# mmigas/LiverRenderer

Hardware: AMD Instinct MI355X
Metric: Msamples/s (higher is better)
Workload: dtype f32; 1 GPU; C3 Liver-SingleMesh volpath 1920x1080 512 spp max_depth 12 (homogeneous medium, isotropic phase, envmap); width=1920, height=1080, spp=512, parallelism=1 GPU

## Files before the change

include/liverrt.h:

```cpp
#ifndef LIVERRT_H
#define LIVERRT_H

#include <stdint.h>
#include <stddef.h>

#ifdef __cplusplus
extern "C" {
#endif

#define LRT_API __attribute__((visibility("default")))

typedef enum {
    LRT_OK = 0,
    LRT_ERR_INVALID = 1,
    LRT_ERR_IO = 2,
    LRT_ERR_DEVICE = 3,
    LRT_ERR_UNSUPPORTED = 4
} lrt_status;

enum { LRT_INTEGRATOR_PATH = 0, LRT_INTEGRATOR_VOLPATH = 1, LRT_INTEGRATOR_PRBVOLPATH = 2,
       LRT_INTEGRATOR_VOLPATHMIS = 5,
       LRT_INTEGRATOR_BIOVOLPATH = 3,
       LRT_INTEGRATOR_BIOVOLPATH06 = 4    };
enum { LRT_MEDIUM_HOMOGENEOUS = 0, LRT_MEDIUM_LIVER = 1, LRT_MEDIUM_PARENCHYMA = 2, LRT_MEDIUM_GLISSON = 3,
// ... 129 lines not shown
} lrt_integrator_desc;

typedef struct {
    uint32_t n_vertices, n_faces, n_shapes, n_bsdfs, n_textures, n_media, n_emitters;
    const float    *positions;
    const float    *normals;
    const float    *texcoords;
    const uint32_t *faces;
    const uint32_t *face_shape;
    const lrt_shape_desc   *shapes;
    const lrt_bsdf_desc    *bsdfs;
    const lrt_texture_desc *textures;
    const lrt_medium_desc  *media;
    const lrt_emitter_desc *emitters;
    lrt_sensor_desc     sensor;
    lrt_film_desc       film;
    lrt_integrator_desc integrator;
    uint32_t sample_count;
    uint32_t sampler_seed;
    uint32_t sampler_type;
    uint32_t samples_per_pass;
    uint32_t use_spectral_mis;
    uint32_t pad;
    uint32_t n_phases, pad_phases;
    const lrt_phase_desc *phases;
} lrt_scene_desc;

typedef struct {
    int32_t  integrator;
    int32_t  max_depth;
    int32_t  rr_depth;
    int32_t  hide_emitters;
    uint32_t spp;
    uint32_t seed;
    uint32_t tile_rank, tile_count;
    int32_t  device;
    int32_t  output_on_device;
    int32_t  grad_medium;
    int32_t  pad;
} lrt_render_opts;

typedef struct {
    uint64_t n_samples;
    uint64_t n_iter;
    uint64_t n_shadow;
    uint64_t n_launches;
    uint64_t n_records;
    double   kernel_ms;
    double   total_ms;
    uint64_t lds_resident;
    uint64_t record_bytes;
    uint64_t n_closed_guard;
    uint64_t n_proven;
} lrt_render_stats;

typedef struct {
    float d_sigma_t[3];
    float d_albedo[3];
    float d_g;
} lrt_param_grads;

typedef struct lrt_scene lrt_scene;

LRT_API const char *lrt_last_error(void);
LRT_API int         lrt_version(void);

LRT_API lrt_status lrt_scene_load_xml(const char *path, const char *const *defines,
                                      int n_defines, lrt_scene **out);
LRT_API lrt_status lrt_scene_load_xml_string(const char *xml, const char *base_dir,
                                             const char *const *defines, int n_defines,
                                             lrt_scene **out);
LRT_API lrt_status lrt_scene_from_desc(const lrt_scene_desc *desc, lrt_scene **out);
LRT_API const lrt_scene_desc *lrt_scene_desc_get(const lrt_scene *scene);
LRT_API void       lrt_scene_free(lrt_scene *scene);

LRT_API lrt_status lrt_render(lrt_scene *scene, const lrt_render_opts *opts,
                              float *film_raw, float *image);
LRT_API lrt_status lrt_render_stats_get(const lrt_scene *scene, lrt_render_stats *out);
LRT_API lrt_status lrt_film_develop(lrt_scene *scene, const float *film_raw, float *image,
                                    int on_device);

LRT_API lrt_status lrt_render_samples(lrt_scene *scene, const lrt_render_opts *opts,
                                      uint64_t lane_begin, uint32_t n, float *out);

LRT_API lrt_status lrt_render_backward(lrt_scene *scene, const lrt_render_opts *opts,
                                       const float *grad_image, lrt_param_grads *out);

LRT_API lrt_status lrt_render_backward_grid(lrt_scene *scene, const lrt_render_opts *opts, const float *grad_image,
                                            lrt_param_grads *out, float *d_grid);

LRT_API lrt_status lrt_render_multi(lrt_scene *scene, const lrt_render_opts *opts, int n_devices, const int *device_ids,
                                    float *film_raw, float *image);
LRT_API lrt_status lrt_render_backward_multi(lrt_scene *scene, const lrt_render_opts *opts, int n_devices, const int *device_ids,
                                             const float *grad_image, lrt_param_grads *out);

LRT_API lrt_status lrt_math_eval(int fn, const float *x, const float *y, uint32_t n, float *out, float *out2, int device);

#define LRT_PROBE_FLOATS 20
LRT_API lrt_status lrt_emitter_probe(lrt_scene *scene, const float *ref_p, const float *sample, uint32_t n, float *out, int device);

LRT_API lrt_status lrt_envmap_probe(lrt_scene *scene, const float *dir, uint32_t n, float *out, int device);

#define LRT_BSDF_PROBE_FLOATS 30
LRT_API lrt_status lrt_bsdf_probe(lrt_scene *scene, const float *o, const float *d, const float *sample, const float *wo_query,
                                  uint32_t n, float *out, int device);

#define LRT_PHASE_PROBE_FLOATS 7
LRT_API lrt_status lrt_phase_probe(lrt_scene *scene, int medium, const float *wi, const float *sample, const float *wo_query,
                                   uint32_t n, float *out, int device);

#define LRT_MEDIUM_PROBE_FLOATS 22
LRT_API lrt_status lrt_medium_probe(lrt_scene *scene, int medium, const float *o, const float *d, const float *maxt, const float *sample,
                                    const uint32_t *channel, uint32_t n, float *out, int device);

#define LRT_SENSOR_PROBE_FLOATS 16
LRT_API lrt_status lrt_sensor_probe(lrt_scene *scene, const float *in, uint32_t n, float *out, int device);

typedef struct { const float *ox, *oy, *oz, *dx, *dy, *dz, *tmax; } lrt_rays_soa;
typedef struct { float *t, *u, *v; uint32_t *prim; } lrt_hits_soa;
LRT_API lrt_status lrt_trace(lrt_scene *scene, const lrt_rays_soa *rays,
                             const lrt_hits_soa *hits, uint32_t n, int any_hit);

LRT_API lrt_status lrt_param_set(lrt_scene *scene, const char *key, const float *v, int n);
LRT_API lrt_status lrt_param_get(const lrt_scene *scene, const char *key, float *v, int n);

LRT_API lrt_status lrt_image_read(const char *path, int *width, int *height, int *channels, float **data);
LRT_API void       lrt_image_free(float *data);
LRT_API lrt_status lrt_image_write_exr(const char *path, int width, int height, int channels, const float *data);
LRT_API lrt_status lrt_image_write_png(const char *path, int width, int height, int channels, const float *data);

#define LRT_AOV_MAX_INTEGRATORS 4
// ... 90 lines not shown
```

liverrenderer_amd/__init__.py:

```python
import ctypes as C
import math
import os

import numpy as np

from . import _lib
from ._lib import make_opts

__all__ = ["set_variant", "variant", "variants", "load_file", "load_string", "load_dict", "cornell_box", "render",
           "traverse", "Scene", "ScalarTransform4f", "render_stats", "write_volume_grid", "Bitmap", "Struct", "util", "read_image", "write_exr", "write_png",
           "Denoiser", "OptixDenoiser", "denoise", "moment_variance", "z_test"]

_VARIANT = "hip_ad_rgb"


def variants():
    return ["hip_ad_rgb"]


def set_variant(name):
    global _VARIANT
    if name not in variants():
        raise ImportError(f"Requested an unsupported variant \"{name}\". The following variants are available: "
                          + ", ".join(variants()) + ".")
# ... 339 lines not shown
        out = _lib.ParamGrads()
        _lib.check(self._lib.lrt_render_backward(self._h, C.byref(o), g.ctypes.data, C.byref(out)))
        return {"sigma_t": np.array(out.d_sigma_t[:], dtype=np.float32), "albedo": np.array(out.d_albedo[:], dtype=np.float32),
                "g": float(out.d_g)}

    def heterogeneous_media(self):
        d = self.desc
        return [i for i in range(d.n_media) if d.media[i].type == _lib.MEDIUM["heterogeneous"]]

    def grid_shape(self, medium):
        r = self.desc.media[medium].grid_res
        return (int(r[2]), int(r[1]), int(r[0]))

    def _render_backward_grid(self, grad_image, kw):
        m = kw.get("medium")
        if m is None or m < 0:
            het = self.heterogeneous_media()
            if len(het) != 1:
                raise RuntimeError(f"render_backward(grid=True): the scene holds {len(het)} heterogeneous media; name one with medium=")
            m = het[0]
        if not 0 <= m < self.desc.n_media or m not in self.heterogeneous_media():
            shape = None
        else:
            shape = self.grid_shape(m)
        out_t = kw.get("out")
        on_device = out_t is not None
        h, w, c = self.film_shape()
        if on_device:
            import torch
            if not _is_torch(out_t) or not out_t.is_cuda or out_t.dtype != torch.float32 or not out_t.is_contiguous() or (shape is not None and tuple(out_t.shape) != shape):
                raise RuntimeError(f"render_backward(grid=True): out must be a contiguous float32 CUDA tensor of shape {shape}")
            dev = out_t.device.index or 0
            if kw.get("device", dev) != dev:
                raise RuntimeError(f"render_backward(grid=True): out lives on {out_t.device}, the render was asked for device {kw['device']}")
            g = grad_image if _is_torch(grad_image) else torch.from_numpy(np.ascontiguousarray(grad_image, dtype=np.float32))
            g = g.to(device=out_t.device, dtype=torch.float32).contiguous()
            if g.numel() != h * w * c:
                raise RuntimeError(f"render_backward: grad_image has {g.numel()} values, the image {h * w * c}")
            torch.cuda.current_stream(out_t.device).synchronize()
            g_ptr, d_ptr, res = g.data_ptr(), out_t.data_ptr(), out_t
        else:
            g = np.ascontiguousarray(grad_image, dtype=np.float32)
            if g.size != h * w * c:
                raise RuntimeError(f"render_backward: grad_image has {g.size} values, the image {h * w * c}")
            res = np.empty(shape if shape is not None else (1,), dtype=np.float32)
            g_ptr, d_ptr, dev = g.ctypes.data, res.ctypes.data, kw.get("device", 0)
        o = make_opts(kw.get("integrator"), kw.get("max_depth"), kw.get("rr_depth"), kw.get("hide_emitters"), kw.get("spp", 0),
                      kw.get("seed", 0), kw.get("tile_rank", 0), kw.get("tile_count", 1), dev, on_device, grad_medium=m)
        out = _lib.ParamGrads()
        _lib.check(self._lib.lrt_render_backward_grid(self._h, C.byref(o), C.c_void_p(g_ptr), C.byref(out), C.c_void_p(d_ptr)))
        return {"sigma_t": np.array(out.d_sigma_t[:], dtype=np.float32), "albedo": np.array(out.d_albedo[:], dtype=np.float32),
                "g": float(out.d_g), "sigma_t_data": res}

    def stats(self):
        s = _lib.RenderStats()
        _lib.check(self._lib.lrt_render_stats_get(self._h, C.byref(s)))
        return {k: getattr(s, k) for k, _ in _lib.RenderStats._fields_}

    def trace(self, o, d, tmax=None, any_hit=False):
        o = np.ascontiguousarray(o, dtype=np.float32); d = np.ascontiguousarray(d, dtype=np.float32)
        n = o.shape[0]
        tmax = np.full(n, np.finfo(np.float32).max, dtype=np.float32) if tmax is None else np.ascontiguousarray(tmax, dtype=np.float32)
        cols = [np.ascontiguousarray(a) for a in (o[:, 0], o[:, 1], o[:, 2], d[:, 0], d[:, 1], d[:, 2], tmax)]
        t = np.empty(n, np.float32); u = np.empty(n, np.float32); v = np.empty(n, np.float32); prim = np.empty(n, np.uint32)
        FP = C.POINTER(C.c_float)
        rays = _lib.RaysSoA(*[c.ctypes.data_as(FP) for c in cols])
        hits = _lib.HitsSoA(t.ctypes.data_as(FP), u.ctypes.data_as(FP), v.ctypes.data_as(FP), prim.ctypes.data_as(C.POINTER(C.c_uint32)))
        _lib.check(self._lib.lrt_trace(self._h, C.byref(rays), C.byref(hits), n, int(any_hit)))
        return t, u, v, prim

    def _probe(self, name, inputs, out_width, alloc=np.empty, medium=None, device=0):
        cols = [np.ascontiguousarray(a, dtype=dt).reshape(-1, w) for _, a, w, dt in inputs]
        n = cols[0].shape[0]
        if any(c.shape[0] != n for c in cols):
            names = [i[0] for i in inputs]
            raise ValueError("%s: %s and %s must have the same number of rows" % (name, ", ".join(names[:-1]), names[-1]))
        out = alloc((n, out_width), dtype=np.float32)
        ptr = lambda a: a.ctypes.data_as(C.POINTER(np.ctypeslib.as_ctypes_type(a.dtype)))
        _lib.check(getattr(self._lib, "lrt_" + name)(self._h, *([] if medium is None else [int(medium)]), *map(ptr, cols), n, ptr(out), int(device)))
        return out

    def emitter_probe(self, ref_p, sample, device=0):
        out = self._probe("emitter_probe", [("ref_p", ref_p, 3, np.float32), ("sample", sample, 2, np.float32)], _lib.PROBE_FLOATS, device=device)
        return {"p": out[:, 0:3], "n": out[:, 3:6], "d": out[:, 6:9], "dist": out[:, 9], "pdf": out[:, 10], "weight": out[:, 11:14],
                "emitter": out[:, 14].astype(np.int32), "hit_shape": out[:, 15].astype(np.int32), "hit_pdf": out[:, 16], "hit_le": out[:, 17:20]}

    def envmap_probe(self, directions, device=0):
        out = self._probe("envmap_probe", [("directions", directions, 3, np.float32)], 4, device=device)
        return out[:, 0].copy(), out[:, 1:4].copy()

    def phase_probe(self, medium, wi, sample, wo_query, device=0):
        out = self._probe("phase_probe", [("wi", wi, 3, np.float32), ("sample", sample, 3, np.float32), ("wo_query", wo_query, 3, np.float32)],
                          _lib.PHASE_PROBE_FLOATS, np.zeros, medium, device)
        return {"wo": out[:, 0:3], "weight": out[:, 3], "pdf": out[:, 4], "eval": out[:, 5], "eval_pdf": out[:, 6]}

    def medium_probe(self, medium, o, d, maxt, sample, channel, device=0):
        out = self._probe("medium_probe", [("o", o, 3, np.float32), ("d", d, 3, np.float32), ("maxt", maxt, 1, np.float32), ("sample", sample, 1, np.float32),
                                           ("channel", channel, 1, np.uint32)], _lib.MEDIUM_PROBE_FLOATS, np.zeros, medium, device)
        return _lib.medium_probe_fields(out)

    def sensor_probe(self, inputs, device=0):
        return _lib.sensor_probe_fields(self._probe("sensor_probe", [("inputs", inputs, 5, np.float32)], _lib.SENSOR_PROBE_FLOATS, np.zeros, device=device))

    def bsdf_probe(self, o, d, sample, wo_query, device=0):
        out = self._probe("bsdf_probe", [("o", o, 3, np.float32), ("d", d, 3, np.float32), ("sample", sample, 3, np.float32), ("wo_query", wo_query, 3, np.float32)],
                          _lib.BSDF_PROBE_FLOATS, device=device)
# ... 475 lines not shown
```

liverrenderer_amd/_lib.py:

```python
import ctypes as C
import os

_HERE = os.path.dirname(os.path.abspath(__file__))
LIB_PATH = os.environ.get("LRT_LIBRARY") or os.path.join(_HERE, "libliverrt.so")

OK, INVALID, UNSUPPORTED = 0, 1, 4
INTEGRATOR = {"path": 0, "volpath": 1, "prbvolpath": 2, "biovolpath": 3, "biovolpath06": 4, "volpathmis": 5}
MEDIUM = {"homogeneous": 0, "liver": 1, "parenchyma": 2, "glissonCapsule": 3, "heterogeneous": 4}
EMITTER = {"area": 0, "envmap": 1, "constant": 2, "point": 3, "spot": 4, "directional": 5}
PROBE_FLOATS = 20
MEDIUM_PROBE_FLOATS = 22
PHASE_PROBE_FLOATS = 7
SENSOR_PROBE_FLOATS = 16
BSDF_PROBE_FLOATS = 30


class ShapeDesc(C.Structure):
    _fields_ = [("kind", C.c_int32), ("first_face", C.c_uint32), ("n_faces", C.c_uint32), ("bsdf", C.c_int32),
                ("emitter", C.c_int32), ("interior_medium", C.c_int32), ("exterior_medium", C.c_int32),
                ("has_normals", C.c_int32), ("has_texcoords", C.c_int32), ("flip_normals", C.c_int32),
                ("to_world", C.c_float * 16)]


class TextureDesc(C.Structure):
# ... 38 lines not shown
class SensorDesc(C.Structure):
    _fields_ = [("to_world", C.c_float * 16), ("fov_x", C.c_float), ("near_clip", C.c_float), ("far_clip", C.c_float),
                ("medium", C.c_int32), ("principal_point_offset_x", C.c_float), ("principal_point_offset_y", C.c_float), ("pad", C.c_int32)]


class FilmDesc(C.Structure):
    _fields_ = [("width", C.c_int32), ("height", C.c_int32), ("crop_offset_x", C.c_int32), ("crop_offset_y", C.c_int32),
                ("crop_width", C.c_int32), ("crop_height", C.c_int32), ("has_alpha", C.c_int32), ("rfilter", C.c_int32),
                ("rfilter_param", C.c_float)]


class IntegratorDesc(C.Structure):
    _fields_ = [("type", C.c_int32), ("max_depth", C.c_int32), ("rr_depth", C.c_int32), ("hide_emitters", C.c_int32)]


class SceneDesc(C.Structure):
    _fields_ = [("n_vertices", C.c_uint32), ("n_faces", C.c_uint32), ("n_shapes", C.c_uint32), ("n_bsdfs", C.c_uint32),
                ("n_textures", C.c_uint32), ("n_media", C.c_uint32), ("n_emitters", C.c_uint32),
                ("positions", C.POINTER(C.c_float)), ("normals", C.POINTER(C.c_float)), ("texcoords", C.POINTER(C.c_float)),
                ("faces", C.POINTER(C.c_uint32)), ("face_shape", C.POINTER(C.c_uint32)),
                ("shapes", C.POINTER(ShapeDesc)), ("bsdfs", C.POINTER(BsdfDesc)), ("textures", C.POINTER(TextureDesc)),
                ("media", C.POINTER(MediumDesc)), ("emitters", C.POINTER(EmitterDesc)),
                ("sensor", SensorDesc), ("film", FilmDesc), ("integrator", IntegratorDesc),
                ("sample_count", C.c_uint32), ("sampler_seed", C.c_uint32),
                ("sampler_type", C.c_uint32), ("samples_per_pass", C.c_uint32), ("use_spectral_mis", C.c_uint32), ("pad", C.c_uint32),
                ("n_phases", C.c_uint32), ("pad_phases", C.c_uint32), ("phases", C.POINTER(PhaseDesc))]


AOV_MAX_INTEGRATORS, AOV_MAX_AOVS, AOV_NAME_LEN = 4, 16, 64
AOV_TYPES = {"albedo": 0, "depth": 1, "position": 2, "uv": 3, "geo_normal": 4, "sh_normal": 5, "dp_du": 6, "dp_dv": 7,
             "prim_index": 8, "shape_index": 9}


class AovDesc(C.Structure):
    _fields_ = [("n_integrators", C.c_int32), ("integrators", IntegratorDesc * AOV_MAX_INTEGRATORS),
                ("integrator_names", (C.c_char * AOV_NAME_LEN) * AOV_MAX_INTEGRATORS),
                ("n_aovs", C.c_int32), ("aov_types", C.c_int32 * AOV_MAX_AOVS), ("aov_names", (C.c_char * AOV_NAME_LEN) * AOV_MAX_AOVS),
                ("n_aov_channels", C.c_int32), ("n_channels", C.c_int32)]


class MomentDesc(C.Structure):
    _fields_ = [("integrator", IntegratorDesc), ("name", C.c_char * AOV_NAME_LEN), ("n_channels", C.c_int32), ("n_raw_channels", C.c_int32)]


class RenderOpts(C.Structure):
    _fields_ = [("integrator", C.c_int32), ("max_depth", C.c_int32), ("rr_depth", C.c_int32), ("hide_emitters", C.c_int32),
                ("spp", C.c_uint32), ("seed", C.c_uint32), ("tile_rank", C.c_uint32), ("tile_count", C.c_uint32),
                ("device", C.c_int32), ("output_on_device", C.c_int32), ("grad_medium", C.c_int32), ("pad", C.c_int32)]


class RenderStats(C.Structure):
    _fields_ = [("n_samples", C.c_uint64), ("n_iter", C.c_uint64), ("n_shadow", C.c_uint64), ("n_launches", C.c_uint64),
                ("n_records", C.c_uint64), ("kernel_ms", C.c_double), ("total_ms", C.c_double), ("lds_resident", C.c_uint64),
                ("record_bytes", C.c_uint64), ("n_closed_guard", C.c_uint64), ("n_proven", C.c_uint64)]


class ParamGrads(C.Structure):
    _fields_ = [("d_sigma_t", C.c_float * 3), ("d_albedo", C.c_float * 3), ("d_g", C.c_float)]


class DenoiseParams(C.Structure):
    _fields_ = [("iterations", C.c_int32), ("sigma_color", C.c_float), ("sigma_normal", C.c_float), ("sigma_albedo", C.c_float), ("eps_a", C.c_float)]


class RaysSoA(C.Structure):
    _fields_ = [(n, C.POINTER(C.c_float)) for n in ("ox", "oy", "oz", "dx", "dy", "dz", "tmax")]


class HitsSoA(C.Structure):
    _fields_ = [("t", C.POINTER(C.c_float)), ("u", C.POINTER(C.c_float)), ("v", C.POINTER(C.c_float)), ("prim", C.POINTER(C.c_uint32))]


def make_opts(integrator=None, max_depth=None, rr_depth=None, hide_emitters=None, spp=0, seed=0,
              tile_rank=0, tile_count=1, device=0, output_on_device=False, grad_medium=0):
    o = RenderOpts()
    o.integrator = -1 if integrator is None else (INTEGRATOR[integrator] if isinstance(integrator, str) else int(integrator))
    o.max_depth = -2 if max_depth is None else int(max_depth)
    o.rr_depth = -1 if rr_depth is None else int(rr_depth)
    o.hide_emitters = -1 if hide_emitters is None else int(bool(hide_emitters))
    o.spp, o.seed, o.tile_rank, o.tile_count = int(spp), int(seed) & 0xffffffff, int(tile_rank), int(tile_count)
    o.device, o.output_on_device = int(device), int(bool(output_on_device))
    o.grad_medium = int(grad_medium)
    return o


_lib = None


def _pytorch_context_first():
    import importlib.util
    import sys
    if os.environ.get("LRT_NO_TORCH_INIT"):
        return "skipped"
    if "torch" not in sys.modules and importlib.util.find_spec("torch") is None:
        return "no torch"
    import torch
    if not torch.cuda.is_available():
        return "no device"
    if not torch.cuda.is_initialized():
        lr = os.environ.get("LOCAL_RANK")
        if lr is not None and lr.isdigit() and torch.cuda.device_count() > 0:
            torch.cuda.set_device(int(lr) % torch.cuda.device_count())
        torch.zeros(1, device="cuda")
    if not torch.cuda.is_initialized():
        raise RuntimeError("PyTorch is importable but its HIP context could not be created before libliverrt.so was loaded; "
                           "set LRT_NO_TORCH_INIT=1 if this process does not use PyTorch")
    return "initialised"


def lib():
    global _lib
    if _lib is not None:
        return _lib
    _pytorch_context_first()
    if not os.path.exists(LIB_PATH):
        raise RuntimeError(f"{LIB_PATH} is missing: build it with `python -c 'import __graft_entry__ as g; g.build()'` "
                           "(the hip_ad_rgb back-end has no CPU fallback)")
    L = C.CDLL(LIB_PATH)
    P = C.POINTER
    L.lrt_last_error.restype = C.c_char_p
    L.lrt_version.restype = C.c_int
    L.lrt_scene_load_xml.argtypes = [C.c_char_p, P(C.c_char_p), C.c_int, P(C.c_void_p)]
    L.lrt_scene_load_xml_string.argtypes = [C.c_char_p, C.c_char_p, P(C.c_char_p), C.c_int, P(C.c_void_p)]
    L.lrt_scene_from_desc.argtypes = [P(SceneDesc), P(C.c_void_p)]
    L.lrt_scene_desc_get.argtypes = [C.c_void_p]
    L.lrt_scene_desc_get.restype = P(SceneDesc)
    L.lrt_scene_free.argtypes = [C.c_void_p]
    L.lrt_scene_free.restype = None
    L.lrt_render.argtypes = [C.c_void_p, P(RenderOpts), C.c_void_p, C.c_void_p]
    L.lrt_render_multi.argtypes = [C.c_void_p, P(RenderOpts), C.c_int, P(C.c_int), C.c_void_p, C.c_void_p]
    L.lrt_render_backward_multi.argtypes = [C.c_void_p, P(RenderOpts), C.c_int, P(C.c_int), C.c_void_p, P(ParamGrads)]
    L.lrt_math_eval.argtypes = [C.c_int, P(C.c_float), P(C.c_float), C.c_uint32, P(C.c_float), P(C.c_float), C.c_int]
    L.lrt_render_stats_get.argtypes = [C.c_void_p, P(RenderStats)]
    L.lrt_film_develop.argtypes = [C.c_void_p, C.c_void_p, C.c_void_p, C.c_int]
    L.lrt_render_samples.argtypes = [C.c_void_p, P(RenderOpts), C.c_uint64, C.c_uint32, C.c_void_p]
    L.lrt_render_backward.argtypes = [C.c_void_p, P(RenderOpts), C.c_void_p, P(ParamGrads)]
    L.lrt_render_backward_grid.argtypes = [C.c_void_p, P(RenderOpts), C.c_void_p, P(ParamGrads), C.c_void_p]
    L.lrt_render_backward_grid.restype = C.c_int
    L.lrt_trace.argtypes = [C.c_void_p, P(RaysSoA), P(HitsSoA), C.c_uint32, C.c_int]
    F, U = P(C.c_float), P(C.c_uint32)
    for name, medium, arrays in (("lrt_emitter_probe", 0, [F, F]), ("lrt_envmap_probe", 0, [F]), ("lrt_bsdf_probe", 0, [F, F, F, F]),
                                 ("lrt_phase_probe", 1, [F, F, F]), ("lrt_medium_probe", 1, [F, F, F, F, U]), ("lrt_sensor_probe", 0, [F])):
        getattr(L, name).argtypes = [C.c_void_p] + [C.c_int] * medium + arrays + [C.c_uint32, F, C.c_int]
        getattr(L, name).restype = C.c_int
    L.lrt_param_set.argtypes = [C.c_void_p, C.c_char_p, P(C.c_float), C.c_int]
    L.lrt_param_get.argtypes = [C.c_void_p, C.c_char_p, P(C.c_float), C.c_int]
    L.lrt_image_read.argtypes = [C.c_char_p, P(C.c_int), P(C.c_int), P(C.c_int), P(P(C.c_float))]
    L.lrt_image_free.argtypes = [P(C.c_float)]
    L.lrt_image_free.restype = None
    L.lrt_image_write_exr.argtypes = [C.c_char_p, C.c_int, C.c_int, C.c_int, C.c_void_p]
    L.lrt_image_write_png.argtypes = [C.c_char_p, C.c_int, C.c_int, C.c_int, C.c_void_p]
    L.lrt_image_write_exr_channels.argtypes = [C.c_char_p, C.c_int, C.c_int, C.c_int, P(C.c_char_p), C.c_void_p]
    L.lrt_scene_aov_get.argtypes = [C.c_void_p, P(AovDesc)]
    L.lrt_aov_channel_name.argtypes = [C.c_void_p, C.c_int]
    L.lrt_aov_channel_name.restype = C.c_char_p
    L.lrt_render_aov.argtypes = [C.c_void_p, P(RenderOpts), C.c_void_p, C.c_void_p]
    L.lrt_render_aov_samples.argtypes = [C.c_void_p, P(RenderOpts), C.c_uint64, C.c_uint32, C.c_void_p]
    L.lrt_scene_moment_get.argtypes = [C.c_void_p, P(MomentDesc)]
    L.lrt_moment_channel_name.argtypes = [C.c_void_p, C.c_int]
    L.lrt_moment_channel_name.restype = C.c_char_p
    L.lrt_render_moment.argtypes = [C.c_void_p, P(RenderOpts), C.c_void_p, C.c_void_p]
    L.lrt_render_moment_samples.argtypes = [C.c_void_p, P(RenderOpts), C.c_uint64, C.c_uint32, C.c_void_p]
    L.lrt_denoiser_create.argtypes = [C.c_int, C.c_int, C.c_int, C.c_int, C.c_int, P(DenoiseParams), C.c_int, P(C.c_void_p)]
    L.lrt_denoise.argtypes = [C.c_void_p, C.c_void_p, C.c_int, C.c_void_p, C.c_void_p, C.c_void_p, C.c_int]
    L.lrt_denoiser_free.argtypes = [C.c_void_p]
    L.lrt_denoiser_free.restype = None
    L.lrt_denoiser_get.argtypes = [C.c_void_p, P(C.c_int), P(C.c_int), P(DenoiseParams)]
    L.lrt_image_read_named.argtypes = [C.c_char_p, P(C.c_int), P(C.c_int), P(C.c_int), P(P(C.c_float)), P(C.c_void_p)]
    L.lrt_image_free_names.argtypes = [C.c_void_p]
    L.lrt_image_free_names.restype = None
    for name in ("lrt_denoiser_create", "lrt_denoise", "lrt_denoiser_get", "lrt_image_read_named", "lrt_scene_moment_get", "lrt_render_moment", "lrt_render_moment_samples"):
        getattr(L, name).restype = C.c_int
    for name in ("lrt_image_read", "lrt_image_write_exr", "lrt_image_write_png", "lrt_scene_load_xml", "lrt_scene_load_xml_string", "lrt_scene_from_desc", "lrt_render", "lrt_render_multi", "lrt_render_backward_multi", "lrt_math_eval", "lrt_render_stats_get",
                 "lrt_film_develop", "lrt_render_samples", "lrt_render_backward", "lrt_trace", "lrt_param_set", "lrt_param_get",
                 "lrt_image_write_exr_channels", "lrt_scene_aov_get", "lrt_render_aov", "lrt_render_aov_samples"):
        getattr(L, name).restype = C.c_int
    _lib = L
    return L


EXPORTED_SYMBOLS = ["lrt_last_error", "lrt_version", "lrt_scene_load_xml", "lrt_scene_load_xml_string", "lrt_scene_from_desc",
                    "lrt_scene_desc_get", "lrt_scene_free", "lrt_render", "lrt_render_multi", "lrt_render_backward_multi", "lrt_math_eval", "lrt_render_stats_get", "lrt_film_develop",
                    "lrt_render_samples", "lrt_render_backward", "lrt_render_backward_grid", "lrt_trace", "lrt_emitter_probe", "lrt_envmap_probe", "lrt_bsdf_probe", "lrt_phase_probe", "lrt_medium_probe", "lrt_sensor_probe", "lrt_param_set", "lrt_param_get",
                    "lrt_image_read", "lrt_image_free", "lrt_image_write_exr", "lrt_image_write_png",
                    "lrt_vae_model_create", "lrt_vae_model_free", "lrt_vae_scatter",
                    "lrt_scene_aov_get", "lrt_aov_channel_name", "lrt_render_aov", "lrt_render_aov_samples", "lrt_image_write_exr_channels",
                    "lrt_denoiser_create", "lrt_denoise", "lrt_denoiser_free", "lrt_denoiser_get", "lrt_image_read_named", "lrt_image_free_names",
                    "lrt_scene_moment_get", "lrt_moment_channel_name", "lrt_render_moment", "lrt_render_moment_samples"]


def bsdf_probe_fields(out):
    return {"shape": out[:, 0].astype("int32"), "t": out[:, 1], "p": out[:, 2:5], "n": out[:, 5:8], "sh_n": out[:, 8:11], "uv": out[:, 11:13],
            "wi": out[:, 13:16], "wo": out[:, 16:19], "wo_z": out[:, 19], "pdf": out[:, 20], "eta": out[:, 21], "type": out[:, 22].astype("int32"),
            "weight": out[:, 23:26], "eval": out[:, 26:29], "eval_pdf": out[:, 29], "raw": out}


def medium_probe_fields(out):
    return {"valid": out[:, 0] != 0, "t": out[:, 1], "p": out[:, 2:5], "mint": out[:, 5], "sigma_t": out[:, 6:9], "sigma_s": out[:, 9:12],
            "sigma_n": out[:, 12:15], "combined": out[:, 15:18], "local": out[:, 18:21], "grid": out[:, 21], "raw": out}


def sensor_probe_fields(out):
    return {"o": out[:, 0:3], "d": out[:, 3:6], "maxt": out[:, 6], "adjusted": out[:, 7:9], "origin": out[:, 9:11].astype("int64"),
            "rel": out[:, 11:13], "weight": out[:, 13], "fcount": out[:, 14].astype("int64"), "raw": out}


def check(status):
    if status != OK:
        raise RuntimeError(lib().lrt_last_error().decode("utf-8", "replace"))
```

liverrenderer_amd/csrc/capi.cpp:

```cpp
#include "host_scene.h"
#include "device_scene.h"
#include "scene_prep.h"
#include "scene_check.h"
#include "image_io.h"
#include <algorithm>
#include <cmath>
#include <cstring>
#include <cstdio>
#include <fstream>
#include <sstream>
#include <stdexcept>

using namespace lrt;

static thread_local std::string g_error;
static lrt_status fail(lrt_status st, const std::string &msg) { g_error = msg; return st; }

#define LRT_TRY try {
#define LRT_CATCH } catch (const std::exception &e) { \
        std::string m = e.what(); \
        lrt_status st = LRT_ERR_INVALID; \
        if (m.find("hip") != std::string::npos || m.find("HIP") != std::string::npos) st = LRT_ERR_DEVICE; \
        if (m.find("cannot open") != std::string::npos || m.find("file not found") != std::string::npos) st = LRT_ERR_IO; \
        if (m.find("unsupported") != std::string::npos || m.find("not supported") != std::string::npos) st = LRT_ERR_UNSUPPORTED; \
        return fail(st, m); \
    } catch (...) { return fail(LRT_ERR_INVALID, "unknown error"); }

extern "C" {

const char *lrt_last_error(void) { return g_error.c_str(); }
int lrt_version(void) { return 120; }

static std::vector<std::pair<std::string, std::string>> parse_defines(const char *const *defines, int n) {
    std::vector<std::pair<std::string, std::string>> r;
    for (int i = 0; i < n; ++i) {
        std::string s = defines[i]; size_t eq = s.find('=');
        if (eq == std::string::npos) throw std::runtime_error("define \"" + s + "\" must have the form key=value");
        r.emplace_back(s.substr(0, eq), s.substr(eq + 1));
    }
    return r;
}

lrt_status lrt_scene_load_xml_string(const char *xml, const char *base_dir, const char *const *defines, int n_defines, lrt_scene **out) {
    if (!xml || !out) return fail(LRT_ERR_INVALID, "lrt_scene_load_xml_string: null argument");
    *out = nullptr;
    LRT_TRY
        std::unique_ptr<lrt_scene> s(new lrt_scene());
        load_scene_xml(xml, base_dir ? base_dir : "", parse_defines(defines, n_defines), s->st);
        *out = s.release();
        return LRT_OK;
    LRT_CATCH
}

lrt_status lrt_scene_load_xml(const char *path, const char *const *defines, int n_defines, lrt_scene **out) {
    if (!path || !out) return fail(LRT_ERR_INVALID, "lrt_scene_load_xml: null argument");
    *out = nullptr;
    std::ifstream f(path, std::ios::binary);
    if (!f) return fail(LRT_ERR_IO, std::string("cannot open \"") + path + "\"");
    std::stringstream ss; ss << f.rdbuf();
    std::string p = path, dir; size_t sl = p.rfind('/'); dir = sl == std::string::npos ? "." : p.substr(0, sl);
    return lrt_scene_load_xml_string(ss.str().c_str(), dir.c_str(), defines, n_defines, out);
}

lrt_status lrt_scene_from_desc(const lrt_scene_desc *desc, lrt_scene **out) {
    if (!desc || !out) return fail(LRT_ERR_INVALID, "lrt_scene_from_desc: null argument");
    *out = nullptr;
    LRT_TRY
        validate_scene_desc(*desc);
        std::unique_ptr<lrt_scene> s(new lrt_scene());
        s->st.copy_from(*desc);
        *out = s.release();
        return LRT_OK;
    LRT_CATCH
}

const lrt_scene_desc *lrt_scene_desc_get(const lrt_scene *scene) { return scene ? &scene->st.desc : nullptr; }

static void multi_release(lrt_scene *s) {
    if (s->multi_ctx) { multi_context_destroy(s->multi_ctx); s->multi_ctx = nullptr; }
    for (auto *D : s->multi) device_scene_destroy(D);
    s->multi.clear(); s->multi_ids.clear();
}

void lrt_scene_free(lrt_scene *scene) {
// ... 146 lines not shown
    if (st != LRT_OK) return st;
    LRT_TRY
        ensure_device(scene, opts ? opts->device : 0);
        device_render_aov_samples(scene->dev, scene->st.desc, scene->st.aov, opts, lane_begin, n, out, scene->stats);
        return LRT_OK;
    LRT_CATCH
}

lrt_status lrt_scene_moment_get(const lrt_scene *scene, lrt_moment_desc *out) {
    if (!scene || !out) return fail(LRT_ERR_INVALID, "lrt_scene_moment_get: null argument");
    if (!scene->st.has_moment) return fail(LRT_ERR_INVALID, "lrt_scene_moment_get: the scene has no moment integrator");
    *out = scene->st.moment; return LRT_OK;
}

const char *lrt_moment_channel_name(const lrt_scene *scene, int c) {
    if (!scene || !scene->st.has_moment || c < 0 || c >= (int) scene->st.moment_channel_names.size()) return nullptr;
    return scene->st.moment_channel_names[(size_t) c].c_str();
}

static lrt_status check_moment_call(const lrt_scene *scene, const lrt_render_opts *opts, const char *fn) {
    if (!scene->st.has_moment) return fail(LRT_ERR_INVALID, std::string(fn) + ": the scene has no moment integrator");
    if (opts && (opts->integrator != -1 || opts->max_depth != -2 || opts->rr_depth != -1 || opts->hide_emitters != -1))
        return fail(LRT_ERR_INVALID, std::string(fn) + ": integrator, max_depth, rr_depth and hide_emitters come from the scene's nested integrator (leave them at -1 / -2 / -1 / -1)");
    return LRT_OK;
}

lrt_status lrt_render_moment(lrt_scene *scene, const lrt_render_opts *opts, float *film_raw, float *image) {
    if (!scene) return fail(LRT_ERR_INVALID, "lrt_render_moment: null scene");
    lrt_status st = check_moment_call(scene, opts, "lrt_render_moment");
    if (st != LRT_OK) return st;
    LRT_TRY
        ensure_device(scene, opts ? opts->device : 0);
        device_render_moment(scene->dev, scene->st.desc, opts, film_raw, image, scene->stats);
        return LRT_OK;
    LRT_CATCH
}

lrt_status lrt_render_moment_samples(lrt_scene *scene, const lrt_render_opts *opts, uint64_t lane_begin, uint32_t n, float *out) {
    if (!scene || !out) return fail(LRT_ERR_INVALID, "lrt_render_moment_samples: null argument");
    lrt_status st = check_moment_call(scene, opts, "lrt_render_moment_samples");
    if (st != LRT_OK) return st;
    LRT_TRY
        ensure_device(scene, opts ? opts->device : 0);
        device_render_moment_samples(scene->dev, scene->st.desc, opts, lane_begin, n, out, scene->stats);
        return LRT_OK;
    LRT_CATCH
}

lrt_status lrt_trace(lrt_scene *scene, const lrt_rays_soa *rays, const lrt_hits_soa *hits, uint32_t n, int any_hit) {
    if (!scene || !rays || !hits) return fail(LRT_ERR_INVALID, "lrt_trace: null argument");
    LRT_TRY
        ensure_device(scene, -1);
        device_trace(scene->dev, rays, hits, n, any_hit);
        return LRT_OK;
    LRT_CATCH
}

static lrt_status probe_call(const char *fn, ProbeKind kind, lrt_scene *scene, const int *medium, std::initializer_list<ProbeColumn> columns, uint32_t n, float *out, int device) {
    bool null = !scene || (!out && n);
    for (const ProbeColumn &c : columns) null = null || (!c.p && n);
    if (null) return fail(LRT_ERR_INVALID, std::string(fn) + ": null argument");
    if (medium && (*medium < 0 || (size_t) *medium >= scene->st.media.size())) return fail(LRT_ERR_INVALID, std::string(fn) + ": no such medium");
    LRT_TRY
        ensure_device(scene, device);
        device_probe(scene->dev, kind, medium ? *medium : 0, columns, n, out);
        return LRT_OK;
    LRT_CATCH
}

lrt_status lrt_emitter_probe(lrt_scene *scene, const float *ref_p, const float *sample, uint32_t n, float *out, int device) {
    return probe_call("lrt_emitter_probe", PROBE_EMITTER, scene, nullptr, { { ref_p, 3 }, { sample, 2 } }, n, out, device);
}

lrt_status lrt_envmap_probe(lrt_scene *scene, const float *dir, uint32_t n, float *out, int device) {
    return probe_call("lrt_envmap_probe", PROBE_ENVMAP, scene, nullptr, { { dir, 3 } }, n, out, device);
}

lrt_status lrt_bsdf_probe(lrt_scene *scene, const float *o, const float *d, const float *sample, const float *wo_query, uint32_t n, float *out, int device) {
    return probe_call("lrt_bsdf_probe", PROBE_BSDF, scene, nullptr, { { o, 3 }, { d, 3 }, { sample, 3 }, { wo_query, 3 } }, n, out, device);
}

lrt_status lrt_phase_probe(lrt_scene *scene, int medium, const float *wi, const float *sample, const float *wo_query, uint32_t n, float *out, int device) {
    return probe_call("lrt_phase_probe", PROBE_PHASE, scene, &medium, { { wi, 3 }, { sample, 3 }, { wo_query, 3 } }, n, out, device);
}

lrt_status lrt_medium_probe(lrt_scene *scene, int medium, const float *o, const float *d, const float *maxt, const float *sample, const uint32_t *channel,
                            uint32_t n, float *out, int device) {
    LRT_TRY
        std::vector<float> ch;
        if (channel) for (uint32_t i = 0; i < n; ++i) ch.push_back((float) std::min<uint32_t>(channel[i], 2u));
        return probe_call("lrt_medium_probe", PROBE_MEDIUM, scene, &medium, { { o, 3 }, { d, 3 }, { maxt, 1 }, { sample, 1 }, { channel ? ch.data() : nullptr, 1 } }, n, out, device);
    LRT_CATCH
}

lrt_status lrt_sensor_probe(lrt_scene *scene, const float *in, uint32_t n, float *out, int device) {
    return probe_call("lrt_sensor_probe", PROBE_SENSOR, scene, nullptr, { { in, 5 } }, n, out, device);
}

static lrt_medium_desc *find_medium(lrt_scene *s, const char *key, const char **rest) {
    for (auto &M : s->st.media) {
        size_t L = strlen(M.id);
        if (!strncmp(key, M.id, L) && key[L] == '.') { *rest = key + L + 1; return &M; }
    }
    return nullptr;
}

// ... 204 lines not shown
```

liverrenderer_amd/csrc/device.hip:

```cpp
#include "host_scene.h"
#include "device_scene.h"
#include "kernels_prb.h"
#include "kernels_vae.h"
#include "kernels_aov.h"
#include "kernels_denoise.h"
#include "kernels_moment.h"
#include "probes.h"
#include <functional>
#include "scene_prep.h"
#include <cmath>
#include <array>
#include <cstring>
#include <algorithm>
#include <stdexcept>
#include <string>
#include <cstdio>
#include <cstdlib>
#include <thread>
#include <chrono>
#include <exception>
#include <dlfcn.h>
#include <rccl/rccl.h>

namespace lrt {

#define HIP_CHECK(expr) do { hipError_t e_ = (expr); if (e_ != hipSuccess) throw std::runtime_error(std::string(#expr) + ": " + hipGetErrorString(e_)); } while (0)

template <typename T> static T *dev_upload(const T *src, size_t n, hipStream_t st) {
    T *p = nullptr; size_t bytes = std::max<size_t>(n, 1) * sizeof(T);
    HIP_CHECK(hipMalloc((void **) &p, bytes));
    if (n) HIP_CHECK(hipMemcpyAsync(p, src, n * sizeof(T), hipMemcpyHostToDevice, st));
    return p;
}

struct DevTmp {
    float *p = nullptr;
    DevTmp() = default;
    explicit DevTmp(size_t floats) { alloc(floats); }
    DevTmp(const DevTmp &) = delete; DevTmp &operator=(const DevTmp &) = delete;
    void alloc(size_t floats) { HIP_CHECK(hipMalloc((void **) &p, std::max<size_t>(floats, 1) * sizeof(float))); }
    void upload(const float *src, size_t floats, hipStream_t st) { alloc(floats); HIP_CHECK(hipMemcpyAsync(p, src, floats * sizeof(float), hipMemcpyHostToDevice, st)); }
    ~DevTmp() { if (p) (void) hipFree(p); }
};

static void select_device(int device) {
    int count = 0;
    if (hipGetDeviceCount(&count) != hipSuccess || count == 0) throw std::runtime_error("no HIP device available: the hip_ad_rgb back-end has no CPU fallback");
    if (device < 0 || device >= count) throw std::runtime_error("invalid HIP device ordinal " + std::to_string(device));
    HIP_CHECK(hipSetDevice(device));
}

static lrt_render_opts default_opts() { return lrt_render_opts{ -1, -2, -1, -1, 0, 0, 0, 1, 0, 0, 0, 0 }; }

static void add_stats(lrt_render_stats &total, const lrt_render_stats &s) {
    total.n_samples += s.n_samples; total.n_iter += s.n_iter; total.n_shadow += s.n_shadow; total.n_launches += s.n_launches;
    total.n_records += s.n_records; total.kernel_ms += s.kernel_ms; total.total_ms += s.total_ms;
    total.record_bytes = s.record_bytes; total.n_closed_guard += s.n_closed_guard; total.n_proven += s.n_proven;
}

#define LRT_LAUNCH_SLOTS 64
#define LRT_WIDE_BLOCK 768

struct DeviceScene {
    int device = 0;
    hipStream_t stream = nullptr;
    DScene sc{};
    DScene *d_sc = nullptr;
    DLaunch *d_launch = nullptr, *h_launch = nullptr; uint32_t launch_next = 0;
    std::vector<void *> allocs;
    uint32_t capacity = 0;
    DPathStreams q[2]{};
    float4 *dl[2] = { nullptr, nullptr }; size_t dl_records[2] = { 0, 0 }; float4 *L_buf = nullptr; size_t l_buf_lanes = 0;
    double *d_grads = nullptr; float *wfilm = nullptr; size_t wfilm_floats = 0; float *grad_image = nullptr; size_t grad_floats = 0;
    DCounters *counters = nullptr;
    DCounters *h_counters = nullptr;
    float *film = nullptr; size_t film_floats = 0;
    float *image = nullptr; size_t image_floats = 0;
    unsigned long long *pass_state[2] = { nullptr, nullptr }; size_t pass_state_lanes[2] = { 0, 0 };
    const unsigned long long *cur_pass_in = nullptr; unsigned long long *cur_pass_out = nullptr;
    uint32_t *pixel_slot = nullptr;
    uint32_t *pixel_list = nullptr; uint32_t pixel_list_rank = 0xffffffffu, pixel_list_count = 0, n_owned_pixels = 0;
    uint32_t *halo_list = nullptr; uint32_t halo_rank = 0xffffffffu, halo_count = 0, halo_width = 0, n_halo_pixels = 0;
    std::vector<hipEvent_t> ev_pool;
    std::vector<DMedium> h_media; DMedium *d_media = nullptr;
    std::vector<DBioMedium> h_bio; DBioMedium *d_bio = nullptr;
    std::vector<DHetMedium> h_het; DHetMedium *d_het = nullptr; std::vector<float *> het_data; bool has_het = false, has_non_bio = false, need_mis = false; uint32_t ws_layouts = 0;
    bool ext = false;
    bool smooth_bsdf = false;
    bool has_area_emitter = false;
    float *dgrid = nullptr; size_t dgrid_floats = 0;
    bool prb_null = false;
    DLdsInfo lds{}; bool use_lds = false; int n_cus = 256; int bvh_leaf = 4;
    DAovSpec *d_aov_spec = nullptr; uint32_t *d_first_face = nullptr;
    float *aov_film = nullptr; size_t aov_film_floats = 0; float *aov_image = nullptr; size_t aov_image_floats = 0; float *aov_inner = nullptr; size_t aov_inner_floats = 0;

    template <typename T> T *track(T *p) { allocs.push_back((void *) p); return p; }
    void release(void *p) {
        if (!p) return;
        for (auto it = allocs.begin(); it != allocs.end(); ++it) if (*it == p) { allocs.erase(it); break; }
        (void) hipFree(p);
    }
    template <typename T> T *grow(T *&p, size_t &have, size_t want) {
        if (have >= want) return p;
        HIP_CHECK(hipStreamSynchronize(stream));
        release(p); p = nullptr; have = 0;
        HIP_CHECK(hipMalloc((void **) &p, std::max<size_t>(want, 1) * sizeof(T))); track(p);
        have = want;
        return p;
    }
    ~DeviceScene() {
        for (void *p : allocs) (void) hipFree(p);
        for (auto e : ev_pool) (void) hipEventDestroy(e);
        if (h_counters) (void) hipHostFree(h_counters);
        if (h_launch) (void) hipHostFree(h_launch);
        if (stream) (void) hipStreamDestroy(stream);
    }
};

void device_scene_destroy(DeviceScene *d) { delete d; }

static_assert(PREP_F_DELTA == F_DELTA && PREP_F_SMOOTH == F_SMOOTH && PREP_F_NULL == F_NULL, "scene_prep.h restates the BSDF leaf flags of dshade.h");

__global__ void k_bio_prepare(DBioMedium *bio, uint32_t n) {
    const uint32_t i = blockIdx.x * blockDim.x + threadIdx.x;
    if (i < n) bio[i].log10_hep = m_log2(bio[i].hepatocity + 1.f) / m_log2(10.f);
}

__global__ void k_medium_prepare(DMedium *media, uint32_t n) {
// ... 110 lines not shown
    prepare_geometry(d, opt, P);
    D->n_cus = opt.n_cus; D->bvh_leaf = P.bvh_leaf; D->ext = P.ext; D->smooth_bsdf = P.smooth_bsdf;
    auto up = [&](const auto &v) { return D->track(dev_upload(v.data(), v.size(), st)); };
    sc.spheres = P.spheres.empty() ? nullptr : up(P.spheres);
    sc.nodes = (const float4 *) up(P.bvh.nodes);
    sc.tris = (const float4 *) up(P.bvh.tris);
    if (P.use_lds) {
        D->lds = P.lds; D->lds.blob = (const uint4 *) up(P.lds_blob);
        const size_t lds_limit = opt.lds_limit;
        auto raise_lds = [&](const void *k) { if (k) HIP_CHECK(hipFuncSetAttribute(k, hipFuncAttributeMaxDynamicSharedMemorySize, (int) lds_limit)); };
        const KernelTable &K = kernels();
        for (const RenderRow &r : K.render) if (r.lds && (!r.ext || D->ext)) raise_lds((const void *) r.fn);
        for (const auto &adjoint : K.prb) for (const auto &ld : adjoint[1]) for (RenderFn fn : ld) raise_lds((const void *) fn);
        for (RenderFn fn : K.prb_grid[1]) raise_lds((const void *) fn);
        for (int i = 0; i < 2; ++i) for (int ext = 0; ext <= (D->ext ? 1 : 0); ++ext) {
            raise_lds((const void *) aov_kernel(true, i, ext)); raise_lds((const void *) trace_lds_kernel(i, ext));
        }
        D->use_lds = true;
    }
    if (sc.grid.enabled) {
        const size_t n_cells = (size_t) sc.grid.n[0] * sc.grid.n[1] * sc.grid.n[2];
        uint16_t *buf = nullptr; HIP_CHECK(hipMalloc((void **) &buf, n_cells * sizeof(uint16_t))); D->track(buf);
        k_build_dist_grid<<<(uint32_t) ((n_cells + LRT_BLOCK - 1) / LRT_BLOCK), LRT_BLOCK, 0, st>>>(sc.tris, d.n_faces ? (uint32_t) (P.bvh.tris.size() / 12) : 0u, sc.grid, buf, P.grid_abs_margin,
                                                                                             sc.spheres, sc.n_spheres);
        HIP_CHECK(hipGetLastError());
        sc.grid.d = buf;
    }
    prepare_shading(d, opt, P);
    D->has_area_emitter = P.has_area_emitter; D->has_het = P.has_het; D->has_non_bio = P.has_non_bio; D->prb_null = P.prb_null;
    sc.positions = D->track(dev_upload(d.positions, 3 * (size_t) d.n_vertices, st));
    sc.vattr = (const float4 *) up(P.vattr);
    sc.faces = D->track(dev_upload(d.faces, 3 * (size_t) d.n_faces, st));
    sc.face_shape = D->track(dev_upload(d.face_shape, d.n_faces, st));
    sc.shapes = up(P.shapes);
    sc.textures = up(P.textures);
    sc.tex_data = up(P.tex_data);
    sc.bsdfs = up(P.bsdfs);
    HIP_CHECK(hipMalloc((void **) &D->d_media, std::max<uint32_t>(d.n_media, 1) * sizeof(DMedium))); D->track(D->d_media);
    HIP_CHECK(hipMalloc((void **) &D->d_bio, std::max<uint32_t>(d.n_media, 1) * sizeof(DBioMedium))); D->track(D->d_bio);
    HIP_CHECK(hipMalloc((void **) &D->d_het, std::max<uint32_t>(d.n_media, 1) * sizeof(DHetMedium))); D->track(D->d_het);
    D->het_data.assign(std::max<uint32_t>(d.n_media, 1), nullptr);
    for (uint32_t i = 0; i < d.n_media; ++i) {
        const lrt_medium_desc &M = d.media[i];
        if (M.type == LRT_MEDIUM_HETEROGENEOUS) D->het_data[i] = D->track(dev_upload(M.grid_data, (size_t) M.grid_res[0] * M.grid_res[1] * M.grid_res[2], st));
    }
    D->sc = sc;
    upload_media(D.get(), d); sc.media = D->d_media; sc.bio = D->d_bio; sc.het = D->d_het;
    sc.emitters = up(P.emitters);
    sc.mesh_emitters = up(P.mesh_emitters);
    sc.mesh_emitter_tab = up(P.mesh_emitter_tab);
    sc.delta_emitters = P.delta_emitters.empty() ? nullptr : up(P.delta_emitters);
    sc.bsdf_ext = P.bsdf_ext.empty() ? nullptr : up(P.bsdf_ext);
    sc.cone_tab = P.cone_tab.empty() ? nullptr : (const uint2 *) up(P.cone_tab);
    sc.phases = P.phases.empty() ? nullptr : up(P.phases);
    sc.phase_pool = P.phase_pool.empty() ? nullptr : up(P.phase_pool);
    sc.env_data = (const float4 *) up(P.env_data);
    sc.env_hier = up(P.env_hier);
    HIP_CHECK(hipMalloc((void **) &D->d_sc, sizeof(DScene))); D->track(D->d_sc);
    D->sc = sc;
    HIP_CHECK(hipMemcpyAsync(D->d_sc, &D->sc, sizeof(DScene), hipMemcpyHostToDevice, st));
    HIP_CHECK(hipMalloc((void **) &D->d_launch, LRT_LAUNCH_SLOTS * sizeof(DLaunch))); D->track(D->d_launch);
    HIP_CHECK(hipHostMalloc((void **) &D->h_launch, LRT_LAUNCH_SLOTS * sizeof(DLaunch)));
    HIP_CHECK(hipMalloc((void **) &D->counters, sizeof(DCounters))); D->track(D->counters);
    HIP_CHECK(hipHostMalloc((void **) &D->h_counters, sizeof(DCounters)));
    HIP_CHECK(hipStreamSynchronize(st));
    return D.release();
}

void device_scene_update_params(DeviceScene *D, const lrt_scene_desc &d, bool grids) {
    HIP_CHECK(hipSetDevice(D->device));
    if (grids) for (uint32_t i = 0; i < d.n_media; ++i) {
        const lrt_medium_desc &M = d.media[i];
        if (M.type == LRT_MEDIUM_HETEROGENEOUS && D->het_data[i])
            HIP_CHECK(hipMemcpyAsync(D->het_data[i], M.grid_data, (size_t) M.grid_res[0] * M.grid_res[1] * M.grid_res[2] * sizeof(float), hipMemcpyHostToDevice, D->stream));
    }
    upload_media(D, d);
    HIP_CHECK(hipStreamSynchronize(D->stream));
}

static void ensure_workspace(DeviceScene *D, uint32_t capacity) {
    const uint32_t layouts = workspace_layouts(D->has_het, D->need_mis);
    if (D->capacity >= capacity && D->ws_layouts == layouts) return;
    HIP_CHECK(hipStreamSynchronize(D->stream));
    D->capacity = 0;
    auto get = [](const DPathStreams *q, const RecordStream &r) { void *p; memcpy(&p, (const char *) q + r.member, sizeof p); return p; };
    auto set = [](DPathStreams *q, const RecordStream &r, void *p) { memcpy((char *) q + r.member, &p, sizeof p); };
    for (DPathStreams *q : { &D->q[0], &D->q[1] })
        for (const RecordStream &r : kRecordStreams) if (r.member != kNoMember) { D->release(get(q, r)); set(q, r, nullptr); }
    for (DPathStreams *q : { &D->q[0], &D->q[1] })
        for (size_t k = 0; k < std::size(kRecordStreams); ++k) if (const uint32_t bytes = workspace_stream_bytes(k, layouts)) {
            void *p = nullptr; HIP_CHECK(hipMalloc(&p, (size_t) capacity * bytes)); D->track(p); set(q, kRecordStreams[k], p);
        }
    D->capacity = capacity; D->ws_layouts = layouts;
}

static hipEvent_t get_event(DeviceScene *D, size_t i) {
    while (D->ev_pool.size() <= i) { hipEvent_t e; HIP_CHECK(hipEventCreate(&e)); D->ev_pool.push_back(e); }
    return D->ev_pool[i];
}

static void ensure_pixel_list(DeviceScene *D, const ResolvedOpts &O) {
    const DFilm &F = D->sc.film;
    if (O.tile_count == 1) { D->n_owned_pixels = (uint32_t) F.width * F.height; return; }
    if (D->pixel_list && D->pixel_list_rank == O.tile_rank && D->pixel_list_count == O.tile_count) return;
    const TilePixels T = tile_pixel_list(F, O.tile_rank, O.tile_count);
    D->release(D->pixel_list); D->release(D->pixel_slot); D->pixel_list = nullptr; D->pixel_slot = nullptr;
// ... 114 lines not shown
        case LRT_INTEGRATOR_PATH: case LRT_INTEGRATOR_BIOVOLPATH: case LRT_INTEGRATOR_BIOVOLPATH06: mode = integrator; break;
        case LRT_INTEGRATOR_VOLPATHMIS: mode = spectral_mis ? LRT_INTEGRATOR_VOLPATHMIS : LRT_INTEGRATOR_VOLPATHMIS_PLAIN; break;
        default: mode = closed ? LRT_INTEGRATOR_VOLPATH_CLOSED : (has_het ? LRT_INTEGRATOR_VOLPATH_HET : LRT_INTEGRATOR_VOLPATH);
    }
    for (const RenderRow &r : kernels().render) if (r.mode == mode && r.lds == lds && r.ld == ld && r.compact == compact && r.ext == ext) return r;
    throw std::runtime_error("no render-kernel instance for mode " + std::to_string(mode) + (lds ? ", LDS BVH" : ", global BVH") + (ld ? ", ld sampler" : ", independent sampler") +
                             (compact ? ", compact records" : ", wide records") + (ext ? ", EXT" : ""));
}

static void run_wavefront(DeviceScene *D, const lrt_scene_desc &d, const ResolvedOpts &O, uint64_t lane_begin, uint64_t n_lanes,
                          const uint32_t *pixel_list, float *film, float *sample_out, lrt_render_stats &stats) {
    hipStream_t st = D->stream;
    DRenderParams rp = make_params(d, O, n_lanes);
    rp.pixel_slot = pixel_list ? D->pixel_slot : nullptr;
    rp.pass_in = D->cur_pass_in; rp.pass_out = D->cur_pass_out;
    const bool prb = O.integrator == LRT_INTEGRATOR_PRBVOLPATH;
    check_integrator_media(D, O.integrator);
    PoolGeometry g = pool_geometry(D, n_lanes);
    const uint32_t records = (uint32_t) std::min<uint64_t>((uint64_t) g.n_wg * 2u * g.P, 0xffffffffull);
    ensure_workspace(D, records);
    if (prb) ensure_prb_workspace(D, records, 0);
    HIP_CHECK(hipMemsetAsync(D->counters, 0, sizeof(DCounters), st));
    LaunchLog log;
    hipEvent_t e_begin = get_event(D, log.ev++), e_end = get_event(D, log.ev++);
    HIP_CHECK(hipEventRecord(e_begin, st));
    const bool count_iter = !(O.integrator == LRT_INTEGRATOR_PATH && O.max_depth == 0);
    hipEvent_t a = get_event(D, log.ev++), b = get_event(D, log.ev++);
    HIP_CHECK(hipEventRecord(a, st));
    if (prb) { stats.record_bytes = 0; launch_prb<false>(D, rp, g, pixel_list, lane_begin, nullptr, nullptr, nullptr, film, sample_out); }
    else {
        DLaunch a{}; a.rp = rp; a.li = D->lds; a.q0 = D->q[0]; a.q1 = D->q[1]; a.P = g.P; a.cnt = D->counters; a.pixel_list = pixel_list;
        a.lane_begin = lane_begin; a.n = n_lanes; a.film = film; a.sample_out = sample_out; a.sample_base = lane_begin;
        const bool compact = D->use_lds && !D->has_area_emitter && !D->ext && !getenv("LRT_WIDE_RECORDS") && O.integrator != LRT_INTEGRATOR_VOLPATHMIS && !(O.integrator == LRT_INTEGRATOR_VOLPATH && D->has_het);
        const bool closed = compact && O.integrator == LRT_INTEGRATOR_VOLPATH && closed_records(d, D->sc.cam.medium) && !getenv("LRT_NO_CLOSED_RECORDS");
#ifdef LRT_DEV_VOLPATH_ONLY
        if (D->ext) throw std::runtime_error("developer build: no EXT instances (spheres / point emitters)");
        if (!(D->use_lds && (O.integrator == LRT_DEV_INTEGRATOR || (LRT_DEV_INTEGRATOR == LRT_INTEGRATOR_VOLPATH_HET && D->has_het)) && (rp.ld_count != 0) == LRT_DEV_LD)) throw std::runtime_error("developer build: one integrator / sampler / LDS BVH only");
#endif
        const RenderRow &row = select_render_kernel(O.integrator, D->has_het, d.use_spectral_mis != 0, D->use_lds, rp.ld_count != 0, D->ext, compact, closed);
        stats.record_bytes = row.record_bytes;
        const LaunchPtr lp = push_launch(D, a);
        row.fn<<<g.n_wg, row.block, g.smem, st>>>((ScenePtr) D->d_sc, lp);
        HIP_CHECK(hipGetLastError());
    }
    HIP_CHECK(hipEventRecord(b, st));
    log.launches.emplace_back(a, b); log.sizes.push_back(0);
    HIP_CHECK(hipMemcpyAsync(D->h_counters, D->counters, sizeof(DCounters), hipMemcpyDeviceToHost, st));
    HIP_CHECK(hipStreamSynchronize(st));
    log.n_iter = count_iter ? D->h_counters->n_iter : 0;
    log.n_records = D->h_counters->n_records;
    finish_stats(D, log, e_begin, e_end, n_lanes, stats);
    stats.n_closed_guard = D->h_counters->n_closed_guard;
    stats.n_proven = D->h_counters->n_proven;
    if (stats.n_closed_guard)
        throw std::runtime_error("64-byte path records: " + std::to_string(stats.n_closed_guard) + " trips broke the premise of the layout (radiance before a path's last trip, "
                                 "or an emitter hit that needs its MIS weight); the scene test in closed_records() is wrong for this scene: LRT_NO_CLOSED_RECORDS=1 renders it with 80-byte records");
}

static void render_passes(DeviceScene *D, const lrt_scene_desc &d, const lrt_render_opts *opts, float *film_raw, float *image, lrt_render_stats &stats,
                          const std::function<void(const ResolvedOpts &)> &after_pass, bool moment = false);

void device_render(DeviceScene *D, const lrt_scene_desc &d, const lrt_render_opts *opts, float *film_raw, float *image, lrt_render_stats &stats) {
    render_passes(D, d, opts, film_raw, image, stats, nullptr);
}

static void develop_and_download(DeviceScene *D, const float *film, float *film_raw, float *image, size_t film_floats, size_t image_floats, bool on_device, bool moment = false) {
    const DFilm &F = D->sc.film; const size_t np = (size_t) F.width * F.height;
    if (image) {
        float *img = on_device ? image : D->grow(D->image, D->image_floats, image_floats);
        if (!moment) k_develop<<<(uint32_t) ((np + 255) / 256), 256, 0, D->stream>>>(F, film, img, (uint32_t) np);
        else if (F.has_alpha) k_moment_develop<true><<<(uint32_t) ((np + 255) / 256), 256, 0, D->stream>>>(film, img, (uint32_t) np);
        else k_moment_develop<false><<<(uint32_t) ((np + 255) / 256), 256, 0, D->stream>>>(film, img, (uint32_t) np);
        if (!on_device) HIP_CHECK(hipMemcpyAsync(image, img, image_floats * 4, hipMemcpyDeviceToHost, D->stream));
    }
    if (film_raw && !on_device) HIP_CHECK(hipMemcpyAsync(film_raw, film, film_floats * 4, hipMemcpyDeviceToHost, D->stream));
    HIP_CHECK(hipStreamSynchronize(D->stream));
    HIP_CHECK(hipGetLastError());
}

static void render_passes(DeviceScene *D, const lrt_scene_desc &d, const lrt_render_opts *opts, float *film_raw, float *image, lrt_render_stats &stats,
                          const std::function<void(const ResolvedOpts &)> &after_pass, bool moment) {
    HIP_CHECK(hipSetDevice(D->device));
    ResolvedOpts O = resolve(d, opts);
    const DFilm &F = D->sc.film;
    bool on_device = opts && opts->output_on_device;
    const size_t film_channels = moment ? (F.has_alpha ? 11 : 10) : (size_t) F.channels, image_channels = moment ? film_channels - 1 : (F.has_alpha ? 4 : 3);
    size_t np = (size_t) F.width * F.height, film_floats = np * film_channels, image_floats = np * image_channels;
    ensure_pixel_list(D, O);
    const uint64_t n_lanes = (uint64_t) D->n_owned_pixels * O.spp;
    float *film = (on_device && film_raw) ? film_raw : D->grow(D->film, D->film_floats, film_floats);
    HIP_CHECK(hipMemsetAsync(film, 0, film_floats * 4, D->stream));
    const uint32_t *pixel_list = O.tile_count > 1 ? D->pixel_list : nullptr;
    const bool carry = O.n_passes > 1 && d.sampler_type != LRT_SAMPLER_LD;
    if (carry) for (int k = 0; k < 2; ++k) D->grow(D->pass_state[k], D->pass_state_lanes[k], n_lanes);
    const bool lane_splat = moment || (F.rfilter != LRT_RFILTER_BOX && (O.n_passes > 1 || !getenv("LRT_NO_LANE_SPLAT")));
    lrt_render_stats total{};
    for (uint32_t pass = 0; pass < O.n_passes; ++pass) {
        O.pass = pass;
        D->cur_pass_in = carry ? D->pass_state[pass & 1] : nullptr;
        D->cur_pass_out = (carry && pass + 1 < O.n_passes) ? D->pass_state[(pass & 1) ^ 1] : nullptr;
        if (!lane_splat) {
            lrt_render_stats st1{};
            run_wavefront(D, d, O, 0, n_lanes, pixel_list, film, nullptr, st1);
            add_stats(total, st1);
            if (after_pass) after_pass(O);
            continue;
        }
        const uint64_t chunk = std::min<uint64_t>(std::max<uint64_t>(n_lanes, 1), 1ull << 28);
        ensure_prb_workspace(D, 0, chunk);
        for (uint64_t base = 0; base < n_lanes; base += chunk) {
            const uint64_t n = std::min<uint64_t>(chunk, n_lanes - base);
            lrt_render_stats st1{};
            run_wavefront(D, d, O, base, n, pixel_list, nullptr, reinterpret_cast<float *>(D->L_buf), st1);
            DRenderParams rp = make_params(d, O, n); rp.pass_in = D->cur_pass_in;
            DLaunch a{}; a.rp = rp; a.L_buf = D->L_buf; a.pixel_list = pixel_list; a.lane_begin = base; a.n = n; a.film = film;
            const uint32_t grid = (uint32_t) ((n + LRT_BLOCK - 1) / LRT_BLOCK);
            const LaunchPtr lp = push_launch(D, a);
            if (!moment) k_splat_lanes<false><<<grid, LRT_BLOCK, 0, D->stream>>>((ScenePtr) D->d_sc, lp);
            else moment_splat_kernel(F.rfilter != LRT_RFILTER_BOX, F.has_alpha != 0)<<<grid, LRT_BLOCK, 0, D->stream>>>((ScenePtr) D->d_sc, lp);
            HIP_CHECK(hipGetLastError());
            add_stats(total, st1);
        }
        if (after_pass) after_pass(O);
    }
    D->cur_pass_in = nullptr; D->cur_pass_out = nullptr;
    total.lds_resident = D->use_lds ? 1 : 0;
    stats = total;
    develop_and_download(D, film, film_raw, image, film_floats, image_floats, on_device, moment);
}

void device_render_moment(DeviceScene *D, const lrt_scene_desc &d, const lrt_render_opts *opts, float *film_raw, float *image, lrt_render_stats &stats) {
    render_passes(D, d, opts, film_raw, image, stats, nullptr, true);
}

void device_render_moment_samples(DeviceScene *D, const lrt_scene_desc &d, const lrt_render_opts *opts, uint64_t lane_begin, uint32_t n, float *out, lrt_render_stats &stats) {
    HIP_CHECK(hipSetDevice(D->device));
    ResolvedOpts O = resolve(d, opts);
    if (lane_begin + n > 0x100000000ull) throw std::runtime_error("lane range exceeds 2^32");
    if (!n) { stats = lrt_render_stats{}; return; }
    DevTmp buf((size_t) n * 10);
    float *d_buf = buf.p, *d_m = d_buf + (size_t) n * 4;
    HIP_CHECK(hipMemsetAsync(d_buf, 0, (size_t) n * 16, D->stream));
    run_wavefront(D, d, O, lane_begin, n, nullptr, nullptr, d_buf, stats);
    k_moment_lanes<<<(n + 255u) / 256u, 256, 0, D->stream>>>(reinterpret_cast<const float4 *>(d_buf), O.integrator == LRT_INTEGRATOR_PATH ? 1 : 0, n, d_m);
    HIP_CHECK(hipGetLastError());
    HIP_CHECK(hipMemcpyAsync(out, d_m, (size_t) n * 24, hipMemcpyDeviceToHost, D->stream));
    HIP_CHECK(hipStreamSynchronize(D->stream));
}

void device_develop(DeviceScene *D, const float *film_raw, float *image, int on_device) {
    HIP_CHECK(hipSetDevice(D->device));
    const DFilm &F = D->sc.film;
    size_t np = (size_t) F.width * F.height, film_floats = np * F.channels, image_floats = np * (F.has_alpha ? 4 : 3);
    const float *film = film_raw;
    if (!on_device) {
        film = D->grow(D->film, D->film_floats, film_floats);
        HIP_CHECK(hipMemcpyAsync(D->film, film_raw, film_floats * 4, hipMemcpyHostToDevice, D->stream));
    }
    develop_and_download(D, film, nullptr, image, film_floats, image_floats, on_device != 0);
}

void device_render_samples(DeviceScene *D, const lrt_scene_desc &d, const lrt_render_opts *opts, uint64_t lane_begin, uint32_t n, float *out, lrt_render_stats &stats) {
    HIP_CHECK(hipSetDevice(D->device));
    ResolvedOpts O = resolve(d, opts);
    if (lane_begin + n > 0x100000000ull) throw std::runtime_error("lane range exceeds 2^32");
    DevTmp d_out((size_t) n * 4);
    HIP_CHECK(hipMemsetAsync(d_out.p, 0, (size_t) n * 16, D->stream));
    run_wavefront(D, d, O, lane_begin, n, nullptr, nullptr, d_out.p, stats);
    HIP_CHECK(hipMemcpyAsync(out, d_out.p, (size_t) n * 16, hipMemcpyDeviceToHost, D->stream));
    HIP_CHECK(hipStreamSynchronize(D->stream));
}

static void upload_aov_spec(DeviceScene *D, const lrt_scene_desc &d, const lrt_aov_desc &aov) {
    if (!D->d_aov_spec) { HIP_CHECK(hipMalloc((void **) &D->d_aov_spec, sizeof(DAovSpec))); D->track(D->d_aov_spec); }
    if (!D->d_first_face) {
        std::vector<uint32_t> ff(std::max<uint32_t>(d.n_shapes, 1), 0u);
        for (uint32_t i = 0; i < d.n_shapes; ++i) ff[i] = d.shapes[i].first_face;
        D->d_first_face = D->track(dev_upload(ff.data(), ff.size(), D->stream));
    }
    static thread_local DAovSpec h;
    h = DAovSpec{}; h.n_aovs = aov.n_aovs; h.first_face = D->d_first_face;
    int off = 0;
    for (int k = 0; k < aov.n_aovs; ++k) {
        h.type[k] = aov.aov_types[k]; h.offset[k] = off;
        off += aov.aov_types[k] == LRT_AOV_DEPTH || aov.aov_types[k] >= LRT_AOV_PRIM_INDEX ? 1 : aov.aov_types[k] == LRT_AOV_UV ? 2 : 3;
    }
    h.n_ch = off;
    if (off != aov.n_aov_channels) throw std::runtime_error("aov: channel count mismatch");
    HIP_CHECK(hipMemcpyAsync(D->d_aov_spec, &h, sizeof(DAovSpec), hipMemcpyHostToDevice, D->stream));
    HIP_CHECK(hipStreamSynchronize(D->stream));
}

static void launch_aov(DeviceScene *D, const lrt_scene_desc &d, const ResolvedOpts &O, uint64_t lane_begin, uint64_t n, float *film, float *sample_out,
                       const unsigned long long *pass_in, unsigned long long *pass_out) {
    if (!n) return;
    hipStream_t st = D->stream;
    DRenderParams rp = make_params(d, O, n);
    rp.pass_in = pass_in; rp.pass_out = pass_out;
    DLaunch a{}; a.rp = rp; a.li = D->lds; a.lane_begin = lane_begin; a.n = n; a.film = film; a.sample_out = sample_out; a.sample_base = lane_begin;
    const LaunchPtr lp = push_launch(D, a);
    const AovSpecPtr spec = (AovSpecPtr) D->d_aov_spec;
    const AovFn fn = aov_kernel(D->use_lds, rp.ld_count != 0, D->ext);
// ... 259 lines not shown
        std::vector<int> ids; for (auto *D : devs) ids.push_back(D->device);
        if (!ctx || ctx->devices != ids) {
            delete ctx; ctx = new MultiContext(); ctx->devices = ids; ctx->comms.assign(N, nullptr);
            g_rccl.check(g_rccl.CommInitAll(ctx->comms.data(), N, ids.data()), "ncclCommInitAll");
        }
        g_rccl.check(g_rccl.GroupStart(), "ncclGroupStart");
        for (int i = 0; i < N; ++i) {
            HIP_CHECK(hipSetDevice(devs[i]->device));
            g_rccl.check(g_rccl.AllReduce(buf[i], buf[i], count, sizeof(T) == 8 ? ncclDouble : ncclFloat, ncclSum, ctx->comms[i], devs[i]->stream), "ncclAllReduce");
        }
        g_rccl.check(g_rccl.GroupEnd(), "ncclGroupEnd");
        for (auto *D : devs) { HIP_CHECK(hipSetDevice(D->device)); HIP_CHECK(hipStreamSynchronize(D->stream)); }
    } else {
        for (int i = 1; i < N; ++i) if (devs[i]->device != devs[0]->device) throw std::runtime_error("lrt_render_multi: a device list is either all distinct or one device repeated");
        static_assert(sizeof(T) == 4 || sizeof(T) == 8, "float or double");
        HIP_CHECK(hipSetDevice(devs[0]->device));
        for (int i = 1; i < N; ++i) {
            if (sizeof(T) == 4) k_film_add<<<(uint32_t) ((count + 255) / 256), 256, 0, devs[0]->stream>>>((float *) buf[0], (const float *) buf[i], count);
            else { std::vector<double> a(count), b(count); HIP_CHECK(hipMemcpy(a.data(), buf[0], count * 8, hipMemcpyDeviceToHost)); HIP_CHECK(hipMemcpy(b.data(), buf[i], count * 8, hipMemcpyDeviceToHost));
                   for (size_t k = 0; k < count; ++k) a[k] += b[k]; HIP_CHECK(hipMemcpy(buf[0], a.data(), count * 8, hipMemcpyHostToDevice)); }
        }
        HIP_CHECK(hipGetLastError()); HIP_CHECK(hipStreamSynchronize(devs[0]->stream));
    }
}

template <typename F> static void on_every_device(size_t n, F fn) {
    std::vector<std::exception_ptr> err(n);
    std::vector<std::thread> th;
    for (size_t i = 0; i < n; ++i) th.emplace_back([&, i]() { try { fn(i); } catch (...) { err[i] = std::current_exception(); } });
    for (auto &t : th) t.join();
    for (auto &e : err) if (e) std::rethrow_exception(e);
}

void device_render_multi(std::vector<DeviceScene *> &devs, MultiContext *&ctx, const lrt_scene_desc &d, const lrt_render_opts *opts, float *film_raw, float *image, lrt_render_stats &stats) {
    const int N = (int) devs.size();
    const DFilm &F = devs[0]->sc.film;
    const size_t np = (size_t) F.width * F.height, film_floats = np * F.channels, image_floats = np * (F.has_alpha ? 4 : 3);
    const bool on_device = opts && opts->output_on_device;
    std::vector<float *> films(N); std::vector<lrt_render_stats> st(N);
    const auto t0 = std::chrono::steady_clock::now();
    on_every_device(N, [&](size_t i) {
        HIP_CHECK(hipSetDevice(devs[i]->device));
        films[i] = (i == 0 && on_device && film_raw) ? film_raw : devs[i]->grow(devs[i]->film, devs[i]->film_floats, film_floats);
        lrt_render_opts o = opts ? *opts : default_opts();
        o.tile_rank = (uint32_t) i; o.tile_count = (uint32_t) N; o.device = devs[i]->device; o.output_on_device = 1;
        device_render(devs[i], d, &o, films[i], nullptr, st[i]);
    });
    if (N > 1 || getenv("LRT_MULTI_ALWAYS_REDUCE")) reduce_across(devs, ctx, films, film_floats);
    DeviceScene *D0 = devs[0];
    HIP_CHECK(hipSetDevice(D0->device));
    develop_and_download(D0, films[0], film_raw, image, film_floats, image_floats, on_device);
    lrt_render_stats total{};
    for (auto &x : st) { total.n_samples += x.n_samples; total.n_iter += x.n_iter; total.n_shadow += x.n_shadow; total.n_launches += x.n_launches; total.n_records += x.n_records;
                         total.kernel_ms = std::max(total.kernel_ms, x.kernel_ms); total.lds_resident = x.lds_resident; total.record_bytes = x.record_bytes; total.n_closed_guard += x.n_closed_guard; total.n_proven += x.n_proven; }
    total.total_ms = std::chrono::duration<double, std::milli>(std::chrono::steady_clock::now() - t0).count();
    stats = total;
}

void device_render_backward_multi(std::vector<DeviceScene *> &devs, MultiContext *&ctx, const lrt_scene_desc &d, const lrt_render_opts *opts, const float *grad_image, lrt_param_grads *out, lrt_render_stats &stats) {
    const int N = (int) devs.size();
    if (opts && opts->output_on_device) throw std::runtime_error("lrt_render_backward_multi: grad_image is a host buffer (every device takes its own copy)");
    std::vector<lrt_param_grads> g(N); std::vector<lrt_render_stats> st(N);
    on_every_device(N, [&](size_t i) {
        lrt_render_opts o = opts ? *opts : default_opts();
        o.tile_rank = (uint32_t) i; o.tile_count = (uint32_t) N; o.device = devs[i]->device; o.output_on_device = 0;
        device_render_backward(devs[i], d, &o, grad_image, &g[i], st[i]);
    });
    std::vector<double *> bufs; for (auto *D : devs) bufs.push_back(D->d_grads);
    if (N > 1) reduce_across(devs, ctx, bufs, 7);
    double h[7]; HIP_CHECK(hipSetDevice(devs[0]->device)); HIP_CHECK(hipMemcpy(h, devs[0]->d_grads, sizeof(h), hipMemcpyDeviceToHost));
    for (int k = 0; k < 3; ++k) { out->d_sigma_t[k] = (float) h[k]; out->d_albedo[k] = (float) h[3 + k]; }
    out->d_g = (float) h[6];
    lrt_render_stats total{};
    for (auto &x : st) { total.n_samples += x.n_samples; total.n_iter += x.n_iter; total.n_shadow += x.n_shadow; total.n_launches += x.n_launches; total.n_records += x.n_records;
                         total.kernel_ms = std::max(total.kernel_ms, x.kernel_ms); total.total_ms = std::max(total.total_ms, x.total_ms); total.lds_resident = x.lds_resident; }
    stats = total;
}

void device_probe(DeviceScene *D, ProbeKind kind, int arg, std::initializer_list<ProbeColumn> columns, uint32_t n, float *out) {
    const ProbeRow &P = kProbes[kind];
    HIP_CHECK(hipSetDevice(D->device));
    if (P.needs_env && D->sc.env.emitter < 0) throw std::runtime_error(std::string(P.name) + ": the scene has no environment emitter");
    if (!n) return;
    int width = 0; for (const ProbeColumn &c : columns) width += c.width;
    if (width != P.in) throw std::logic_error(std::string(P.name) + ": the columns do not add up to the lane record");
    std::vector<float> packed((size_t) n * P.in);
    int at = 0;
    for (const ProbeColumn &c : columns) {
        for (size_t i = 0; i < n; ++i) std::copy_n(c.p + i * c.width, c.width, packed.data() + i * P.in + at);
        at += c.width;
    }
    hipStream_t st = D->stream;
    DevTmp in, dout((size_t) n * P.out);
    in.upload(packed.data(), packed.size(), st);
    probe_kernel(kind)<<<(n + LRT_BLOCK - 1) / LRT_BLOCK, LRT_BLOCK, 0, st>>>((ScenePtr) D->d_sc, arg, in.p, n, dout.p);
    HIP_CHECK(hipGetLastError());
    HIP_CHECK(hipMemcpyAsync(out, dout.p, (size_t) n * P.out * sizeof(float), hipMemcpyDeviceToHost, st));
    HIP_CHECK(hipStreamSynchronize(st));
}

__global__ void k_math_eval(int fn, const float *__restrict__ x, const float *__restrict__ y, uint32_t n, float *__restrict__ out, float *__restrict__ out2) {
    const uint32_t i = blockIdx.x * blockDim.x + threadIdx.x;
    if (i >= n) return;
    float a = 0.f, b = 0.f;
    switch (fn) {
        case 0: a = m_log(x[i]); break;
        case 1: a = m_exp(x[i]); break;
// ... 100 lines not shown
```

liverrenderer_amd/csrc/device_scene.h:

```cpp
#pragma once
#include "../../include/liverrt.h"
#include <initializer_list>
#include <vector>

namespace lrt {
struct DeviceScene;
DeviceScene *device_scene_create(const lrt_scene_desc &d, int device);
void device_scene_destroy(DeviceScene *d);
void device_scene_update_params(DeviceScene *D, const lrt_scene_desc &d, bool grids = false);
void device_render(DeviceScene *D, const lrt_scene_desc &d, const lrt_render_opts *opts, float *film_raw, float *image, lrt_render_stats &stats);
void device_develop(DeviceScene *D, const float *film_raw, float *image, int on_device);
void device_render_aov(DeviceScene *D, const lrt_scene_desc &d, const lrt_aov_desc &aov, const lrt_render_opts *opts, float *aov_film_raw, float *image, lrt_render_stats &stats);
void device_render_aov_samples(DeviceScene *D, const lrt_scene_desc &d, const lrt_aov_desc &aov, const lrt_render_opts *opts, uint64_t lane_begin, uint32_t n, float *out, lrt_render_stats &stats);
void device_render_moment(DeviceScene *D, const lrt_scene_desc &d, const lrt_render_opts *opts, float *film_raw, float *image, lrt_render_stats &stats);
void device_render_moment_samples(DeviceScene *D, const lrt_scene_desc &d, const lrt_render_opts *opts, uint64_t lane_begin, uint32_t n, float *out, lrt_render_stats &stats);
void device_render_samples(DeviceScene *D, const lrt_scene_desc &d, const lrt_render_opts *opts, uint64_t lane_begin, uint32_t n, float *out, lrt_render_stats &stats);
void device_trace(DeviceScene *D, const lrt_rays_soa *rays, const lrt_hits_soa *hits, uint32_t n, int any_hit);
enum ProbeKind { PROBE_EMITTER, PROBE_ENVMAP, PROBE_BSDF, PROBE_PHASE, PROBE_MEDIUM, PROBE_SENSOR, PROBE_KINDS };
struct ProbeColumn { const float *p; int width; };
void device_probe(DeviceScene *D, ProbeKind kind, int arg, std::initializer_list<ProbeColumn> columns, uint32_t n, float *out);
void device_vae_scatter(const float *blob, uint32_t n, const float *in_pos, const float *in_dir, const float *poly, const float albedo[3], float g, float ior,
                        const float sigma_t[3], float fit_scale, uint32_t seed, float *out_pos, float *out_absorption, int device);
void device_render_backward(DeviceScene *D, const lrt_scene_desc &d, const lrt_render_opts *opts, const float *grad_image, lrt_param_grads *out, lrt_render_stats &stats,
                            float *d_grid = nullptr);
void device_math_eval(int fn, const float *x, const float *y, uint32_t n, float *out, float *out2, int device);
struct Denoiser;
Denoiser *denoiser_create(int width, int height, bool use_albedo, bool use_normals, bool denoise_alpha, const lrt_denoise_params &params, int device);
void denoiser_destroy(Denoiser *d);
void denoiser_run(Denoiser *d, const float *noisy, int channels, const float *albedo, const float *normals, float *out, int device_buffers);
struct MultiContext;
void multi_context_destroy(MultiContext *m);
void device_render_multi(std::vector<DeviceScene *> &devs, MultiContext *&ctx, const lrt_scene_desc &d, const lrt_render_opts *opts, float *film_raw, float *image, lrt_render_stats &stats);
void device_render_backward_multi(std::vector<DeviceScene *> &devs, MultiContext *&ctx, const lrt_scene_desc &d, const lrt_render_opts *opts, const float *grad_image, lrt_param_grads *out, lrt_render_stats &stats);
}
```

liverrenderer_amd/csrc/device_types.h:

```cpp
#pragma once
#include <stdint.h>
#include <hip/hip_vector_types.h>

namespace lrt {

struct DShape {
    int32_t bsdf, emitter, interior_medium, exterior_medium;
    int32_t has_normals, has_texcoords, flip_normals, kind;
};

#define LRT_MICRO_GGX 1
#define LRT_MICRO_VISIBLE 2
struct DBsdf {
    int32_t type;
    union { int32_t reflectance; int32_t specular_reflectance; };
    union { int32_t nested; int32_t micro; };
    union { int32_t texture; int32_t specular_transmittance; };
    float eta;
    union { float scale; float alpha_u; };
    int32_t flags;
    union { int32_t pad; float alpha_v; };
};
static_assert(sizeof(DBsdf) == 32, "DBsdf stride");

// ... 99 lines not shown
    int32_t width, height;
    int32_t crop_offset_x, crop_offset_y;
    float scale_x, scale_y, offset_x, offset_y;
    int32_t channels, has_alpha, rfilter, fcount;
    float rf_radius, rf_inv_radius; int32_t fn, pad;
    float rf_coeff[10];
    int32_t pad2[2];
};

struct DEnv {
    int32_t type;
    int32_t emitter;
    uint32_t w, h;
    float scale;
    float bsphere_c[3]; float bsphere_r;
    float to_world[9];
    float to_local[9];
    float patch_size[2], inv_patch_size[2];
    uint32_t max_patch[2];
    int32_t n_levels;
    uint32_t level_offset[LRT_MAX_HIER_LEVELS];
    uint32_t level_width[LRT_MAX_HIER_LEVELS];
    float radiance[3];
};

struct DDistGrid {
    const uint16_t *d;
    float lo[3]; float cell, inv_cell;
    int32_t n[3]; int32_t enabled;
};

struct DScene {
    const float4 *nodes;
    const float4 *tris;
    const float *positions;
    const float4 *vattr;
    const uint32_t *faces, *face_shape;
    const DShape *shapes; const DBsdf *bsdfs; const DTexture *textures; const DMedium *media; const DBioMedium *bio; const DHetMedium *het; const DEmitter *emitters;
    const float *tex_data;
    const float4 *env_data;
    const float *env_hier;
    uint32_t n_faces, n_emitters;
    int32_t root_is_leaf, has_null_bsdf;
    int32_t nee_fast_reject;
    int32_t one_shape;
    uint32_t root_leaf_first, root_leaf_count;
    DCamera cam; DFilm film; DEnv env;
    DDistGrid grid;
    const DSphere *spheres;
    uint32_t n_spheres, pad_sph;
    const DMeshEmitter *mesh_emitters;
    const float *mesh_emitter_tab;
    const uint2 *cone_tab;
    int32_t cone_enabled, pad_cone;
    const DPhase *phases;
    const float *phase_pool;
    const DDeltaEmitter *delta_emitters;
    const DBsdfExt *bsdf_ext;
};

#define LRT_CONE_BINS 4
#define LRT_CONE_COS0 0.95f
#define LRT_CONE_COS1 0.85f
#define LRT_CONE_COS2 0.70f
#define LRT_CONE_COS3 0.50f

#define LRT_CONST __attribute__((address_space(4)))
typedef const LRT_CONST DScene &SceneRef;
typedef const LRT_CONST DFilm &FilmRef;
typedef const LRT_CONST DEnv &EnvRef;
typedef const LRT_CONST DDistGrid &GridRef;
typedef const LRT_CONST DScene *ScenePtr;

struct DRenderParams {
    int32_t integrator, max_depth, rr_depth, hide_emitters;
    uint32_t spp, log2_spp;
    uint32_t seed_value;
    uint32_t base_seed, seed;
    uint32_t ld_count, pad1;
    uint32_t tile_rank, tile_count;
    int32_t grad_medium;
    uint32_t tiles_x, tiles_y, profile;
    uint32_t pad2;
    uint64_t n_lanes;
    const uint32_t *pixel_slot;
    uint32_t pass_index, spp_total;
    const unsigned long long *pass_in;
    unsigned long long *pass_out;
};

struct DPathStreams {
    float4 *o_maxt;
    float4 *d_eta;
    float4 *tp_pdf;
    float4 *res_flags;
    float4 *lp_lane;
    uint2  *rng;
    float2 *tdepth;
    float4 *hit;
    float4 *w1, *w2, *w3, *w4;
};

#define LRT_INTEGRATOR_VOLPATHMIS_PLAIN 102
#define LRT_INTEGRATOR_VOLPATH_HET 101
#define LRT_INTEGRATOR_VOLPATH_CLOSED 103

#define PF_DEPTH_MASK   0x0000ffffu
#define PF_MEDIUM_SHIFT 16
#define PF_MEDIUM_MASK  0x00ff0000u
#define PF_CHANNEL_SHIFT 24
#define PF_SPECULAR     (1u << 26)
#define PF_VALID        (1u << 27)
#define PF_NOHIT        (1u << 28)
#define PF_BIO_SCATTERED (1u << 29)
#define PF_LONG_QUERY   (1u << 29)
#define PF_HAVE_SI      (1u << 29)
#define PF_LAST_NULL    (1u << 30)
#define PF_BIO_EMIT     (1u << 30)
#define PF_BIO_FULL     (1u << 31)

struct DCounters {
    uint32_t pad[4];
    unsigned long long n_shadow;
    unsigned long long n_iter;
    unsigned long long next_lane;
    unsigned long long n_records;
    unsigned long long prof_cycles[4], prof_tiles[4];
    unsigned long long prof_wg[6];
    unsigned long long n_closed_guard;
    unsigned long long n_proven;
};

struct DLdsInfo {
    const uint4 *blob;
    uint32_t blob_bytes, nodes_off, verts_off, tris_off, stack_off, total_bytes;
};

struct DLaunch {
    DRenderParams rp; DLdsInfo li; DPathStreams q0, q1;
    float4 *dl0, *dl1;
    uint32_t P, pad; DCounters *cnt; const uint32_t *pixel_list; uint64_t lane_begin, n;
    float4 *L_buf; const float *grad_image; const float *wfilm; double *grads;
    float *film; float *sample_out; uint64_t sample_base;
    float *dgrid;
};
typedef const LRT_CONST DRenderParams &RpRef;
typedef const LRT_CONST DLaunch *LaunchPtr;

}
```

liverrenderer_amd/csrc/dshade.h:

```cpp
#pragma once
#include "device_types.h"
#include "dmath.h"
#include "../../include/liverrt.h"

namespace lrt {

#define LRT_BLOCK 256
#define LRT_STACK 32

template <class T> DEV T tab(const T *table, uint32_t i, bool worth_a_look = true) {
    if (!worth_a_look) return table[i];
    const uint32_t i0 = (uint32_t) __builtin_amdgcn_readfirstlane((int) i);
    if (__builtin_amdgcn_ballot_w64(true) != 0ull && __builtin_amdgcn_ballot_w64(i != i0) == 0ull)
    { T out; __builtin_memcpy(&out, reinterpret_cast<const LRT_CONST T *>((uintptr_t) table) + i0, sizeof(T)); return out; }
    return table[i];
}

struct Ray { V3 o, d; float maxt; };
struct Hit { float t, u, v; uint32_t prim; uint32_t slot = 0xffffffffu; };
struct SI { bool valid; float t; V3 p, n; Frame sh; V2 uv; V3 dp_du, dp_dv, wi; uint32_t prim, shape; };

DEV float slab_rcp(float x) { return fmin_(fmax_(__builtin_amdgcn_rcpf(x), -1e20f), 1e20f); }
DEV void test_tri(const float4 *__restrict__ tris, uint32_t slot, V3 o, V3 d, float maxt, Hit &best) {
    float4 a = tris[3 * slot], b = tris[3 * slot + 1], c = tris[3 * slot + 2];
// ... 15 lines not shown
template <bool ANY_HIT>
DEV Hit trace(SceneRef sc, const Ray &r, int *__restrict__ stack ) {
    Hit best; best.t = kInf; best.u = best.v = 0.f; best.prim = 0xffffffffu;
    if (sc.n_faces == 0) return best;
    const V3 o = r.o, d = r.d;
    if (sc.root_is_leaf) {
        for (uint32_t i = 0; i < sc.root_leaf_count; ++i) test_tri(sc.tris, sc.root_leaf_first + i, o, d, r.maxt, best);
        return best;
    }
    const float ix = slab_rcp(d.x), iy = slab_rcp(d.y), iz = slab_rcp(d.z);
    const float ox = -o.x * ix, oy = -o.y * iy, oz = -o.z * iz;
    const f32x2 vix = { ix, ix }, viy = { iy, iy }, viz = { iz, iz }, vox = { ox, ox }, voy = { oy, oy }, voz = { oz, oz };
    const uint32_t DONE = 0x7fffffffu;
    int sp = 0; uint32_t cur = 0;
    for (;;) {
        while (cur < DONE) {
            const float4 *nd = sc.nodes + 4 * (size_t) cur;
            float4 n0 = nd[0], n1 = nd[1], n2 = nd[2], n3 = nd[3];
            float limit = fmin_(best.t, r.maxt);
            const f32x2 vax = pk_fma(f32x2{ n0.x, n0.y }, vix, vox), vay = pk_fma(f32x2{ n0.z, n0.w }, viy, voy), vaz = pk_fma(f32x2{ n2.x, n2.y }, viz, voz);
            const f32x2 vbx = pk_fma(f32x2{ n1.x, n1.y }, vix, vox), vby = pk_fma(f32x2{ n1.z, n1.w }, viy, voy), vbz = pk_fma(f32x2{ n2.z, n2.w }, viz, voz);
            const float ax0 = vax.x, ax1 = vax.y, ay0 = vay.x, ay1 = vay.y, az0 = vaz.x, az1 = vaz.y;
            const float bx0 = vbx.x, bx1 = vbx.y, by0 = vby.x, by1 = vby.y, bz0 = vbz.x, bz1 = vbz.y;
            float tmin0 = fmax_(fmax_(fmin_(ax0, ax1), fmin_(ay0, ay1)), fmax_(fmin_(az0, az1), 0.f));
            float tmax0 = fmin_(fmin_(fmax_(ax0, ax1), fmax_(ay0, ay1)), fmin_(fmax_(az0, az1), limit));
            float tmin1 = fmax_(fmax_(fmin_(bx0, bx1), fmin_(by0, by1)), fmax_(fmin_(bz0, bz1), 0.f));
            float tmax1 = fmin_(fmin_(fmax_(bx0, bx1), fmax_(by0, by1)), fmin_(fmax_(bz0, bz1), limit));
            bool h0 = tmin0 <= tmax0 * 1.000002f, h1 = tmin1 <= tmax1 * 1.000002f;
            int r0 = (int) f2u(n3.x), r1 = (int) f2u(n3.y);
            uint32_t c0 = r0 < 0 ? (0x80000000u | (uint32_t) ~r0) : (uint32_t) r0;
            uint32_t c1 = r1 < 0 ? (0x80000000u | (uint32_t) ~r1) : (uint32_t) r1;
            if (h0 && h1) {
                bool swap = tmin1 < tmin0;
                stack[sp * LRT_BLOCK] = (int) (swap ? c0 : c1); ++sp;
                cur = swap ? c1 : c0;
            } else if (h0 || h1) cur = h0 ? c0 : c1;
            else if (sp == 0) cur = DONE;
            else { --sp; cur = (uint32_t) stack[sp * LRT_BLOCK]; }
        }
        if (cur == DONE) break;
        uint32_t slot = cur & 0x7fffffffu; bool last;
        do { last = sc.tris[3 * slot + 1].w != 0.f; test_tri(sc.tris, slot, o, d, r.maxt, best); ++slot; } while (!last);
        if (ANY_HIT && best.prim != 0xffffffffu) return best;
        if (sp == 0) break;
        --sp; cur = (uint32_t) stack[sp * LRT_BLOCK];
    }
    return best;
}

struct GlobalTracer {
    static constexpr bool kExt = false;
    SceneRef sc; int *stack;
    DEV Hit closest(const Ray &r) const { return trace<false>(sc, r, stack); }
    DEV Hit any(const Ray &r) const { return trace<true>(sc, r, stack); }
    DEV SI surface(SceneRef s, const Ray &r, const Hit &h) const;
};

struct LdsScene {
    const float4 *nodes; const float4 *verts; const uint2 *tris;
    uint32_t n_faces, root_is_leaf, root_first, root_count;
};
#define LRT_LDS_BLOCK_MAX 1024

DEV void test_tri_lds(const LdsScene &L, uint2 ix, uint32_t slot, V3 o, V3 d, float maxt, Hit &best) {
    float4 a = L.verts[ix.x & 0xffffu], b = L.verts[ix.x >> 16], c = L.verts[ix.y & 0xffffu];
    V3 p0(a.x, a.y, a.z), e1(b.x - a.x, b.y - a.y, b.z - a.z), e2(c.x - a.x, c.y - a.y, c.z - a.z);
    V3 pvec = cross(d, e2);
    float inv_det = rcp(dot(e1, pvec));
    V3 tvec = o - p0;
    float u = dot(tvec, pvec) * inv_det;
    if (!(u >= 0.f && u <= 1.f)) return;
    V3 qvec = cross(tvec, e1);
    float v = dot(d, qvec) * inv_det;
    if (!(v >= 0.f && u + v <= 1.f)) return;
    float t = dot(e2, qvec) * inv_det;
    if (!(t >= 0.f && t <= maxt)) return;
    if (t > best.t) return;
    uint32_t f = ix.y >> 17;
    if (t < best.t || f < (best.prim & 0x7fffu)) { best.t = t; best.u = u; best.v = v; best.prim = f | (slot << 16); }
}

#ifdef LRT_TRAV_STATS
__device__ unsigned long long g_trav[8];
#define LRT_TRAV_COUNT(k) { const unsigned long long m_ = __ballot(true); if ((threadIdx.x & 63u) == (uint32_t) (__ffsll((long long) m_) - 1)) { atomicAdd(&g_trav[(ANY_HIT ? 4 : 0) + k], 1ull); atomicAdd(&g_trav[(ANY_HIT ? 4 : 0) + k + 1], (unsigned long long) __popcll(m_)); } }
#else
#define LRT_TRAV_COUNT(k)
#endif
template <bool ANY_HIT, int STRIDE>
DEV Hit trace_lds(const LdsScene &L, const Ray &r, uint16_t *__restrict__ stack ) {
    Hit best; best.t = kInf; best.u = best.v = 0.f; best.prim = 0xffffffffu;
    if (L.n_faces == 0) return best;
    const V3 o = r.o, d = r.d;
    if (L.root_is_leaf) {
        for (uint32_t i = 0; i < L.root_count; ++i) test_tri_lds(L, L.tris[L.root_first + i], L.root_first + i, o, d, r.maxt, best);
        if (best.prim != 0xffffffffu) { best.slot = best.prim >> 16; best.prim &= 0x7fffu; }
        return best;
    }
    const float ix = slab_rcp(d.x), iy = slab_rcp(d.y), iz = slab_rcp(d.z);
    const float ox = -o.x * ix, oy = -o.y * iy, oz = -o.z * iz;
    const f32x2 vix = { ix, ix }, viy = { iy, iy }, viz = { iz, iz }, vox = { ox, ox }, voy = { oy, oy }, voz = { oz, oz };
    const uint32_t DONE = 0x10000u;
    int sp = 0; uint32_t cur = 0;
    for (;;) {
        while (cur < 0x8000u) {
            LRT_TRAV_COUNT(0)
            const float4 *nd = L.nodes + 4 * cur;
            float4 n0 = nd[0], n1 = nd[1], n2 = nd[2], n3 = nd[3];
            float limit = fmin_(best.t, r.maxt);
            const f32x2 vax = pk_fma(f32x2{ n0.x, n0.y }, vix, vox), vay = pk_fma(f32x2{ n0.z, n0.w }, viy, voy), vaz = pk_fma(f32x2{ n2.x, n2.y }, viz, voz);
            const f32x2 vbx = pk_fma(f32x2{ n1.x, n1.y }, vix, vox), vby = pk_fma(f32x2{ n1.z, n1.w }, viy, voy), vbz = pk_fma(f32x2{ n2.z, n2.w }, viz, voz);
            const float ax0 = vax.x, ax1 = vax.y, ay0 = vay.x, ay1 = vay.y, az0 = vaz.x, az1 = vaz.y;
            const float bx0 = vbx.x, bx1 = vbx.y, by0 = vby.x, by1 = vby.y, bz0 = vbz.x, bz1 = vbz.y;
            float tmin0 = fmax_(fmax_(fmin_(ax0, ax1), fmin_(ay0, ay1)), fmax_(fmin_(az0, az1), 0.f));
            float tmax0 = fmin_(fmin_(fmax_(ax0, ax1), fmax_(ay0, ay1)), fmin_(fmax_(az0, az1), limit));
            float tmin1 = fmax_(fmax_(fmin_(bx0, bx1), fmin_(by0, by1)), fmax_(fmin_(bz0, bz1), 0.f));
            float tmax1 = fmin_(fmin_(fmax_(bx0, bx1), fmax_(by0, by1)), fmin_(fmax_(bz0, bz1), limit));
            bool h0 = tmin0 <= tmax0 * 1.000002f, h1 = tmin1 <= tmax1 * 1.000002f;
            const uint32_t c0 = f2u(n3.x), c1 = f2u(n3.y);
            if (h0 && h1) {
                bool swap = tmin1 < tmin0;
                stack[sp * STRIDE] = (uint16_t) (swap ? c0 : c1); ++sp;
                cur = swap ? c1 : c0;
            } else if (h0 || h1) cur = h0 ? c0 : c1;
            else if (sp == 0) cur = DONE;
            else { --sp; cur = stack[sp * STRIDE]; }
        }
        if (cur == DONE) break;
        uint32_t slot = cur & 0x7fffu, last;
        do {
            LRT_TRAV_COUNT(2)
            const uint2 ix = L.tris[slot];
            last = (ix.y >> 16) & 1u;
            test_tri_lds(L, ix, slot, o, d, r.maxt, best);
            ++slot;
        } while (!last);
        if (ANY_HIT && best.prim != 0xffffffffu) return best;
        if (sp == 0) break;
        --sp; cur = stack[sp * STRIDE];
    }
    if (best.prim != 0xffffffffu) { best.slot = best.prim >> 16; best.prim &= 0x7fffu; }
    return best;
}

template <int STRIDE>
struct LdsTracer {
    static constexpr bool kExt = false;
    const LdsScene &L; uint16_t *stack;
    DEV Hit closest(const Ray &r) const { return trace_lds<false, STRIDE>(L, r, stack); }
    DEV Hit any(const Ray &r) const { return trace_lds<true, STRIDE>(L, r, stack); }
    DEV SI surface(SceneRef s, const Ray &r, const Hit &h) const;
};

DEV float dist_grid_lower_bound(GridRef g, V3 p) {
    float fx = (p.x - g.lo[0]) * g.inv_cell, fy = (p.y - g.lo[1]) * g.inv_cell, fz = (p.z - g.lo[2]) * g.inv_cell;
    int ix = min(max((int) fx, 0), g.n[0] - 1), iy = min(max((int) fy, 0), g.n[1] - 1), iz = min(max((int) fz, 0), g.n[2] - 1);
    union { uint16_t u; _Float16 h; } cv; cv.u = g.d[(uint32_t) ((iz * g.n[1] + iy) * g.n[0] + ix)];
    float D = (float) cv.h;
    float cx = fx - ((float) ix + .5f), cy = fy - ((float) iy + .5f), cz = fz - ((float) iz + .5f);
    return D - __builtin_amdgcn_sqrtf(cx * cx + cy * cy + cz * cz) * (g.cell * 1.001f);
}

#ifndef LRT_GRID_STEPS
#define LRT_GRID_STEPS 3
#endif
template <int STEPS = LRT_GRID_STEPS>
DEV bool segment_proven_empty(GridRef g, V3 o, V3 d, float maxt) {
    if (!g.enabled || !(maxt < 1e30f)) return false;
    float len = __builtin_amdgcn_sqrtf(dot(d, d));
    float remaining = maxt * len * 1.01f, inv_len = __builtin_amdgcn_rcpf(len);
    V3 p = o;
    for (int k = 0; k < STEPS; ++k) {
        float lb = dist_grid_lower_bound(g, p);
        if (remaining < lb) return true;
        if (!(lb > .5f * g.cell)) return false;
        float adv = lb * .99f;
        p = p + d * (adv * inv_len);
        remaining -= adv * .995f;
    }
    return false;
}

template <int K>
DEV bool segment_covered_by_balls(GridRef g, V3 o, V3 d, float maxt, float start = 0.f) {
    if (!g.enabled || !(maxt < 1e30f)) return false;
    const float len = __builtin_amdgcn_sqrtf(dot(d, d));
    const float L = maxt * len * 1.01f;
#define LRT_FRAC(k) (((float) (k) + .5f) / (float) K)
    float lb[K];
#pragma unroll
    for (int k = 0; k < K; ++k) lb[k] = dist_grid_lower_bound(g, fma3(d, maxt * LRT_FRAC(k), o)) * .995f;
    float covered = start; bool ok = true;
#pragma unroll
    for (int k = 0; k < K; ++k) {
        const float c = L * LRT_FRAC(k);
        ok = ok && (lb[k] > 0.f) && (c - lb[k] <= covered);
        covered = fmax_(covered, c + lb[k]);
    }
    return ok && covered >= L;
#undef LRT_FRAC
}

// ... 1193 lines not shown
```

liverrenderer_amd/csrc/kernels.h:

```cpp
#pragma once
#include "dshade.h"
#include "record.h"

namespace lrt {

#ifndef LRT_STAMP_KIND
#define LRT_STAMP_KIND 0
#endif
struct StampClock {
    unsigned long long *acc; unsigned long long t; bool on;
    DEV void start(unsigned long long *a, bool enable) { acc = a; on = enable; t = on ? __builtin_amdgcn_s_memtime() : 0ull; }
    DEV void at(int k) { if (on) { const unsigned long long now = __builtin_amdgcn_s_memtime(); if ((threadIdx.x & 63u) == 0) atomicAdd(&acc[k], now - t); t = now; } }
};

template <bool LD>
DEV uint64_t lane_rng_inc(RpRef rp, uint32_t lane) {
    if (LD) {
        const uint32_t pixel = (rp.log2_spp != 0xffffffffu) ? (lane >> rp.log2_spp) : (lane / rp.spp);
        uint32_t v0, v1; tea32(rp.base_seed, rp.spp * pixel + rp.seed, &v0, &v1);
        return (uint64_t) v0 | ((uint64_t) (rp.pass_index * rp.spp + (lane - pixel * rp.spp)) << 32);
    }
    uint32_t v0, v1; tea32(rp.seed_value, lane, &v0, &v1);
    return ((uint64_t) v1 << 1) | 1u;
}
// ... 13 lines not shown
    SamplerT<LD> r; r.ld_count = rp.ld_count; r.state = state;
    if (LD) {
        const uint32_t pixel = (rp.log2_spp != 0xffffffffu) ? (lane >> rp.log2_spp) : (lane / rp.spp);
        r.inc = (uint64_t) word | ((uint64_t) (rp.pass_index * rp.spp + (lane - pixel * rp.spp)) << 32);
    } else r.inc = ((uint64_t) word << 1) | 1u;
    r.ld_prepare(); return r;
}
template <bool LD> DEV uint32_t lane_rng_word(const SamplerT<LD> &r) { return LD ? (uint32_t) r.inc : (uint32_t) (r.inc >> 1); }
DEV uint64_t lane_local_index(RpRef rp, uint32_t lane) {
    if (!rp.pixel_slot) return lane;
    const uint32_t pixel = (rp.log2_spp != 0xffffffffu) ? (lane >> rp.log2_spp) : (lane / rp.spp);
    return (uint64_t) rp.pixel_slot[pixel] * rp.spp + (lane - pixel * rp.spp);
}
DEV uint32_t slot_to_lane(RpRef rp, const uint32_t *__restrict__ pixel_list, uint64_t j) {
    if (!pixel_list) return (uint32_t) j;
    const uint32_t pj = (rp.log2_spp != 0xffffffffu) ? (uint32_t) (j >> rp.log2_spp) : (uint32_t) (j / rp.spp);
    return pixel_list[pj] * rp.spp + (uint32_t) (j - (uint64_t) pj * rp.spp);
}
template <bool LD>
DEV SamplerT<LD> lane_rng_pass_start(RpRef rp, uint32_t lane, uint64_t j) {
    SamplerT<LD> r = lane_rng_fresh<LD>(rp, lane);
    if (!LD && rp.pass_index > 0) r.state = rp.pass_in[j];
    return r;
}
DEV void lane_jitter(RpRef rp, uint32_t lane, uint64_t j, float &jx, float &jy) {
    if (rp.ld_count) { SamplerT<true> r = lane_rng_pass_start<true>(rp, lane, j); r.next2(jx, jy); }
    else { SamplerT<false> r = lane_rng_pass_start<false>(rp, lane, j); r.next2(jx, jy); }
}

DEV void lane_to_pixel(SceneRef sc, RpRef rp, uint32_t lane, int *px, int *py) {
    uint32_t idx = (rp.log2_spp != 0xffffffffu) ? (lane >> rp.log2_spp) : (lane / rp.spp);
    uint32_t W = (uint32_t) sc.film.width;
    uint32_t y = idx / W, x = idx - y * W;
    *px = (int) x + sc.film.crop_offset_x; *py = (int) y + sc.film.crop_offset_y;
}

DEV Ray camera_ray(SceneRef sc, float ax, float ay) {
    const LRT_CONST float *m = sc.cam.s2c;
    V3 p(ax + sc.cam.ppo_x, ay + sc.cam.ppo_y, 0.f);
    float r[4];
#pragma unroll
    for (int i = 0; i < 4; ++i) r[i] = fma_(m[4 * i + 2], p.z, fma_(m[4 * i + 1], p.y, fma_(m[4 * i + 0], p.x, m[4 * i + 3])));
    V3 near_p(r[0] / r[3], r[1] / r[3], r[2] / r[3]);
    V3 d = normalize(near_p);
    Ray ray;
    ray.o = V3(sc.cam.to_world[3], sc.cam.to_world[7], sc.cam.to_world[11]);
    ray.d = xform_vec12(sc.cam.to_world, d);
    float inv_z = rcp(d.z), near_t = sc.cam.near_clip * inv_z, far_t = sc.cam.far_clip * inv_z;
    ray.o = ray.o + ray.d * near_t;
    ray.maxt = far_t - near_t;
    return ray;
}

template <bool LD>
DEV PathState generate_camera_path(SceneRef sc, RpRef rp, const uint32_t *__restrict__ pixel_list, uint64_t j) {
    uint32_t lane;
    if (pixel_list) { uint32_t pj = (rp.log2_spp != 0xffffffffu) ? (uint32_t) (j >> rp.log2_spp) : (uint32_t) (j / rp.spp); lane = pixel_list[pj] * rp.spp + (uint32_t) (j - (uint64_t) pj * rp.spp); }
    else lane = (uint32_t) j;
    SamplerT<LD> rng = lane_rng_pass_start<LD>(rp, lane, j);
    int px, py; lane_to_pixel(sc, rp, lane, &px, &py);
    float jx, jy; rng.next2(jx, jy);
    float spx = (float) px + jx, spy = (float) py + jy;
    Ray ray = camera_ray(sc, fma_(spx, sc.film.scale_x, sc.film.offset_x), fma_(spy, sc.film.scale_y, sc.film.offset_y));
    PathState s;
    s.o = ray.o; s.d = ray.d; s.maxt = ray.maxt; s.eta = 1.f; s.tp = V3(1.f); s.res = V3(0.f); s.lp = V3(0.f); s.last_pdf = 1.f; s.lane = lane;
    s.tdepth = 0.f; s.si_t = kInf; s.ff_t = u2f(0x7fc00000u); s.bio_dist = u2f(0x7fc00000u); s.bio_hep = false; s.hit = make_float4(0.f, 0.f, 0.f, 0.f);
    for (int a = 0; a < 2; ++a) for (int i = 0; i < 3; ++i) for (int j = 0; j < 3; ++j) s.W[a][i][j] = 1.f;
    bool env_visible = !rp.hide_emitters && sc.env.type >= 0;
    uint32_t flags = env_visible ? PF_VALID : 0u;
    if (rp.integrator == LRT_INTEGRATOR_PATH) flags |= PF_SPECULAR;
    else {
        if (!rp.hide_emitters) flags |= PF_SPECULAR;
        uint32_t channel = min((uint32_t) (rng.next() * 3.f), 2u);
        flags |= channel << PF_CHANNEL_SHIFT;
        flags |= (uint32_t) (sc.cam.medium + 1) << PF_MEDIUM_SHIFT;
        if (rp.integrator == LRT_INTEGRATOR_BIOVOLPATH06) flags |= PF_BIO_EMIT | PF_BIO_FULL;
    }
    s.flags = flags; s.rng_state = rng.state; s.rng_word = lane_rng_word<LD>(rng);
    return s;
}

#include "film.h"

template <bool HET, typename SMP, typename TR, typename CNT>
DEV V3 volpath_sample_emitter(SceneRef sc, SMP &rng, V3 ref_p, V3 ref_n, bool ref_is_surface, uint32_t ref_shape, V3 ref_geo_n,
                              int medium, uint32_t channel, DirSample *ds_out, const TR &tr, CNT &n_shadow) {
    V3 transmittance(1.f);
    float sx, sy; rng.next2(sx, sy);
    DirSample ds; V3 emitter_val = sample_emitter_direction<TR::kExt>(sc, ref_p, sx, sy, &ds);
    *ds_out = ds;
    if (ds.pdf == 0.f) return V3(0.f);
    Ray ray = spawn_ray_to(ref_p, ref_n, ds.p);
    float max_dist = ray.maxt;
    if (ref_is_surface) { const DShape sd = tab(sc.shapes, ref_shape, sc.one_shape); if (is_medium_transition(sd)) medium = target_medium(sd, ray.d, ref_geo_n); }
    float total_dist = 0.f;
    SI si; si.valid = false; si.t = 0.f; si.shape = 0; si.p = V3(0.f); si.n = V3(0.f);
    bool needs_intersection = true, active = true;
    while (active) {
        float remaining_dist = max_dist - total_dist;
        ray.maxt = remaining_dist;
        if (!(remaining_dist > 0.f)) { rng.skip(1); break; }
        bool escaped_medium = false, active_medium = medium >= 0, active_surface = !active_medium;
        if (!active_medium) rng.skip(1);
        if (active_medium) {
            const DMedium M = tab(sc.media, medium);
            const bool het = HET && M.het;
            MI mei = het ? het_sample_interaction(M, tab(sc.het, medium), ray, rng.next()) : medium_sample_interaction(M, ray, rng.next(), channel);
            if (mei.valid() && !het) ray.maxt = fmin_(mei.t, remaining_dist);
            if (needs_intersection) {
                bool elide = mei.valid() && !sc.has_null_bsdf && !het;
                if (!elide) { n_shadow++; Hit h = tr.closest(ray); si = tr.surface(sc, ray, h); }
                else { si.valid = false; si.t = kInf; }
            }
            if (si.t < mei.t) mei.t = kInf;
            needs_intersection = false;
            bool spectral = M.has_spectral_extinction;
            if (spectral) {
                float t = fmin_(remaining_dist, fmin_(mei.t, si.t)) - mei.mint;
                V3 tr = exp_neg(t, mei.combined);
                V3 ffp = (si.t < mei.t || mei.t > remaining_dist) ? tr : tr * mei.combined;
                float tr_pdf = idx3(ffp, channel);
                transmittance = transmittance * ((tr_pdf > 0.f) ? div_uniform(tr, tr_pdf) : V3(0.f));
            }
            if ((mei.t > remaining_dist) && mei.valid()) total_dist = ds.dist;
            if (mei.t > remaining_dist) mei.t = kInf;
            escaped_medium = !mei.valid();
            active_medium = mei.valid();
            if (active_medium) {
                total_dist += mei.t;
                ray.o = mei.p;
                si.t = si.t - mei.t;
                if (spectral) transmittance = transmittance * mei.sigma_n;
                else transmittance = transmittance * (mei.sigma_n / mei.combined);
            }
        }
        bool intersect = active_surface && needs_intersection;
        if (intersect) { n_shadow++; Hit h = tr.closest(ray); si = tr.surface(sc, ray, h); needs_intersection = false; }
        active_surface = active_surface || escaped_medium;
        if (active_surface) total_dist += si.t;
        active_surface = active_surface && si.valid && !active_medium;
        if (active_surface) {
            transmittance = transmittance * bsdf_null_transmission(sc, tab(sc.shapes, si.shape, sc.one_shape).bsdf);
            ray = spawn_ray(si.p, si.n, ray.d);
        }
        ray.maxt = remaining_dist;
        needs_intersection = needs_intersection || active_surface;
        active = (active_medium || active_surface) && any_nonzero(transmittance);
        if (active_surface) { const DShape sd = tab(sc.shapes, si.shape, sc.one_shape); if (is_medium_transition(sd)) medium = target_medium(sd, ray.d, si.n); }
    }
    return transmittance * emitter_val;
}

struct WaveCount {
    unsigned long long *c;
    DEV void operator++(int) {
        const unsigned long long m = __ballot(true);
        if ((threadIdx.x & 63u) == (uint32_t) (__ffsll((long long) m) - 1)) atomicAdd(c, (unsigned long long) __popcll(m));
    }
};

template <bool HET, bool CLOSED = false, typename SMP, typename TR, typename CNT>
DEV bool volpath_iteration(SceneRef sc, RpRef rp, PathState &s, SMP &rng, const TR &tr, CNT &n_shadow, CNT &n_extra, bool fresh = false, StampClock *clk = nullptr,
                           unsigned long long *guard = nullptr) {
    constexpr bool PRE = !HET;
    uint32_t depth = s.flags & PF_DEPTH_MASK;
    bool proven_empty = (s.flags & PF_NOHIT) != 0;
    float ff_t = s.ff_t;
    const bool needs_intersection = !(HET && (s.flags & PF_HAVE_SI));
    bool act_null_scatter = false;
    Hit hkeep; hkeep.t = s.hit.x; hkeep.u = s.hit.y; hkeep.v = s.hit.z; hkeep.prim = f2u(s.hit.w);
    if (PRE) { hkeep.t = kInf; hkeep.u = hkeep.v = 0.f; hkeep.prim = 0xffffffffu; }
    int medium = (int) ((s.flags & PF_MEDIUM_MASK) >> PF_MEDIUM_SHIFT) - 1;
    const uint32_t channel = (s.flags >> PF_CHANNEL_SHIFT) & 3u;
    bool specular_chain = (s.flags & PF_SPECULAR) != 0, valid_ray = (s.flags & PF_VALID) != 0;
    const uint32_t max_depth = (uint32_t) rp.max_depth;
    V3 throughput = s.tp, result = CLOSED ? V3(0.f) : s.res;
    bool broken = false;
    float eta = s.eta;
    Ray ray; ray.o = s.o; ray.d = s.d; ray.maxt = s.maxt;
    auto commit = [&]() {
        s.tp = throughput; s.res = result; s.eta = eta; s.o = ray.o; s.d = ray.d; s.maxt = ray.maxt;
        s.flags = (depth & PF_DEPTH_MASK) | ((uint32_t) (medium + 1) << PF_MEDIUM_SHIFT) | (channel << PF_CHANNEL_SHIFT) |
                  (specular_chain ? PF_SPECULAR : 0u) | (valid_ray ? PF_VALID : 0u);
    };
    auto termination_stage = [&]() -> bool {
        bool a = any_nonzero(throughput);
        const float q = fmin_(max3(throughput) * sqr(eta), .95f);
        const bool perform_rr = depth > (uint32_t) rp.rr_depth;
        if (a) { const float u = rng.next(); a = (u < q) || !perform_rr; }
        if (perform_rr) throughput = throughput * rcp(q);
        return a && depth < max_depth;
    };
    uint32_t nohit = 0;
    float cache_t = u2f(0x7fc00000u);
    float cone_free = 0.f;
    auto free_flight_stage = [&]() {
        if (medium < 0) return;
        const DMedium M = tab(sc.media, medium);
        cache_t = medium_sampled_t(M, rng.next(), channel);
        if (sc.grid.enabled) {
            const MI m2 = medium_interaction_at(M, ray, cache_t);
            if (m2.valid() && (CLOSED ? segment_free_of_surfaces_from(sc.grid, ray.o, ray.d, m2.t, cone_free) : segment_free_of_surfaces(sc.grid, ray.o, ray.d, m2.t))) nohit = PF_NOHIT;
        }
    };
    bool active = true;
    if (!PRE) active = termination_stage();
    else if (fresh) { active = termination_stage(); if (active && !CLOSED) { free_flight_stage(); ff_t = cache_t; proven_empty = nohit != 0; nohit = 0; cache_t = u2f(0x7fc00000u); } }
    if (!active) { commit(); return false; }

    bool active_medium = medium >= 0, active_surface = !active_medium;
    bool act_medium_scatter = false, escaped_medium = false;
    MI mei; mei.t = kInf;
    SI si; si.valid = false; si.t = kInf;
    if (!active_medium) rng.skip(2);
    if (active_medium) {
        const DMedium M = tab(sc.media, medium);
// ... 41 lines not shown
            else throughput = throughput * (mei.sigma_s / mei.sigma_t);
        } else if (M.has_spectral_extinction) throughput = throughput * V3(M.w_spec[0], M.w_spec[1], M.w_spec[2]);
        else throughput = throughput * V3(M.w_plain[0], M.w_plain[1], M.w_plain[2]);
        bool sample_emitters = M.sample_emitters != 0;
        valid_ray = true;
        specular_chain = !sample_emitters;
        if (!sample_emitters) rng.skip(1);
        if (sample_emitters) {
            bool rejected = false;
            if (sc.nee_fast_reject) {
                SMP saved = rng;
                float sx, sy; rng.next2(sx, sy);
                float u3 = rng.next();
                const float lo = 9.5367431640625e-7f, hi = 1.f - 9.5367431640625e-7f;
                bool interior = sc.env.type == LRT_EMITTER_CONSTANT || (sx > lo && sx < hi && sy > lo && sy < hi);
                rejected = interior;
                if (!(1.f - u3 >= idx3(V3(M.nee_vmin[0], M.nee_vmin[1], M.nee_vmin[2]), channel))) {
                    float sampled_t = 0.f + (-m_log(1.f - u3) / idx3(V3(M.sigma_t[0], M.sigma_t[1], M.sigma_t[2]), channel));
                    V3 cc(sc.env.bsphere_c[0], sc.env.bsphere_c[1], sc.env.bsphere_c[2]);
                    float dist = 2.f * fmax_(sc.env.bsphere_r, norm(mei.p - cc));
                    rejected = interior && sampled_t <= dist * 0.998f - 1e-3f;
                }
                if (!rejected) rng = saved;
            }
            if (!rejected && CLOSED) {
                float sx, sy; rng.next2(sx, sy);
                DirSample ds; (void) sample_emitter_direction<TR::kExt>(sc, mei.p, sx, sy, &ds);
                if (ds.pdf != 0.f) {
                    const Ray r2 = spawn_ray_to(mei.p, V3(0.f), ds.p);
                    if (!(r2.maxt > 0.f)) rng.skip(1);
                    else { const MI m2 = medium_sample_interaction(M, r2, rng.next(), channel); if (!m2.valid()) n_shadow++; }
                }
            } else if (!rejected) {
                DirSample ds;
                V3 emitted = volpath_sample_emitter<HET>(sc, rng, mei.p, V3(0.f), false, 0, V3(0.f), medium, channel, &ds, tr, n_shadow);
                float phase_val = phase_eval<TR::kExt>(sc, M, mei.wi, ds.d);
                V3 c = throughput * phase_val * emitted * mis_weight(ds.pdf, ds.delta ? 0.f : phase_val);
                result = result + c;
            }
        }
        const float s1 = rng.next();
        float s2x, s2y; rng.next2(s2x, s2y);
        V3 wo; float phase_pdf, phase_weight; phase_sample<TR::kExt>(sc, M, mei.wi, s1, s2x, s2y, &wo, &phase_pdf, &phase_weight);
        if (phase_pdf > 0.f) {
            if (TR::kExt) throughput = throughput * phase_weight;
            ray = spawn_ray(mei.p, V3(0.f), wo);
            s.last_pdf = phase_pdf;
        }
    }
    active_surface = active_surface || escaped_medium;
    bool intersect = active_surface && !escaped_medium;
    if (PRE) {
        Hit h = hkeep;
        if (intersect) h = tr.closest(ray);
        if (active_surface) si = tr.surface(sc, ray, h);
    } else if (intersect) { Hit h = tr.closest(ray); si = tr.surface(sc, ray, h); }
    if (active_surface) {
        if (!CLOSED && rp.hide_emitters && depth == 0 && intersect) {
            bool skip = si.valid && tab(sc.shapes, si.shape, sc.one_shape).emitter >= 0;
            if (skip) {
                Ray r2 = spawn_ray(si.p, si.n, ray.d);
                bool a = true; Hit h; h.prim = 0xffffffffu; h.t = kInf; h.u = h.v = 0.f;
                while (a) {
                    h = tr.closest(r2);
                    a = hit_on_emitter(tr, sc, h);
                    if (a) { SI s2 = surface_of(tr, sc, r2, h); r2 = spawn_ray(s2.p, s2.n, r2.d); }
                }
                si = surface_of(tr, sc, r2, h);
            }
        }
        bool count_direct = (depth == 0) || specular_chain;
        int emitter = CLOSED ? (si.valid ? -1 : sc.env.emitter) : si_emitter(sc, si);
        bool active_e = emitter >= 0 && !(depth == 0 && rp.hide_emitters);
        if (active_e) {
            if (CLOSED) { broken = broken || !count_direct; result = result + throughput * emitter_eval_env(sc, -si.wi); }
            else {
                float emitter_pdf = 1.f;
                if (!count_direct) emitter_pdf = pdf_emitter_direction<TR::kExt>(sc, s.lp, si, emitter);
                V3 emitted = emitter_eval(sc, emitter, si);
                V3 contrib = count_direct ? throughput * emitted : throughput * mis_weight(s.last_pdf, emitter_pdf) * emitted;
                result = result + contrib;
            }
        }
    }
    active_surface = active_surface && si.valid;
    if (!active_surface) rng.skip(3);
    if (active_surface) {
        uint4 cone_rows = make_uint4(0u, 0u, 0u, 0u);
        if (CLOSED && sc.cone_enabled) cone_rows = *reinterpret_cast<const uint4 *>(sc.cone_tab + 2u * (size_t) si.prim);
        const DShape sd = tab(sc.shapes, si.shape, sc.one_shape);
        int b = sd.bsdf;
        int flags = tab(sc.bsdfs, b, sc.one_shape).flags;
        bool active_e = !CLOSED && (flags & F_SMOOTH) && (depth + 1 < max_depth);
        if (!active_e) rng.skip(1);
        if (active_e) {
            DirSample ds;
            V3 emitted = volpath_sample_emitter<HET>(sc, rng, si.p, si.n, true, si.shape, si.n, medium, channel, &ds, tr, n_shadow);
            V3 wo = si.sh.to_local(ds.d);
            V3 bsdf_val = bsdf_eval<TR::kExt>(sc, b, si, wo);
            float bpdf = bsdf_pdf<TR::kExt>(sc, b, si, wo);
            V3 c = throughput * bsdf_val * mis_weight(ds.pdf, ds.delta ? 0.f : bpdf) * emitted;
            result = result + c;
        }
        float s1 = rng.next(), s2x, s2y; rng.next2(s2x, s2y);
        const BSDFSample bs = bsdf_sample<CLOSED, TR::kExt>(sc, b, si, s1, s2x, s2y);
        throughput = throughput * bs.weight;
        eta *= bs.eta;
// ... 153 lines not shown
    }
    if (clk) clk->at(6);
    if (rp.pass_out && had_path && !alive) rp.pass_out[lane_local_index(rp, s.lane)] = s.rng_state;
    finish_paths_wave(sc, rp, film, sample_out, sample_base, had_path && !alive, s.lane, s.res, (s.flags & PF_VALID) != 0);
}

template <int INTEGRATOR, int BLOCK, bool LDS_BVH, bool LD, bool COMPACT = false, bool EXT = false>
__global__ void __launch_bounds__(BLOCK, BLOCK == 512 ? 2 : (BLOCK == 768 ? 3 : 4))
k_render(ScenePtr scp, LaunchPtr lp) {
    SceneRef sc = *scp;
    const LRT_CONST DLaunch &A = *lp;
    RpRef rp = A.rp;
    const LRT_CONST DLdsInfo &li = A.li;
    const uint32_t P = A.P;
    extern __shared__ __align__(16) unsigned char smem[];
    __shared__ uint32_t s_in[4], s_out[4], s_ticket, s_fresh;
    __shared__ unsigned long long s_fresh_base, s_prof[8];
#ifdef LRT_STAMP
    __shared__ unsigned long long s_stamp[16];
    if (threadIdx.x < 16) s_stamp[threadIdx.x] = 0;
#endif
    const uint32_t tid = threadIdx.x, lane_in_wave = tid & 63u;
    constexpr bool READLANE = INTEGRATOR != LRT_INTEGRATOR_PATH && INTEGRATOR != LRT_INTEGRATOR_BIOVOLPATH06;
    constexpr bool LONGQ = INTEGRATOR == LRT_INTEGRATOR_BIOVOLPATH;
    constexpr bool CLOSED = INTEGRATOR == LRT_INTEGRATOR_VOLPATH_CLOSED;
    constexpr RecordLayout LAYOUT = record_layout(INTEGRATOR);
    if (tid < 8) s_prof[tid] = 0;
    const unsigned long long t_wg_start = (rp.profile & 1u) ? wall_clock64() : 0ull;
    unsigned long long t_loop_start = 0ull, t_barrier = 0ull;
    LdsScene L{};
    if (LDS_BVH) {
        const uint4 *src = li.blob; uint4 *dst = reinterpret_cast<uint4 *>(smem);
        for (uint32_t k = tid; k < li.blob_bytes / 16u; k += BLOCK) dst[k] = src[k];
        L.nodes = reinterpret_cast<const float4 *>(smem + li.nodes_off); L.verts = reinterpret_cast<const float4 *>(smem + li.verts_off);
        L.tris = reinterpret_cast<const uint2 *>(smem + li.tris_off);
        L.n_faces = sc.n_faces; L.root_is_leaf = (uint32_t) sc.root_is_leaf; L.root_first = sc.root_leaf_first; L.root_count = sc.root_leaf_count;
    }
    const LdsTracer<BLOCK> tr_lds_tri{ L, reinterpret_cast<uint16_t *>(smem + li.stack_off) + tid };
    const GlobalTracer tr_glb_tri{ sc, reinterpret_cast<int *>(smem) + tid };
    const ExtTracer<LdsTracer<BLOCK>> tr_lds_ext{ tr_lds_tri, sc };
    const ExtTracer<GlobalTracer> tr_glb_ext{ tr_glb_tri, sc };
    const auto &tr_lds = pick<EXT>(tr_lds_tri, tr_lds_ext);
    const auto &tr_glb = pick<EXT>(tr_glb_tri, tr_glb_ext);
    const size_t pool = (size_t) blockIdx.x * 2u * P;
    uint32_t parity = 0;
    if (tid == 0) { s_in[0] = s_in[1] = s_in[2] = 0; if (LONGQ) s_in[3] = 0; }
    bool lanes_left = true;
    constexpr bool VP_LDS_COUNT = INTEGRATOR == LRT_INTEGRATOR_VOLPATH || CLOSED;
    __shared__ unsigned long long s_cnt[2];
    if (VP_LDS_COUNT && tid < 2) s_cnt[tid] = 0;
    WaveCount wc_shadow{ &s_cnt[0] }, wc_extra{ &s_cnt[1] };
    uint32_t n_shadow = 0, n_extra = 0, n_trips = 0, n_loaded = 0;
    uint32_t n_proven = 0;
    if (rp.profile & 1u) t_loop_start = wall_clock64();
    for (;;) {
        if (tid == 0) {
            const uint32_t want = P - (s_in[0] + s_in[1] + s_in[2] + (LONGQ ? s_in[3] : 0u));
            uint32_t got = 0; unsigned long long base = 0;
            if (want && lanes_left) {
                base = atomicAdd(&A.cnt->next_lane, (unsigned long long) want);
                if (base < rp.n_lanes) got = (uint32_t) (rp.n_lanes - base < (unsigned long long) want ? rp.n_lanes - base : (unsigned long long) want);
                lanes_left = base + want < rp.n_lanes;
            }
            s_fresh = got; s_fresh_base = base; s_ticket = 0; s_out[0] = s_out[1] = s_out[2] = 0; if (LONGQ) s_out[3] = 0;
        }
        __syncthreads();
        const uint32_t n_a = s_in[0], n_c = s_in[1], n_b = s_in[2], n_l = LONGQ ? s_in[3] : 0u, fresh = s_fresh;
        const unsigned long long fresh_base = s_fresh_base;
        if (n_a + n_c + n_b + n_l + fresh == 0) break;
        const uint32_t ta = (n_a + 63u) >> 6, tc = (n_c + 63u) >> 6, tb = (n_b + 63u) >> 6, tf = (fresh + 63u) >> 6;
        const uint32_t tcl = tc + (LONGQ ? (n_l + 63u) >> 6 : 0u);
        const uint32_t n_tiles = ta + tcl + tb + tf;
        for (;;) {
            uint32_t t = 0;
            if (lane_in_wave == 0) t = atomicAdd(&s_ticket, 1u);
            t = (uint32_t) __builtin_amdgcn_readfirstlane((int) t);
            if (t >= n_tiles) break;
            const unsigned long long t_begin = (rp.profile & 1u) ? wall_clock64() : 0ull;
#ifdef LRT_STAMP
            StampClock clk; clk.start(s_stamp, LRT_STAMP_KIND == 0 ? t < ta : (LRT_STAMP_KIND == 1 ? (t >= ta && t < ta + tcl) : (LRT_STAMP_KIND == 2 ? (t >= ta + tcl && t < ta + tcl + tb) : t >= ta + tcl + tb)));
#endif
            bool had_path = false, alive = false;
            PathState s; s.flags = 0; s.lane = 0; s.res = V3(0.f);
            if (t < ta + tcl + tb) {
                uint32_t i;
                if (t < ta) { i = (t << 6) + lane_in_wave; had_path = i < n_a; }
                else if (t < ta + tc) { i = ((t - ta) << 6) + lane_in_wave; had_path = i < n_c; i += P; }
                else if (LONGQ && t < ta + tcl) { i = ((t - ta - tc) << 6) + lane_in_wave; had_path = i < n_l; i = P - 1u - i; }
                else { i = ((t - ta - tcl) << 6) + lane_in_wave; had_path = i < n_b; i = 2u * P - 1u - i; }
                if (had_path) { load_state<LAYOUT, COMPACT>(parity ? A.q1 : A.q0, pool + i, s); if (!VP_LDS_COUNT) n_loaded += 1; }
            } else {
                const uint32_t i = ((t - ta - tcl - tb) << 6) + lane_in_wave;
                had_path = i < fresh;
                if (had_path) s = generate_camera_path<LD>(sc, rp, A.pixel_list, A.lane_begin + fresh_base + i);
            }
            if (VP_LDS_COUNT) {
                const uint32_t n_had = (uint32_t) __popcll(__ballot(had_path));
                n_trips += n_had;
                if (t < ta + tcl + tb) n_loaded += n_had;
                if (CLOSED && t < ta) n_proven += n_had;
            }
#ifdef LRT_STAMP
            clk.at(0);
#endif
            if (had_path) {
                SamplerT<LD> rng = COMPACT ? lane_rng_resume_word<LD>(rp, s.lane, s.rng_state, s.rng_word) : lane_rng_resume<LD>(rp, s.lane, s.rng_state);
#ifdef LRT_STAMP
                clk.at(1);
#endif
                if (INTEGRATOR == LRT_INTEGRATOR_PATH) alive = LDS_BVH ? path_iteration(sc, rp, s, rng, tr_lds, n_shadow) : path_iteration(sc, rp, s, rng, tr_glb, n_shadow);
                else if (INTEGRATOR == LRT_INTEGRATOR_BIOVOLPATH) { const bool fresh_tile = t >= ta + tcl + tb; alive = LDS_BVH ? biovolpath_iteration(sc, rp, s, rng, tr_lds, n_shadow, n_extra, fresh_tile) : biovolpath_iteration(sc, rp, s, rng, tr_glb, n_shadow, n_extra, fresh_tile); }
                else if (INTEGRATOR == LRT_INTEGRATOR_BIOVOLPATH06) alive = LDS_BVH ? biovolpath06_iteration(sc, rp, s, rng, tr_lds) : biovolpath06_iteration(sc, rp, s, rng, tr_glb);
                else if (INTEGRATOR == LRT_INTEGRATOR_VOLPATHMIS) alive = LDS_BVH ? volpathmis_iteration<true>(sc, rp, s, rng, tr_lds, n_shadow) : volpathmis_iteration<true>(sc, rp, s, rng, tr_glb, n_shadow);
                else if (INTEGRATOR == LRT_INTEGRATOR_VOLPATHMIS_PLAIN) alive = LDS_BVH ? volpathmis_iteration<false>(sc, rp, s, rng, tr_lds, n_shadow) : volpathmis_iteration<false>(sc, rp, s, rng, tr_glb, n_shadow);
                else if (INTEGRATOR == LRT_INTEGRATOR_VOLPATH_HET) alive = LDS_BVH ? volpath_iteration<true>(sc, rp, s, rng, tr_lds, n_shadow, n_extra) : volpath_iteration<true>(sc, rp, s, rng, tr_glb, n_shadow, n_extra);
                else {
                    const bool fresh_tile = t >= ta + tcl + tb;
#ifdef LRT_STAMP
                    StampClock *const pclk = &clk;
#else
                    StampClock *const pclk = nullptr;
#endif
                    unsigned long long *const guard = CLOSED ? &A.cnt->n_closed_guard : nullptr;
                    alive = LDS_BVH ? volpath_iteration<false, CLOSED>(sc, rp, s, rng, tr_lds, wc_shadow, wc_extra, fresh_tile, pclk, guard) : volpath_iteration<false, CLOSED>(sc, rp, s, rng, tr_glb, wc_shadow, wc_extra, fresh_tile, pclk, guard);
                }
                s.rng_state = rng.state;
                if (!VP_LDS_COUNT) n_trips += 1;
            }
#ifdef LRT_STAMP
            retire_and_compact_wave<LAYOUT, READLANE, COMPACT, LONGQ>(sc, rp, had_path, alive, s, A.film, A.sample_out, A.sample_base, parity ? A.q0 : A.q1, pool, P, s_out, &clk);
            clk.at(7);
            if (clk.on && lane_in_wave == 0) atomicAdd(&s_stamp[15], 1ull);
#else
            retire_and_compact_wave<LAYOUT, READLANE, COMPACT, LONGQ>(sc, rp, had_path, alive, s, A.film, A.sample_out, A.sample_base, parity ? A.q0 : A.q1, pool, P, s_out);
#endif
            if ((rp.profile & 1u) && lane_in_wave == 0) {
                const int region = t < ta ? 0 : (t < ta + tcl ? 1 : (t < ta + tcl + tb ? 2 : 3));
                atomicAdd(&s_prof[region], wall_clock64() - t_begin); atomicAdd(&s_prof[4 + region], 1ull);
            }
        }
        { const unsigned long long tb0 = (rp.profile & 1u) ? wall_clock64() : 0ull;
        __syncthreads();
        if (rp.profile & 1u) t_barrier += wall_clock64() - tb0; }
        if (tid == 0) { s_in[0] = s_out[0]; s_in[1] = s_out[1]; s_in[2] = s_out[2]; if (LONGQ) s_in[3] = s_out[3]; }
        parity ^= 1u;
    }
    if ((rp.profile & 1u) && (tid & 63u) == 0) {
        const unsigned long long t_end = wall_clock64();
        if (tid == 0) { atomicAdd(&A.cnt->prof_wg[0], t_loop_start - t_wg_start); atomicMax(&A.cnt->prof_wg[1], t_end); atomicMax(&A.cnt->prof_wg[2], ~t_wg_start); atomicAdd(&A.cnt->prof_wg[3], t_end - t_wg_start); atomicMax(&A.cnt->prof_wg[5], t_wg_start); }
        atomicAdd(&A.cnt->prof_wg[4], t_barrier);
    }
    if ((rp.profile & 1u) && tid < 8) { if (tid < 4) atomicAdd(&A.cnt->prof_cycles[tid], s_prof[tid]); else atomicAdd(&A.cnt->prof_tiles[tid - 4], s_prof[tid]); }
#ifdef LRT_TRAV_STATS
    if (tid == 0 && blockIdx.x == 0) printf("[trav, so far] closest: node steps %llu (lanes %.1f), leaf steps %llu (lanes %.1f); any-hit: node steps %llu (lanes %.1f), leaf steps %llu (lanes %.1f)\n", g_trav[0], (double) g_trav[1] / g_trav[0], g_trav[2], (double) g_trav[3] / g_trav[2], g_trav[4], (double) g_trav[5] / g_trav[4], g_trav[6], (double) g_trav[7] / g_trav[6]);
#endif
#ifdef LRT_STAMP
    __syncthreads();
    if (tid == 0 && blockIdx.x == 7) printf("[stamp] tiles of kind %d in workgroup 7: %llu; cycles per tile: ticket+load issue %.0f, record wait+TEA %.0f, to the end of the medium interaction / ray query %.0f, scatter + surface %.0f, termination+free flight %.0f, ballots+slots %.0f, stores %.0f, film %.0f\n", LRT_STAMP_KIND, s_stamp[15],
        (double) s_stamp[0] / s_stamp[15], (double) s_stamp[1] / s_stamp[15], (double) s_stamp[2] / s_stamp[15], (double) s_stamp[3] / s_stamp[15], (double) s_stamp[4] / s_stamp[15], (double) s_stamp[5] / s_stamp[15], (double) s_stamp[6] / s_stamp[15], (double) s_stamp[7] / s_stamp[15]);
#endif
    if (!VP_LDS_COUNT) {
        n_trips += n_extra;
        for (int off = 32; off > 0; off >>= 1) {
            n_shadow += __shfl_down(n_shadow, off); n_trips += __shfl_down(n_trips, off); n_loaded += __shfl_down(n_loaded, off);
        }
    }
    if (lane_in_wave == 0) {
        if (!VP_LDS_COUNT && n_shadow) atomicAdd(&A.cnt->n_shadow, (unsigned long long) n_shadow);
        if (n_trips) atomicAdd(&A.cnt->n_iter, (unsigned long long) n_trips);
        if (n_loaded) atomicAdd(&A.cnt->n_records, (unsigned long long) n_loaded);
        if (CLOSED && n_proven) atomicAdd(&A.cnt->n_proven, (unsigned long long) n_proven);
    }
    if (VP_LDS_COUNT) {
        __syncthreads();
        if (tid == 0) {
            if (s_cnt[0]) atomicAdd(&A.cnt->n_shadow, s_cnt[0]);
            if (s_cnt[1]) atomicAdd(&A.cnt->n_iter, s_cnt[1]);
        }
    }
}

DEV float point_triangle_dist2(V3 p, V3 a, V3 ab, V3 ac) {
    V3 ap = p - a;
    float d1 = dot(ab, ap), d2 = dot(ac, ap);
    if (d1 <= 0.f && d2 <= 0.f) return dot(ap, ap);
    V3 bp = ap - ab;
    float d3 = dot(ab, bp), d4 = dot(ac, bp);
    if (d3 >= 0.f && d4 <= d3) return dot(bp, bp);
    float vc = d1 * d4 - d3 * d2;
    if (vc <= 0.f && d1 >= 0.f && d3 <= 0.f) { V3 r = ap - ab * (d1 / (d1 - d3)); return dot(r, r); }
    V3 cp = ap - ac;
    float d5 = dot(ab, cp), d6 = dot(ac, cp);
    if (d6 >= 0.f && d5 <= d6) return dot(cp, cp);
    float vb = d5 * d2 - d1 * d6;
    if (vb <= 0.f && d2 >= 0.f && d6 <= 0.f) { V3 r = ap - ac * (d2 / (d2 - d6)); return dot(r, r); }
    float va = d3 * d6 - d5 * d4;
    if (va <= 0.f && (d4 - d3) >= 0.f && (d5 - d6) >= 0.f) { V3 r = bp - (ac - ab) * ((d4 - d3) / ((d4 - d3) + (d5 - d6))); return dot(r, r); }
    float denom = 1.f / (va + vb + vc);
    V3 r = ap - ab * (vb * denom) - ac * (vc * denom);
    return dot(r, r);
}

__global__ void __launch_bounds__(LRT_BLOCK)
k_build_dist_grid(const float4 *__restrict__ tris, uint32_t n_slots, DDistGrid g, uint16_t *__restrict__ out, float abs_margin,
                  const DSphere *__restrict__ spheres, uint32_t n_spheres) {
    const size_t n_cells = (size_t) g.n[0] * g.n[1] * g.n[2];
    const size_t c = (size_t) blockIdx.x * LRT_BLOCK + threadIdx.x;
    if (c >= n_cells) return;
    const int ix = (int) (c % g.n[0]), iy = (int) ((c / g.n[0]) % g.n[1]), iz = (int) (c / ((size_t) g.n[0] * g.n[1]));
    const V3 p(g.lo[0] + ((float) ix + .5f) * g.cell, g.lo[1] + ((float) iy + .5f) * g.cell, g.lo[2] + ((float) iz + .5f) * g.cell);
    float best = kInf;
    for (uint32_t sl = 0; sl < n_slots; ++sl) {
        const float4 a = tris[3 * sl], b = tris[3 * sl + 1], cc = tris[3 * sl + 2];
        float d2 = point_triangle_dist2(p, V3(a.x, a.y, a.z), V3(b.x, b.y, b.z), V3(cc.x, cc.y, cc.z));
        if (!(d2 >= 0.f)) d2 = 0.f;
        best = fmin_(best, d2);
    }
    for (uint32_t k = 0; k < n_spheres; ++k) {
        const DSphere &S = spheres[k];
        const float ds = __builtin_fabsf(norm(p - V3(S.center[0], S.center[1], S.center[2])) - S.radius);
        best = fmin_(best, ds * ds);
    }
    float d = __builtin_sqrtf(best) * .999f - abs_margin;
    d = d > 0.f ? fmin_(d, 60000.f) : 0.f;
// ... 121 lines not shown
```

liverrenderer_amd/csrc/scene_prep.cpp:

```cpp
#include "scene_prep.h"
#include "scene_check.h"
#include <functional>
#include <cmath>
#include <cstring>
#include <cstdlib>
#include <algorithm>
#include <stdexcept>
#include <string>

namespace lrt {

PrepOptions PrepOptions::from_env() {
    PrepOptions o;
    if (getenv("LRT_BVH_LEAF")) o.bvh_leaf = std::max(1, atoi(getenv("LRT_BVH_LEAF")));
    o.no_lds_bvh = getenv("LRT_NO_LDS_BVH") != nullptr;
    o.no_dist_grid = getenv("LRT_NO_DIST_GRID") != nullptr;
    if (getenv("LRT_DIST_GRID_RES")) o.dist_grid_res = std::max(8, std::min(256, atoi(getenv("LRT_DIST_GRID_RES"))));
    o.no_nee_reject = getenv("LRT_NO_NEE_REJECT") != nullptr;
    o.no_cone_proof = getenv("LRT_NO_CONE_PROOF") != nullptr;
    return o;
}

static void m4_mul(const float *a, const float *b, float *r) {
    for (int i = 0; i < 4; ++i) for (int j = 0; j < 4; ++j) { float s = a[4 * i] * b[j]; for (int k = 1; k < 4; ++k) s = fmaf(a[4 * i + k], b[4 * k + j], s); r[4 * i + j] = s; }
}
static void m4_ident(float *m) { for (int i = 0; i < 16; ++i) m[i] = (i % 5 == 0) ? 1.f : 0.f; }

static void build_camera(const lrt_scene_desc &d, DCamera &cam, DFilm &film) {
    const lrt_film_desc &F = d.film; const lrt_sensor_desc &C = d.sensor;
    float fw = (float) F.width, fh = (float) F.height;
    float rsx = (float) F.crop_width / fw, rsy = (float) F.crop_height / fh, rox = (float) F.crop_offset_x / fw, roy = (float) F.crop_offset_y / fh;
    float aspect = fw / fh, recip = 1.f / (C.far_clip - C.near_clip);
    float tn = (float) tan((double) (C.fov_x * .5f) * (3.14159265358979323846 / 180.0));
    (void) recip;
    float S1i[16], T1i[16], S2i[16], T2i[16], Pit[16], t0[16], t1[16], t2[16], it[16];
    m4_ident(S1i); S1i[0] = 1.f / (1.f / rsx); S1i[5] = 1.f / (1.f / rsy); S1i[10] = 1.f / 1.f;
    m4_ident(T1i); T1i[12] = rox; T1i[13] = roy; T1i[14] = -0.f;
    m4_ident(S2i); S2i[0] = 1.f / -0.5f; S2i[5] = 1.f / (-0.5f * aspect); S2i[10] = 1.f;
    m4_ident(T2i); T2i[12] = 1.f; T2i[13] = 1.f / aspect; T2i[14] = -0.f;
    float Pinv[16]; m4_ident(Pinv); Pinv[0] = tn; Pinv[5] = tn; Pinv[10] = 0.f; Pinv[15] = 1.f / C.near_clip; Pinv[11] = 1.f;
    Pinv[14] = (C.near_clip - C.far_clip) / (C.far_clip * C.near_clip);
    for (int i = 0; i < 4; ++i) for (int j = 0; j < 4; ++j) Pit[4 * i + j] = Pinv[4 * j + i];
    m4_mul(S1i, T1i, t0); m4_mul(t0, S2i, t1); m4_mul(t1, T2i, t2); m4_mul(t2, Pit, it);
    for (int i = 0; i < 4; ++i) for (int j = 0; j < 4; ++j) cam.s2c[4 * i + j] = it[4 * j + i];
    memcpy(cam.to_world, C.to_world, sizeof(float) * 12);
    cam.near_clip = C.near_clip; cam.far_clip = C.far_clip; cam.medium = C.medium;
    cam.ppo_x = fw * C.principal_point_offset_x / (float) F.crop_width; cam.ppo_y = fh * C.principal_point_offset_y / (float) F.crop_height;

    film.width = F.crop_width; film.height = F.crop_height; film.crop_offset_x = F.crop_offset_x; film.crop_offset_y = F.crop_offset_y;
    film.scale_x = 1.f / (float) F.crop_width; film.scale_y = 1.f / (float) F.crop_height;
    film.offset_x = -(float) F.crop_offset_x * film.scale_x; film.offset_y = -(float) F.crop_offset_y * film.scale_y;
    film.has_alpha = F.has_alpha; film.channels = F.has_alpha ? 5 : 4; film.rfilter = F.rfilter;
    film.rf_radius = 0.5f; film.rf_inv_radius = 1.f;
    if (F.rfilter == LRT_RFILTER_GAUSSIAN) {
        float stddev = F.rfilter_param; film.rf_radius = 4.f * stddev;
        static const double coeff[10] = { 9.992604880e-1, -4.977025247e-1, 1.222248550e-1, -1.932406282e-2, 2.136713061e-3,
                                          -1.679873860e-4, 9.202145248e-6, -3.329417433e-7, 7.128382794e-9, -6.821193280e-11 };
        double sc = 1; for (int i = 0; i < 10; ++i) { film.rf_coeff[i] = (float) (coeff[i] * sc); sc /= (double) stddev * (double) stddev; }
        float x = film.rf_radius * film.rf_radius, x2 = x * x, x4 = x2 * x2, x8 = x4 * x4; const float *c = film.rf_coeff;
        float a0 = fmaf(x, c[1], c[0]), a1 = fmaf(x, c[3], c[2]), a2 = fmaf(x, c[5], c[4]), a3 = fmaf(x, c[7], c[6]), a4 = fmaf(x, c[9], c[8]);
        float b0 = fmaf(x2, a1, a0), b1 = fmaf(x2, a3, a2), c0 = fmaf(x4, b1, b0);
        film.rf_coeff[0] -= fmaf(x8, a4, c0);
    } else if (F.rfilter == LRT_RFILTER_TENT) { film.rf_radius = F.rfilter_param; film.rf_inv_radius = 1.f / film.rf_radius; }
    film.fn = (int) ceilf(film.rf_radius - .5f); film.fcount = 2 * film.fn + 1;
}

static void inverse3(const float *m16, float *out9) {
    double m[3][3]; for (int i = 0; i < 3; ++i) for (int j = 0; j < 3; ++j) m[i][j] = m16[4 * i + j];
    double det = m[0][0] * (m[1][1] * m[2][2] - m[1][2] * m[2][1]) - m[0][1] * (m[1][0] * m[2][2] - m[1][2] * m[2][0]) + m[0][2] * (m[1][0] * m[2][1] - m[1][1] * m[2][0]);
    double id = 1.0 / det;
    out9[0] = (float) ((m[1][1] * m[2][2] - m[1][2] * m[2][1]) * id); out9[1] = (float) ((m[0][2] * m[2][1] - m[0][1] * m[2][2]) * id); out9[2] = (float) ((m[0][1] * m[1][2] - m[0][2] * m[1][1]) * id);
    out9[3] = (float) ((m[1][2] * m[2][0] - m[1][0] * m[2][2]) * id); out9[4] = (float) ((m[0][0] * m[2][2] - m[0][2] * m[2][0]) * id); out9[5] = (float) ((m[0][2] * m[1][0] - m[0][0] * m[1][2]) * id);
    out9[6] = (float) ((m[1][0] * m[2][1] - m[1][1] * m[2][0]) * id); out9[7] = (float) ((m[0][1] * m[2][0] - m[0][0] * m[2][1]) * id); out9[8] = (float) ((m[0][0] * m[1][1] - m[0][1] * m[1][0]) * id);
}

static uint32_t log2i_ceil(uint32_t v) { uint32_t r = 0; while ((1u << r) < v) ++r; return r; }

static void build_hierarchy(const std::vector<float> &lum, uint32_t w, uint32_t h, DEnv &E, std::vector<float> &out) {
    uint32_t npx = w - 1, npy = h - 1;
    E.patch_size[0] = 1.f / (float) npx; E.patch_size[1] = 1.f / (float) npy;
    E.inv_patch_size[0] = (float) npx; E.inv_patch_size[1] = (float) npy;
// ... 186 lines not shown
            int match[3], ns = 0;
            for (int j = 0; j < 3; ++j) { match[j] = -1; for (int i = 0; i < 3; ++i) if (G.c[j] == T.c[i]) match[j] = i; ns += match[j] >= 0; }
            if (ns == 3 || (ns > 0 && G.dup)) { for (int s = 0; s < 2; ++s) for (int k = 0; k < K; ++k) R[s][k] = 0.0; dead = true; break; }
            for (int s = 0; s < 2; ++s) {
                const D3 hn = nu[s]; const double h_off = dot3(hn, T.v[0]);
                if (ns == 2) {
                    int jw = 0, seen = 0; for (int j = 0; j < 3; ++j) { if (match[j] < 0) jw = j; else seen |= 1 << match[j]; }
                    const int opp = seen == 3 ? 2 : (seen == 6 ? 0 : 1), e = (opp + 1) % 3;
                    const D3 w = G.v[jw]; const double hw = dot3(hn, w) - h_off, lat = dot3(w - T.v[e], ne[s][e]), slack = 1e-9 * (1.0 + len3(w - T.v[e]));
                    for (int k = 0; k < K; ++k) if (hw >= -slack && lat - hw * tan_k[k] <= slack) R[s][k] = 0.0;
                } else if (ns == 1) {
                    int iv = 0, jv = 0; for (int j = 0; j < 3; ++j) if (match[j] >= 0) { iv = match[j]; jv = j; }
                    const D3 v = T.v[iv], w1 = G.v[(jv + 1) % 3], w2 = G.v[(jv + 2) % 3];
                    const int ea = iv, eb = (iv + 2) % 3;
                    const double slack = 1e-9 * (1.0 + std::max(len3(w1 - v), len3(w2 - v)));
                    const double h1 = dot3(hn, w1 - v), h2 = dot3(hn, w2 - v);
                    for (int k = 0; k < K; ++k) {
                        const double c1[3] = { -h1, dot3(w1 - v, ne[s][ea]) - h1 * tan_k[k], dot3(w1 - v, ne[s][eb]) - h1 * tan_k[k] };
                        const double c2[3] = { -h2, dot3(w2 - v, ne[s][ea]) - h2 * tan_k[k], dot3(w2 - v, ne[s][eb]) - h2 * tan_k[k] };
                        double t0 = 0.0, t1 = 1.0;
                        for (int c = 0; c < 3; ++c) {
                            const double u0 = c1[c] - slack, du = c2[c] - c1[c];
                            if (du == 0.0) { if (u0 > 0.0) t1 = -1.0; }
                            else if (du > 0.0) t1 = std::min(t1, -u0 / du);
                            else t0 = std::max(t0, -u0 / du);
                        }
                        if (t0 <= t1) R[s][k] = 0.0;
                    }
                } else {
                    if (dist2 > (base[s] + G.rad) * (base[s] + G.rad)) continue;
                    const double hc = dot3(hn, G.cen) - h_off;
                    if (hc + G.rad < -tau) continue;
                    double lat[3]; for (int e = 0; e < 3; ++e) lat[e] = dot3(G.cen - T.v[e], ne[s][e]);
                    for (int k = K - 1; k >= 0; --k) {
                        if (!(R[s][k] > 0.0) || hc - G.rad - h_o_max - tau >= R[s][k]) continue;
                        const double tp = tau * (1.0 + tan_k[k]);
                        bool outside = false;
                        for (int e = 0; e < 3; ++e) outside = outside || lat[e] - hc * tan_k[k] - G.rad * inv_cos_k[k] > tp;
                        if (outside) break;
                        ConePlane pl[4]; pl[0] = { hn * -1.0, tau - h_off };
                        for (int e = 0; e < 3; ++e) { const D3 n = ne[s][e] - hn * tan_k[k]; pl[1 + e] = { n, tp + dot3(T.v[e], ne[s][e]) - h_off * tan_k[k] }; }
                        double hmin;
                        if (!clip_min_height(G.v, pl, hn, hmin)) break;
                        R[s][k] = std::max(0.0, std::min(R[s][k], hmin - h_off - h_o_max - tau));
                    }
                }
            }
        }
        }
        for (int s = 0; s < 2; ++s) for (int k = 0; k < K; ++k) out[((size_t) 2 * f + s) * K + k] = half_round_down(R[s][k]);
    }
}

static float fresnel_diffuse_reflectance(float eta) {
    const float inv_eta = 1.f / eta;
    const float approx_1 = fmaf(0.0636f, inv_eta, fmaf(eta, fmaf(eta, -1.4399f, 0.7099f), 0.6681f));
    float approx_2 = -1.36881f;
    for (float c : { 4.98554f, -7.80989f, 6.75335f, -3.4793f, 0.919317f }) approx_2 = fmaf(approx_2, inv_eta, c);
    return eta < 1.f ? approx_1 : approx_2;
}
PlasticConstants plastic_constants(float eta, float d_mean, float s_mean) {
    PlasticConstants c;
    c.inv_eta_2 = 1.f / (eta * eta);
    c.fdr_int = fresnel_diffuse_reflectance(1.f / eta);
    c.fdr_ext = fresnel_diffuse_reflectance(eta);
    c.specular_sampling_weight = s_mean / (d_mean + s_mean);
    return c;
}
float texture_mean(const lrt_texture_desc &T) {
    auto mean3 = [](const float *c) { return (c[0] + c[1] + c[2]) * (1.f / 3.f); };
    if (T.type == LRT_TEX_CHECKERBOARD) return .5f * (mean3(T.color0) + mean3(T.color1));
    return mean3(T.color0);
}
void prepare_geometry(const lrt_scene_desc &d, const PrepOptions &opt, PreparedScene &P) {
    DScene &sc = P.sc;
    memset(&sc, 0, sizeof(sc));
    std::vector<DSphere> &spheres = P.spheres;
    for (uint32_t i = 0; i < d.n_shapes; ++i) {
        const lrt_shape_desc &s = d.shapes[i];
        if (s.kind != LRT_SHAPE_SPHERE) continue;
        DSphere o; memset(&o, 0, sizeof(o));
        const float *m = s.to_world;
        for (int a = 0; a < 3; ++a) o.center[a] = m[4 * a + 3];
        o.radius = sqrtf(fmaf(m[8], m[8], fmaf(m[4], m[4], m[0] * m[0])));
        for (int a = 0; a < 3; ++a) for (int b = 0; b < 3; ++b) o.to_world[3 * a + b] = m[4 * a + b];
        double md[16]; for (int k = 0; k < 16; ++k) md[k] = m[k];
        const double c00 = md[5] * md[10] - md[6] * md[9], c01 = md[6] * md[8] - md[4] * md[10], c02 = md[4] * md[9] - md[5] * md[8];
        const double id = 1.0 / (md[0] * c00 + md[1] * c01 + md[2] * c02);
        double inv[12] = { c00 * id, (md[2] * md[9] - md[1] * md[10]) * id, (md[1] * md[6] - md[2] * md[5]) * id, 0,
                           c01 * id, (md[0] * md[10] - md[2] * md[8]) * id, (md[2] * md[4] - md[0] * md[6]) * id, 0,
                           c02 * id, (md[1] * md[8] - md[0] * md[9]) * id, (md[0] * md[5] - md[1] * md[4]) * id, 0 };
        for (int a = 0; a < 3; ++a) inv[4 * a + 3] = -(inv[4 * a] * md[3] + inv[4 * a + 1] * md[7] + inv[4 * a + 2] * md[11]);
        for (int k = 0; k < 12; ++k) o.to_object[k] = (float) inv[k];
        o.shape = i; o.flip_normals = s.flip_normals;
        check_sphere_radius(o.radius);
        spheres.push_back(o);
    }
    sc.n_spheres = (uint32_t) spheres.size();
    const SceneFeatures features = scene_features(d);
    P.ext = features.any(); P.smooth_bsdf = features.smooth_bsdf;
    HostBVH &bvh = P.bvh;
    {
        const int forced = opt.bvh_leaf;
        int chosen = forced ? forced : 4;
        bool done = false;
        if (!forced && lds_possible(d, opt)) {
            for (int leaf : { 2, 3, 4, 6, 8, 12, 16 }) {
                HostBVH b2; build_bvh(d.positions, d.faces, d.n_faces, b2, leaf);
                if (lds_image_fits(d, b2, opt)) { bvh = std::move(b2); chosen = leaf; done = true; break; }
            }
        }
        if (!done) build_bvh(d.positions, d.faces, d.n_faces, bvh, chosen);
        P.bvh_leaf = chosen;
    }
    sc.root_is_leaf = bvh.root_is_leaf; sc.root_leaf_first = bvh.root_first; sc.root_leaf_count = bvh.root_count;
    sc.n_faces = d.n_faces; sc.n_emitters = d.n_emitters; sc.one_shape = d.n_shapes == 1;
    if (lds_image_fits(d, bvh, opt)) { build_lds_image(d, bvh, P); P.use_lds = true; }
    sc.grid = DDistGrid{};
    if (d.n_media > 0 && (d.n_faces > 0 || !spheres.empty()) && d.n_faces <= (1u << 17) && !opt.no_dist_grid) {
        float lo[3], hi[3]; referenced_bounds(d, spheres, lo, hi);
        const float ext = std::max(hi[0] - lo[0], std::max(hi[1] - lo[1], hi[2] - lo[2]));
        const int res = opt.dist_grid_res ? opt.dist_grid_res : (d.n_faces <= (1u << 14) ? 192 : 64);
        if (ext > 0.f && std::isfinite(ext)) {
            DDistGrid g{};
            g.cell = ext / (float) res; g.inv_cell = 1.f / g.cell;
            for (int a = 0; a < 3; ++a) { g.lo[a] = lo[a]; g.n[a] = std::max(1, std::min(res, (int) std::ceil((hi[a] - lo[a]) / g.cell))); }
            float diag = std::sqrt((hi[0] - lo[0]) * (hi[0] - lo[0]) + (hi[1] - lo[1]) * (hi[1] - lo[1]) + (hi[2] - lo[2]) * (hi[2] - lo[2]));
            float amax = 0.f; for (int a = 0; a < 3; ++a) amax = std::max(amax, std::max(std::fabs(lo[a]), std::fabs(hi[a])));
            P.grid_abs_margin = 1e-4f * diag + 1e-5f * amax;
            g.enabled = 1; sc.grid = g;
        }
    }
    if (P.use_lds && !P.ext && sc.grid.enabled && !opt.no_cone_proof && closed_records(d, d.sensor.medium)) { build_cone_table(d, P.cone_tab); sc.cone_enabled = 1; }
}

void prepare_shading(const lrt_scene_desc &d, const PrepOptions &opt, PreparedScene &P) {
    DScene &sc = P.sc; const std::vector<DSphere> &spheres = P.spheres;
    {
        P.vattr.assign(8 * (size_t) d.n_vertices, 0.f); std::vector<float> &va = P.vattr;
        for (size_t v = 0; v < d.n_vertices; ++v) {
            if (d.normals) for (int a = 0; a < 3; ++a) va[8 * v + a] = d.normals[3 * v + a];
            if (d.texcoords) for (int a = 0; a < 2; ++a) va[8 * v + 4 + a] = d.texcoords[2 * v + a];
        }
    }
    std::vector<DShape> &shapes = P.shapes; shapes.resize(d.n_shapes);
    for (uint32_t i = 0; i < d.n_shapes; ++i) { const lrt_shape_desc &s = d.shapes[i]; shapes[i] = { s.bsdf, s.emitter, s.interior_medium, s.exterior_medium, s.has_normals, s.has_texcoords, s.flip_normals, s.kind }; }
    std::vector<DTexture> &tex = P.textures; tex.resize(d.n_textures); std::vector<float> &tex_data = P.tex_data;
    for (uint32_t i = 0; i < d.n_textures; ++i) {
        const lrt_texture_desc &T = d.textures[i]; DTexture &o = tex[i]; memset(&o, 0, sizeof(o));
        o.type = T.type; o.width = T.width; o.height = T.height; o.channels = T.channels;
        for (int k = 0; k < 3; ++k) { o.color0[k] = T.color0[k]; o.color1[k] = T.color1[k]; }
        for (int k = 0; k < 6; ++k) o.to_uv[k] = T.to_uv[k];
        if (T.type == LRT_TEX_BITMAP) {
            o.data_offset = (uint32_t) tex_data.size();
            size_t np = (size_t) T.width * T.height;
            for (size_t p = 0; p < np; ++p) {
                const float *px = T.data + p * T.channels;
                tex_data.push_back(T.channels == 1 ? px[0] : px[0] * 0.212671f + px[1] * 0.715160f + px[2] * 0.072169f);
            }
        }
    }
    std::vector<DBsdf> &bsdfs = P.bsdfs; bsdfs.resize(d.n_bsdfs); sc.has_null_bsdf = 0;
    std::function<int(uint32_t)> leaf_flags = [&](uint32_t b) -> int {
        const lrt_bsdf_desc &B = d.bsdfs[b];
        if (B.type == LRT_BSDF_TWOSIDED) { const int32_t back = B.nested_back < 0 ? B.nested : B.nested_back; return leaf_flags((uint32_t) B.nested) | leaf_flags((uint32_t) back); }
        return (B.type == LRT_BSDF_DIFFUSE || B.type == LRT_BSDF_ROUGHDIELECTRIC) ? PREP_F_SMOOTH : (B.type == LRT_BSDF_DIELECTRIC || B.type == LRT_BSDF_CONDUCTOR) ? PREP_F_DELTA
             : B.type == LRT_BSDF_PLASTIC ? (PREP_F_DELTA | PREP_F_SMOOTH) : PREP_F_NULL;
    };
    bool any_smooth_bsdf = false;
    for (uint32_t i = 0; i < d.n_bsdfs; ++i) if (d.bsdfs[i].type == LRT_BSDF_CONDUCTOR || d.bsdfs[i].type == LRT_BSDF_PLASTIC || d.bsdfs[i].type == LRT_BSDF_TWOSIDED) { check_smooth_bsdf(d, i); any_smooth_bsdf = true; }
    if (any_smooth_bsdf) P.bsdf_ext.assign(d.n_bsdfs, DBsdfExt{});
    for (uint32_t i = 0; i < d.n_bsdfs; ++i) {
        const lrt_bsdf_desc &B = d.bsdfs[i];
        DBsdf &o = bsdfs[i]; memset(&o, 0, sizeof(o));
        o.type = B.type; o.reflectance = B.reflectance; o.nested = B.nested; o.texture = B.texture; o.eta = B.eta; o.scale = B.scale;
        bsdfs[i].flags = leaf_flags(B.type == LRT_BSDF_BUMPMAP ? (uint32_t) B.nested : i);
        if (B.type == LRT_BSDF_NULL) sc.has_null_bsdf = 1;
        if (B.type == LRT_BSDF_ROUGHDIELECTRIC) {
            bsdfs[i].specular_reflectance = B.specular_reflectance; bsdfs[i].specular_transmittance = B.specular_transmittance;
            bsdfs[i].alpha_u = std::max(B.alpha_u, 1e-4f); bsdfs[i].alpha_v = std::max(B.alpha_v, 1e-4f);
            bsdfs[i].micro = (B.distribution == 1 ? LRT_MICRO_GGX : 0) | (B.sample_visible ? LRT_MICRO_VISIBLE : 0);
        }
        if (B.type == LRT_BSDF_CONDUCTOR) {
            DBsdfExt &x = P.bsdf_ext[i];
            o.specular_reflectance = B.specular_reflectance;
            for (int k = 0; k < 3; ++k) { x.eta[k] = B.eta_rgb[k]; x.k[k] = B.k_rgb[k]; }
// ... 267 lines not shown
```

liverrenderer_amd/csrc/scene_prep.h:

```cpp
#pragma once
#include "device_types.h"
#include "bvh.h"
#include "host_scene.h"
#include <utility>

namespace lrt {

struct PrepOptions {
    int bvh_leaf = 0;
    bool no_lds_bvh = false;
    bool no_dist_grid = false;
    int dist_grid_res = 0;
    bool no_nee_reject = false;
    bool no_cone_proof = false;
    size_t lds_limit = 0;
    int n_cus = 256;
    static PrepOptions from_env();
};

enum { PREP_F_DELTA = 1, PREP_F_SMOOTH = 2, PREP_F_NULL = 4 };

struct PreparedScene {
    std::vector<DSphere> spheres;
    HostBVH bvh;
    std::vector<unsigned char> lds_blob; DLdsInfo lds{};
    std::vector<float> vattr;
    std::vector<DShape> shapes;
    std::vector<DTexture> textures; std::vector<float> tex_data;
    std::vector<DBsdf> bsdfs;
    std::vector<DBsdfExt> bsdf_ext;
    std::vector<DEmitter> emitters;
    std::vector<DMeshEmitter> mesh_emitters; std::vector<float> mesh_emitter_tab;
    std::vector<DDeltaEmitter> delta_emitters;
    std::vector<float> env_data, env_hier;
    DScene sc{};
    float grid_abs_margin = 0.f;
    std::vector<DPhase> phases; std::vector<float> phase_pool;
    std::vector<uint16_t> cone_tab;
    bool env_interior_positive = false;
    bool ext = false, has_area_emitter = false, has_het = false, has_non_bio = false, prb_null = false, use_lds = false;
    bool smooth_bsdf = false;
    int bvh_leaf = 4;
};
void prepare_geometry(const lrt_scene_desc &d, const PrepOptions &opt, PreparedScene &P);
void prepare_shading(const lrt_scene_desc &d, const PrepOptions &opt, PreparedScene &P);
PreparedScene prepare_scene(const lrt_scene_desc &d, const PrepOptions &opt);

void build_cone_table(const lrt_scene_desc &d, std::vector<uint16_t> &out);
float cone_table_value(uint16_t h);

size_t lds_image_bytes(const HostBVH &b, uint32_t n_vertices);
bool lds_image_fits(const lrt_scene_desc &d, const HostBVH &b, const PrepOptions &opt);

inline float medium_sigma_t(const lrt_medium_desc &M, int k) { return M.sigma_t[k] * M.scale; }
void prepare_media(const lrt_scene_desc &d, float bsphere_r, std::vector<DMedium> &media, std::vector<DBioMedium> &bio, std::vector<DHetMedium> &het);

struct PhaseTable { std::vector<float> cdf; float interval_size = 0.f, inv_interval_size = 0.f, integral = 0.f, normalization = 0.f; uint32_t valid_x = 0, valid_y = 0; };
void phase_table(const float *values, size_t n, PhaseTable &out);
inline bool medium_has_phase_entry(const lrt_scene_desc &d, uint32_t m) { return d.n_phases > 0 && d.media[m].phase_index >= 0; }
void prepare_phases(const lrt_scene_desc &d, std::vector<DPhase> &phases, std::vector<float> &pool);

struct PlasticConstants { float inv_eta_2, fdr_int, fdr_ext, specular_sampling_weight; };
PlasticConstants plastic_constants(float eta, float d_mean, float s_mean);
float texture_mean(const lrt_texture_desc &T);

struct ResolvedOpts { int integrator, max_depth, rr_depth, hide_emitters; uint32_t spp, seed, tile_rank, tile_count; uint32_t spp_total = 0, n_passes = 1, pass = 0; };
ResolvedOpts resolve(const lrt_scene_desc &d, const lrt_render_opts *o);

struct TilePixels { std::vector<uint32_t> list, slot; };
TilePixels tile_pixel_list(const DFilm &film, uint32_t rank, uint32_t count);
std::vector<uint32_t> halo_pixel_list(const DFilm &film, uint32_t rank, uint32_t count, uint32_t halo);

bool closed_records(const lrt_scene_desc &d, int sensor_medium);

}
```

Measured before the change: 6497 Msamples/s.

## Start primary-ray BVH traversal from a per-pixel precomputed entry node

Precomputes on the host, for each pixel, the lowest BVH node (or a none marker) that must contain any primary-ray hit. It does this by rasterising projected triangles with a conservative margin and culling occluded candidates by depth. In the closed-record LDS path, camera rays start LDS traversal from that node instead of the root, or skip traversal entirely when no triangle can be hit. This is meant to cut the top-level node visits of first-bounce rays, at the cost of a per-pixel table lookup, extra host prep time, and correctness risk if the conservative bounds are wrong.

```diff
diff --git a/include/liverrt.h b/include/liverrt.h
--- a/include/liverrt.h
+++ b/include/liverrt.h
@@ -205,6 +205,7 @@
     uint64_t record_bytes;
     uint64_t n_closed_guard;
     uint64_t n_proven;
+    uint64_t n_primary_entry;
 } lrt_render_stats;
 
 typedef struct {
@@ -230,6 +231,8 @@
 LRT_API lrt_status lrt_render(lrt_scene *scene, const lrt_render_opts *opts,
                               float *film_raw, float *image);
 LRT_API lrt_status lrt_render_stats_get(const lrt_scene *scene, lrt_render_stats *out);
+LRT_API lrt_status lrt_primary_entry_get(lrt_scene *scene, uint16_t *out, uint64_t n_pixels, int device);
+
 LRT_API lrt_status lrt_film_develop(lrt_scene *scene, const float *film_raw, float *image,
                                     int on_device);
 
diff --git a/liverrenderer_amd/__init__.py b/liverrenderer_amd/__init__.py
--- a/liverrenderer_amd/__init__.py
+++ b/liverrenderer_amd/__init__.py
@@ -415,6 +415,12 @@
         return {"sigma_t": np.array(out.d_sigma_t[:], dtype=np.float32), "albedo": np.array(out.d_albedo[:], dtype=np.float32),
                 "g": float(out.d_g), "sigma_t_data": res}
 
+    def primary_entry(self, device=0):
+        h, w, _ = self.film_shape()
+        out = np.zeros((h, w), dtype=np.uint16)
+        _lib.check(self._lib.lrt_primary_entry_get(self._h, out.ctypes.data, h * w, device))
+        return out
+
     def stats(self):
         s = _lib.RenderStats()
         _lib.check(self._lib.lrt_render_stats_get(self._h, C.byref(s)))
diff --git a/liverrenderer_amd/_lib.py b/liverrenderer_amd/_lib.py
--- a/liverrenderer_amd/_lib.py
+++ b/liverrenderer_amd/_lib.py
@@ -114,7 +114,7 @@
 class RenderStats(C.Structure):
     _fields_ = [("n_samples", C.c_uint64), ("n_iter", C.c_uint64), ("n_shadow", C.c_uint64), ("n_launches", C.c_uint64),
                 ("n_records", C.c_uint64), ("kernel_ms", C.c_double), ("total_ms", C.c_double), ("lds_resident", C.c_uint64),
-                ("record_bytes", C.c_uint64), ("n_closed_guard", C.c_uint64), ("n_proven", C.c_uint64)]
+                ("record_bytes", C.c_uint64), ("n_closed_guard", C.c_uint64), ("n_proven", C.c_uint64), ("n_primary_entry", C.c_uint64)]
 
 
 class ParamGrads(C.Structure):
@@ -195,6 +195,7 @@
     L.lrt_math_eval.argtypes = [C.c_int, P(C.c_float), P(C.c_float), C.c_uint32, P(C.c_float), P(C.c_float), C.c_int]
     L.lrt_render_stats_get.argtypes = [C.c_void_p, P(RenderStats)]
     L.lrt_film_develop.argtypes = [C.c_void_p, C.c_void_p, C.c_void_p, C.c_int]
+    L.lrt_primary_entry_get.argtypes = [C.c_void_p, C.c_void_p, C.c_uint64, C.c_int]
     L.lrt_render_samples.argtypes = [C.c_void_p, P(RenderOpts), C.c_uint64, C.c_uint32, C.c_void_p]
     L.lrt_render_backward.argtypes = [C.c_void_p, P(RenderOpts), C.c_void_p, P(ParamGrads)]
     L.lrt_render_backward_grid.argtypes = [C.c_void_p, P(RenderOpts), C.c_void_p, P(ParamGrads), C.c_void_p]
@@ -248,7 +249,7 @@
                     "lrt_vae_model_create", "lrt_vae_model_free", "lrt_vae_scatter",
                     "lrt_scene_aov_get", "lrt_aov_channel_name", "lrt_render_aov", "lrt_render_aov_samples", "lrt_image_write_exr_channels",
                     "lrt_denoiser_create", "lrt_denoise", "lrt_denoiser_free", "lrt_denoiser_get", "lrt_image_read_named", "lrt_image_free_names",
-                    "lrt_scene_moment_get", "lrt_moment_channel_name", "lrt_render_moment", "lrt_render_moment_samples"]
+                    "lrt_scene_moment_get", "lrt_moment_channel_name", "lrt_render_moment", "lrt_render_moment_samples", "lrt_primary_entry_get"]
 
 
 def bsdf_probe_fields(out):
diff --git a/liverrenderer_amd/csrc/capi.cpp b/liverrenderer_amd/csrc/capi.cpp
--- a/liverrenderer_amd/csrc/capi.cpp
+++ b/liverrenderer_amd/csrc/capi.cpp
@@ -29,7 +29,7 @@
 extern "C" {
 
 const char *lrt_last_error(void) { return g_error.c_str(); }
-int lrt_version(void) { return 120; }
+int lrt_version(void) { return 121; }
 
 static std::vector<std::pair<std::string, std::string>> parse_defines(const char *const *defines, int n) {
     std::vector<std::pair<std::string, std::string>> r;
@@ -282,6 +282,18 @@
     LRT_TRY
         ensure_device(scene, -1);
         device_trace(scene->dev, rays, hits, n, any_hit);
+        return LRT_OK;
+    LRT_CATCH
+}
+
+lrt_status lrt_primary_entry_get(lrt_scene *scene, uint16_t *out, uint64_t n_pixels, int device) {
+    if (!scene || (!out && n_pixels)) return fail(LRT_ERR_INVALID, "lrt_primary_entry_get: null argument");
+    LRT_TRY
+        ensure_device(scene, device);
+        const std::vector<uint16_t> &t = device_primary_entry(scene->dev);
+        const uint64_t want = (uint64_t) scene->st.desc.film.crop_width * (uint64_t) scene->st.desc.film.crop_height;
+        if (n_pixels != want) return fail(LRT_ERR_INVALID, "lrt_primary_entry_get: n_pixels is not the crop window's pixel count");
+        for (uint64_t i = 0; i < n_pixels; ++i) out[i] = t.empty() ? (uint16_t) 0 : t[i];
         return LRT_OK;
     LRT_CATCH
 }
diff --git a/liverrenderer_amd/csrc/device.hip b/liverrenderer_amd/csrc/device.hip
--- a/liverrenderer_amd/csrc/device.hip
+++ b/liverrenderer_amd/csrc/device.hip
@@ -55,7 +55,7 @@
 static void add_stats(lrt_render_stats &total, const lrt_render_stats &s) {
     total.n_samples += s.n_samples; total.n_iter += s.n_iter; total.n_shadow += s.n_shadow; total.n_launches += s.n_launches;
     total.n_records += s.n_records; total.kernel_ms += s.kernel_ms; total.total_ms += s.total_ms;
-    total.record_bytes = s.record_bytes; total.n_closed_guard += s.n_closed_guard; total.n_proven += s.n_proven;
+    total.record_bytes = s.record_bytes; total.n_closed_guard += s.n_closed_guard; total.n_proven += s.n_proven; total.n_primary_entry += s.n_primary_entry;
 }
 
 #define LRT_LAUNCH_SLOTS 64
@@ -74,6 +74,7 @@
     double *d_grads = nullptr; float *wfilm = nullptr; size_t wfilm_floats = 0; float *grad_image = nullptr; size_t grad_floats = 0;
     DCounters *counters = nullptr;
     DCounters *h_counters = nullptr;
+    std::vector<uint16_t> primary_tab;
     float *film = nullptr; size_t film_floats = 0;
     float *image = nullptr; size_t image_floats = 0;
     unsigned long long *pass_state[2] = { nullptr, nullptr }; size_t pass_state_lanes[2] = { 0, 0 };
@@ -290,6 +291,8 @@
     sc.delta_emitters = P.delta_emitters.empty() ? nullptr : up(P.delta_emitters);
     sc.bsdf_ext = P.bsdf_ext.empty() ? nullptr : up(P.bsdf_ext);
     sc.cone_tab = P.cone_tab.empty() ? nullptr : (const uint2 *) up(P.cone_tab);
+    sc.primary_tab = P.primary_tab.empty() ? nullptr : (const uint16_t *) up(P.primary_tab);
+    D->primary_tab = P.primary_tab;
     sc.phases = P.phases.empty() ? nullptr : up(P.phases);
     sc.phase_pool = P.phase_pool.empty() ? nullptr : up(P.phase_pool);
     sc.env_data = (const float4 *) up(P.env_data);
@@ -510,6 +513,7 @@
     finish_stats(D, log, e_begin, e_end, n_lanes, stats);
     stats.n_closed_guard = D->h_counters->n_closed_guard;
     stats.n_proven = D->h_counters->n_proven;
+    stats.n_primary_entry = D->h_counters->n_primary_entry;
     if (stats.n_closed_guard)
         throw std::runtime_error("64-byte path records: " + std::to_string(stats.n_closed_guard) + " trips broke the premise of the layout (radiance before a path's last trip, "
                                  "or an emitter hit that needs its MIS weight); the scene test in closed_records() is wrong for this scene: LRT_NO_CLOSED_RECORDS=1 renders it with 80-byte records");
@@ -606,6 +610,8 @@
     HIP_CHECK(hipStreamSynchronize(D->stream));
 }
 
+const std::vector<uint16_t> &device_primary_entry(const DeviceScene *D) { return D->primary_tab; }
+
 void device_develop(DeviceScene *D, const float *film_raw, float *image, int on_device) {
     HIP_CHECK(hipSetDevice(D->device));
     const DFilm &F = D->sc.film;
@@ -971,7 +977,7 @@
     develop_and_download(D0, films[0], film_raw, image, film_floats, image_floats, on_device);
     lrt_render_stats total{};
     for (auto &x : st) { total.n_samples += x.n_samples; total.n_iter += x.n_iter; total.n_shadow += x.n_shadow; total.n_launches += x.n_launches; total.n_records += x.n_records;
-                         total.kernel_ms = std::max(total.kernel_ms, x.kernel_ms); total.lds_resident = x.lds_resident; total.record_bytes = x.record_bytes; total.n_closed_guard += x.n_closed_guard; total.n_proven += x.n_proven; }
+                         total.kernel_ms = std::max(total.kernel_ms, x.kernel_ms); total.lds_resident = x.lds_resident; total.record_bytes = x.record_bytes; total.n_closed_guard += x.n_closed_guard; total.n_proven += x.n_proven; total.n_primary_entry += x.n_primary_entry; }
     total.total_ms = std::chrono::duration<double, std::milli>(std::chrono::steady_clock::now() - t0).count();
     stats = total;
 }
diff --git a/liverrenderer_amd/csrc/device_scene.h b/liverrenderer_amd/csrc/device_scene.h
--- a/liverrenderer_amd/csrc/device_scene.h
+++ b/liverrenderer_amd/csrc/device_scene.h
@@ -16,6 +16,7 @@
 void device_render_moment_samples(DeviceScene *D, const lrt_scene_desc &d, const lrt_render_opts *opts, uint64_t lane_begin, uint32_t n, float *out, lrt_render_stats &stats);
 void device_render_samples(DeviceScene *D, const lrt_scene_desc &d, const lrt_render_opts *opts, uint64_t lane_begin, uint32_t n, float *out, lrt_render_stats &stats);
 void device_trace(DeviceScene *D, const lrt_rays_soa *rays, const lrt_hits_soa *hits, uint32_t n, int any_hit);
+const std::vector<uint16_t> &device_primary_entry(const DeviceScene *D);
 enum ProbeKind { PROBE_EMITTER, PROBE_ENVMAP, PROBE_BSDF, PROBE_PHASE, PROBE_MEDIUM, PROBE_SENSOR, PROBE_KINDS };
 struct ProbeColumn { const float *p; int width; };
 void device_probe(DeviceScene *D, ProbeKind kind, int arg, std::initializer_list<ProbeColumn> columns, uint32_t n, float *out);
diff --git a/liverrenderer_amd/csrc/device_types.h b/liverrenderer_amd/csrc/device_types.h
--- a/liverrenderer_amd/csrc/device_types.h
+++ b/liverrenderer_amd/csrc/device_types.h
@@ -175,11 +175,12 @@
     const DMeshEmitter *mesh_emitters;
     const float *mesh_emitter_tab;
     const uint2 *cone_tab;
-    int32_t cone_enabled, pad_cone;
+    int32_t cone_enabled, primary_enabled;
     const DPhase *phases;
     const float *phase_pool;
     const DDeltaEmitter *delta_emitters;
     const DBsdfExt *bsdf_ext;
+    const uint16_t *primary_tab;
 };
 
 #define LRT_CONE_BINS 4
@@ -252,6 +253,7 @@
     unsigned long long prof_wg[6];
     unsigned long long n_closed_guard;
     unsigned long long n_proven;
+    unsigned long long n_primary_entry;
 };
 
 struct DLdsInfo {
diff --git a/liverrenderer_amd/csrc/dshade.h b/liverrenderer_amd/csrc/dshade.h
--- a/liverrenderer_amd/csrc/dshade.h
+++ b/liverrenderer_amd/csrc/dshade.h
@@ -91,6 +91,7 @@
     static constexpr bool kExt = false;
     SceneRef sc; int *stack;
     DEV Hit closest(const Ray &r) const { return trace<false>(sc, r, stack); }
+    DEV Hit closest_from(const Ray &r, uint32_t) const { return trace<false>(sc, r, stack); }
     DEV Hit any(const Ray &r) const { return trace<true>(sc, r, stack); }
     DEV SI surface(SceneRef s, const Ray &r, const Hit &h) const;
 };
@@ -126,9 +127,10 @@
 #define LRT_TRAV_COUNT(k)
 #endif
 template <bool ANY_HIT, int STRIDE>
-DEV Hit trace_lds(const LdsScene &L, const Ray &r, uint16_t *__restrict__ stack ) {
+DEV Hit trace_lds(const LdsScene &L, const Ray &r, uint16_t *__restrict__ stack , uint32_t start = 0u) {
     Hit best; best.t = kInf; best.u = best.v = 0.f; best.prim = 0xffffffffu;
     if (L.n_faces == 0) return best;
+    if (start == 0xffffu) return best;
     const V3 o = r.o, d = r.d;
     if (L.root_is_leaf) {
         for (uint32_t i = 0; i < L.root_count; ++i) test_tri_lds(L, L.tris[L.root_first + i], L.root_first + i, o, d, r.maxt, best);
@@ -139,7 +141,7 @@
     const float ox = -o.x * ix, oy = -o.y * iy, oz = -o.z * iz;
     const f32x2 vix = { ix, ix }, viy = { iy, iy }, viz = { iz, iz }, vox = { ox, ox }, voy = { oy, oy }, voz = { oz, oz };
     const uint32_t DONE = 0x10000u;
-    int sp = 0; uint32_t cur = 0;
+    int sp = 0; uint32_t cur = start;
     for (;;) {
         while (cur < 0x8000u) {
             LRT_TRAV_COUNT(0)
@@ -186,6 +188,7 @@
     static constexpr bool kExt = false;
     const LdsScene &L; uint16_t *stack;
     DEV Hit closest(const Ray &r) const { return trace_lds<false, STRIDE>(L, r, stack); }
+    DEV Hit closest_from(const Ray &r, uint32_t start) const { return trace_lds<false, STRIDE>(L, r, stack, start); }
     DEV Hit any(const Ray &r) const { return trace_lds<true, STRIDE>(L, r, stack); }
     DEV SI surface(SceneRef s, const Ray &r, const Hit &h) const;
 };
diff --git a/liverrenderer_amd/csrc/kernels.h b/liverrenderer_amd/csrc/kernels.h
--- a/liverrenderer_amd/csrc/kernels.h
+++ b/liverrenderer_amd/csrc/kernels.h
@@ -89,11 +89,12 @@
     return ray;
 }
 
-template <bool LD>
-DEV PathState generate_camera_path(SceneRef sc, RpRef rp, const uint32_t *__restrict__ pixel_list, uint64_t j) {
+template <bool LD, bool ENTRY = false>
+DEV PathState generate_camera_path(SceneRef sc, RpRef rp, const uint32_t *__restrict__ pixel_list, uint64_t j, uint32_t *entry = nullptr) {
     uint32_t lane;
     if (pixel_list) { uint32_t pj = (rp.log2_spp != 0xffffffffu) ? (uint32_t) (j >> rp.log2_spp) : (uint32_t) (j / rp.spp); lane = pixel_list[pj] * rp.spp + (uint32_t) (j - (uint64_t) pj * rp.spp); }
     else lane = (uint32_t) j;
+    if (ENTRY && sc.primary_enabled) *entry = sc.primary_tab[(rp.log2_spp != 0xffffffffu) ? (lane >> rp.log2_spp) : (lane / rp.spp)];
     SamplerT<LD> rng = lane_rng_pass_start<LD>(rp, lane, j);
     int px, py; lane_to_pixel(sc, rp, lane, &px, &py);
     float jx, jy; rng.next2(jx, jy);
@@ -198,7 +199,7 @@
 
 template <bool HET, bool CLOSED = false, typename SMP, typename TR, typename CNT>
 DEV bool volpath_iteration(SceneRef sc, RpRef rp, PathState &s, SMP &rng, const TR &tr, CNT &n_shadow, CNT &n_extra, bool fresh = false, StampClock *clk = nullptr,
-                           unsigned long long *guard = nullptr) {
+                           unsigned long long *guard = nullptr, uint32_t entry = 0u) {
     constexpr bool PRE = !HET;
     uint32_t depth = s.flags & PF_DEPTH_MASK;
     bool proven_empty = (s.flags & PF_NOHIT) != 0;
@@ -346,7 +347,7 @@
     bool intersect = active_surface && !escaped_medium;
     if (PRE) {
         Hit h = hkeep;
-        if (intersect) h = tr.closest(ray);
+        if (intersect) { if constexpr (CLOSED) h = tr.closest_from(ray, entry); else h = tr.closest(ray); }
         if (active_surface) si = tr.surface(sc, ray, h);
     } else if (intersect) { Hit h = tr.closest(ray); si = tr.surface(sc, ray, h); }
     if (active_surface) {
@@ -606,6 +607,7 @@
     WaveCount wc_shadow{ &s_cnt[0] }, wc_extra{ &s_cnt[1] };
     uint32_t n_shadow = 0, n_extra = 0, n_trips = 0, n_loaded = 0;
     uint32_t n_proven = 0;
+    uint32_t n_primary = 0;
     if (rp.profile & 1u) t_loop_start = wall_clock64();
     for (;;) {
         if (tid == 0) {
@@ -636,6 +638,7 @@
 #endif
             bool had_path = false, alive = false;
             PathState s; s.flags = 0; s.lane = 0; s.res = V3(0.f);
+            uint32_t entry = 0u;
             if (t < ta + tcl + tb) {
                 uint32_t i;
                 if (t < ta) { i = (t << 6) + lane_in_wave; had_path = i < n_a; }
@@ -646,7 +649,8 @@
             } else {
                 const uint32_t i = ((t - ta - tcl - tb) << 6) + lane_in_wave;
                 had_path = i < fresh;
-                if (had_path) s = generate_camera_path<LD>(sc, rp, A.pixel_list, A.lane_begin + fresh_base + i);
+                if (had_path) s = generate_camera_path<LD, CLOSED>(sc, rp, A.pixel_list, A.lane_begin + fresh_base + i, &entry);
+                if (CLOSED && sc.primary_enabled) n_primary += (uint32_t) __popcll(__ballot(entry != 0u));
             }
             if (VP_LDS_COUNT) {
                 const uint32_t n_had = (uint32_t) __popcll(__ballot(had_path));
@@ -676,7 +680,7 @@
                     StampClock *const pclk = nullptr;
 #endif
                     unsigned long long *const guard = CLOSED ? &A.cnt->n_closed_guard : nullptr;
-                    alive = LDS_BVH ? volpath_iteration<false, CLOSED>(sc, rp, s, rng, tr_lds, wc_shadow, wc_extra, fresh_tile, pclk, guard) : volpath_iteration<false, CLOSED>(sc, rp, s, rng, tr_glb, wc_shadow, wc_extra, fresh_tile, pclk, guard);
+                    alive = LDS_BVH ? volpath_iteration<false, CLOSED>(sc, rp, s, rng, tr_lds, wc_shadow, wc_extra, fresh_tile, pclk, guard, entry) : volpath_iteration<false, CLOSED>(sc, rp, s, rng, tr_glb, wc_shadow, wc_extra, fresh_tile, pclk, guard, entry);
                 }
                 s.rng_state = rng.state;
                 if (!VP_LDS_COUNT) n_trips += 1;
@@ -724,6 +728,7 @@
         if (n_trips) atomicAdd(&A.cnt->n_iter, (unsigned long long) n_trips);
         if (n_loaded) atomicAdd(&A.cnt->n_records, (unsigned long long) n_loaded);
         if (CLOSED && n_proven) atomicAdd(&A.cnt->n_proven, (unsigned long long) n_proven);
+        if (CLOSED && n_primary) atomicAdd(&A.cnt->n_primary_entry, (unsigned long long) n_primary);
     }
     if (VP_LDS_COUNT) {
         __syncthreads();
diff --git a/liverrenderer_amd/csrc/scene_prep.cpp b/liverrenderer_amd/csrc/scene_prep.cpp
--- a/liverrenderer_amd/csrc/scene_prep.cpp
+++ b/liverrenderer_amd/csrc/scene_prep.cpp
@@ -18,6 +18,7 @@
     if (getenv("LRT_DIST_GRID_RES")) o.dist_grid_res = std::max(8, std::min(256, atoi(getenv("LRT_DIST_GRID_RES"))));
     o.no_nee_reject = getenv("LRT_NO_NEE_REJECT") != nullptr;
     o.no_cone_proof = getenv("LRT_NO_CONE_PROOF") != nullptr;
+    o.no_primary_entry = getenv("LRT_NO_PRIMARY_ENTRY") != nullptr;
     return o;
 }
 
@@ -26,7 +27,7 @@
 }
 static void m4_ident(float *m) { for (int i = 0; i < 16; ++i) m[i] = (i % 5 == 0) ? 1.f : 0.f; }
 
-static void build_camera(const lrt_scene_desc &d, DCamera &cam, DFilm &film) {
+void build_camera(const lrt_scene_desc &d, DCamera &cam, DFilm &film) {
     const lrt_film_desc &F = d.film; const lrt_sensor_desc &C = d.sensor;
     float fw = (float) F.width, fh = (float) F.height;
     float rsx = (float) F.crop_width / fw, rsy = (float) F.crop_height / fh, rox = (float) F.crop_offset_x / fw, roy = (float) F.crop_offset_y / fh;
@@ -319,6 +320,179 @@
     }
 }
 
+namespace {
+struct PeTri {
+    double x[3], y[3];
+    double ex[3], ey[3], ec[3], el[3];
+    double gx, gy, g0;
+    double lox, hix, loy, hiy;
+    bool projected, has_area, plane_ok, occluder;
+};
+void inverse3d(const double m[3][3], double o[3][3], double &det) {
+    det = m[0][0] * (m[1][1] * m[2][2] - m[1][2] * m[2][1]) - m[0][1] * (m[1][0] * m[2][2] - m[1][2] * m[2][0]) + m[0][2] * (m[1][0] * m[2][1] - m[1][1] * m[2][0]);
+    const double id = 1.0 / det;
+    o[0][0] = (m[1][1] * m[2][2] - m[1][2] * m[2][1]) * id; o[0][1] = (m[0][2] * m[2][1] - m[0][1] * m[2][2]) * id; o[0][2] = (m[0][1] * m[1][2] - m[0][2] * m[1][1]) * id;
+    o[1][0] = (m[1][2] * m[2][0] - m[1][0] * m[2][2]) * id; o[1][1] = (m[0][0] * m[2][2] - m[0][2] * m[2][0]) * id; o[1][2] = (m[0][2] * m[1][0] - m[0][0] * m[1][2]) * id;
+    o[2][0] = (m[1][0] * m[2][1] - m[1][1] * m[2][0]) * id; o[2][1] = (m[0][1] * m[2][0] - m[0][0] * m[2][1]) * id; o[2][2] = (m[0][0] * m[1][1] - m[0][1] * m[1][0]) * id;
+}
+struct PeTree {
+    uint32_t n_nodes = 0; std::vector<int32_t> parent; std::vector<uint16_t> depth; std::vector<uint32_t> leaf_first, face_leaf;
+    bool ok = false;
+    explicit PeTree(const HostBVH &b, uint32_t n_faces) {
+        n_nodes = (uint32_t) (b.nodes.size() / 16); const size_t n_slots = b.tris.size() / 12;
+        if (!n_nodes || b.root_is_leaf) return;
+        parent.assign(n_nodes, -2); depth.assign(n_nodes, 0); face_leaf.assign(n_faces, 0xffffffffu);
+        std::vector<uint32_t> todo{ 0u }; parent[0] = -1;
+        while (!todo.empty()) {
+            const uint32_t n = todo.back(); todo.pop_back();
+            int32_t refs[4]; memcpy(refs, &b.nodes[16 * (size_t) n + 12], 16);
+            for (int c = 0; c < 2; ++c) {
+                if (refs[c] >= 0) {
+                    if ((uint32_t) refs[c] >= n_nodes || parent[refs[c]] != -2) return;
+                    parent[refs[c]] = (int32_t) n; depth[refs[c]] = (uint16_t) (depth[n] + 1); todo.push_back((uint32_t) refs[c]);
+                } else {
+                    const uint32_t first = (uint32_t) ~refs[c], count = (uint32_t) refs[2 + c];
+                    if (!count || (size_t) first + count > n_slots) return;
+                    const uint32_t id = n_nodes + (uint32_t) leaf_first.size();
+                    leaf_first.push_back(first); parent.push_back((int32_t) n); depth.push_back((uint16_t) (depth[n] + 1));
+                    for (uint32_t s = first; s < first + count; ++s) { uint32_t f; memcpy(&f, &b.tris[12 * (size_t) s + 3], 4); if (f >= n_faces) return; face_leaf[f] = id; }
+                }
+            }
+        }
+        ok = true;
+    }
+    int32_t lca(int32_t a, int32_t b) const {
+        if (a < 0) return b;
+        if (b < 0) return a;
+        while (a != b) { if (depth[a] >= depth[b]) a = parent[a]; else b = parent[b]; }
+        return a;
+    }
+    uint16_t item(int32_t id) const { return id < 0 ? (uint16_t) LRT_PRIMARY_NONE : ((uint32_t) id >= n_nodes ? (uint16_t) (0x8000u | leaf_first[(uint32_t) id - n_nodes]) : (uint16_t) id); }
+};
+}
+
+bool primary_entry_valid(const HostBVH &bvh, const std::vector<uint16_t> &tab) {
+    const PeTree T(bvh, (uint32_t) (bvh.tris.size() / 12));
+    if (!T.ok || T.n_nodes > 0x8000u) return false;
+    std::vector<char> starts(0x8000u, 0);
+    for (uint32_t f : T.leaf_first) { if (f >= 0x7fffu) return false; starts[f] = 1; }
+    for (uint16_t it : tab) if (it != LRT_PRIMARY_NONE && !(it < 0x8000u ? it < T.n_nodes : starts[it & 0x7fffu])) return false;
+    return true;
+}
+
+void build_primary_entry(const lrt_scene_desc &d, const HostBVH &bvh, std::vector<uint16_t> &out, const PrimaryEntryTune &tune) {
+    out.clear();
+    const uint32_t nf = d.n_faces;
+    if (!nf || bvh.root_is_leaf) return;
+    for (size_t i = 0; i < 3 * (size_t) d.n_vertices; ++i) if (!std::isfinite(d.positions[i])) return;
+    DCamera cam; DFilm film; memset(&cam, 0, sizeof(cam)); memset(&film, 0, sizeof(film)); build_camera(d, cam, film);
+    const int W = film.width, Hh = film.height;
+    if (W <= 0 || Hh <= 0) return;
+    const float *m = cam.s2c;
+    if (m[12] != 0.f || m[13] != 0.f || !(m[15] > 0.f) || !(cam.near_clip > 0.f) || !(cam.far_clip > cam.near_clip)) return;
+    if (!(film.scale_x > 0.f) || !(film.scale_y > 0.f)) return;
+    const double Hm[3][3] = { { m[0], m[1], m[3] }, { m[4], m[5], m[7] }, { m[8], m[9], m[11] } };
+    const double Rm[3][3] = { { cam.to_world[0], cam.to_world[1], cam.to_world[2] }, { cam.to_world[4], cam.to_world[5], cam.to_world[6] }, { cam.to_world[8], cam.to_world[9], cam.to_world[10] } };
+    double Hi[3][3], Ri[3][3], dh, dr; inverse3d(Hm, Hi, dh); inverse3d(Rm, Ri, dr);
+    if (!std::isfinite(1.0 / dh) || !std::isfinite(1.0 / dr)) return;
+    for (int i = 0; i < 12; ++i) if (!std::isfinite(cam.to_world[i])) return;
+    const PeTree tree(bvh, nf);
+    if (!tree.ok) return;
+    for (uint32_t f = 0; f < nf; ++f) if (tree.face_leaf[f] == 0xffffffffu) return;
+    const double eye[3] = { cam.to_world[3], cam.to_world[7], cam.to_world[11] };
+    const double offx = (double) film.offset_x + (double) cam.ppo_x, offy = (double) film.offset_y + (double) cam.ppo_y, isx = 1.0 / (double) film.scale_x, isy = 1.0 / (double) film.scale_y;
+    const double near_lo = (double) cam.near_clip * (1.0 - 1e-3), near_hi = (double) cam.near_clip * (1.0 + 1e-3), far_lo = (double) cam.far_clip * (1.0 - 1e-3);
+    const double delta = tune.delta, half = 0.5 + delta;
+    const int cox = film.crop_offset_x, coy = film.crop_offset_y;
+
+    std::vector<PeTri> T(nf);
+    int32_t everywhere = -1;
+    for (uint32_t f = 0; f < nf; ++f) {
+        PeTri &t = T[f]; t.projected = true; t.has_area = t.plane_ok = t.occluder = false;
+        double w[3], zmin = INFINITY, zmax = -INFINITY;
+        for (int j = 0; j < 3; ++j) {
+            const float *p = &d.positions[3 * (size_t) d.faces[3 * (size_t) f + j]];
+            const double Y[3] = { p[0] - eye[0], p[1] - eye[1], p[2] - eye[2] };
+            double c[3], q[3];
+            for (int a = 0; a < 3; ++a) c[a] = Ri[a][0] * Y[0] + Ri[a][1] * Y[1] + Ri[a][2] * Y[2];
+            for (int a = 0; a < 3; ++a) q[a] = Hi[a][0] * c[0] + Hi[a][1] * c[1] + Hi[a][2] * c[2];
+            if (!(c[2] >= near_lo) || !(q[2] > 0.0)) { t.projected = false; break; }
+            t.x[j] = (q[0] / q[2] - offx) * isx; t.y[j] = (q[1] / q[2] - offy) * isy; w[j] = 1.0 / q[2];
+            zmin = std::min(zmin, c[2]); zmax = std::max(zmax, c[2]);
+            if (!std::isfinite(t.x[j]) || !std::isfinite(t.y[j]) || !std::isfinite(w[j])) { t.projected = false; break; }
+        }
+        if (!t.projected) { everywhere = tree.lca(everywhere, (int32_t) tree.face_leaf[f]); continue; }
+        t.lox = std::min(t.x[0], std::min(t.x[1], t.x[2])); t.hix = std::max(t.x[0], std::max(t.x[1], t.x[2]));
+        t.loy = std::min(t.y[0], std::min(t.y[1], t.y[2])); t.hiy = std::max(t.y[0], std::max(t.y[1], t.y[2]));
+        const double area2 = (t.x[1] - t.x[0]) * (t.y[2] - t.y[0]) - (t.x[2] - t.x[0]) * (t.y[1] - t.y[0]), sg = area2 > 0.0 ? 1.0 : -1.0;
+        double lmax = 0.0;
+        for (int i = 0; i < 3; ++i) {
+            const int j = (i + 1) % 3;
+            t.ex[i] = -sg * (t.y[j] - t.y[i]); t.ey[i] = sg * (t.x[j] - t.x[i]); t.ec[i] = -(t.ex[i] * t.x[i] + t.ey[i] * t.y[i]);
+            t.el[i] = std::sqrt(t.ex[i] * t.ex[i] + t.ey[i] * t.ey[i]); lmax = std::max(lmax, t.el[i]);
+        }
+        t.has_area = area2 != 0.0 && std::isfinite(area2);
+        t.plane_ok = t.has_area && std::fabs(area2) > 1e-6 * lmax * lmax;
+        if (t.plane_ok) {
+            t.gx = ((w[1] - w[0]) * (t.y[2] - t.y[0]) - (w[2] - w[0]) * (t.y[1] - t.y[0])) / area2;
+            t.gy = ((t.x[1] - t.x[0]) * (w[2] - w[0]) - (t.x[2] - t.x[0]) * (w[1] - w[0])) / area2;
+            t.g0 = w[0] - t.gx * t.x[0] - t.gy * t.y[0];
+            t.plane_ok = std::isfinite(t.gx) && std::isfinite(t.gy) && std::isfinite(t.g0);
+        }
+        t.occluder = t.plane_ok && zmin >= near_hi && zmax <= far_lo;
+    }
+    const size_t npix = (size_t) W * (size_t) Hh;
+    auto for_pixels = [&](uint32_t f, auto &&fn) {
+        const PeTri &t = T[f];
+        const double x0 = std::ceil(t.lox - 1.0 - delta) - cox, x1 = std::floor(t.hix + delta) - cox, y0 = std::ceil(t.loy - 1.0 - delta) - coy, y1 = std::floor(t.hiy + delta) - coy;
+        if (!(x1 >= 0.0) || !(y1 >= 0.0) || !(x0 <= W - 1.0) || !(y0 <= Hh - 1.0)) return;
+        const int ix0 = (int) std::max(x0, 0.0), ix1 = (int) std::min(x1, W - 1.0), iy0 = (int) std::max(y0, 0.0), iy1 = (int) std::min(y1, Hh - 1.0);
+        double sup[3]; for (int i = 0; i < 3; ++i) sup[i] = half * (std::fabs(t.ex[i]) + std::fabs(t.ey[i]));
+        for (int y = iy0; y <= iy1; ++y) {
+            const double cy = (double) (y + coy) + 0.5;
+            for (int x = ix0; x <= ix1; ++x) {
+                const double cx = (double) (x + cox) + 0.5;
+                bool in = true;
+                if (t.has_area) for (int i = 0; i < 3; ++i) in = in && t.ex[i] * cx + t.ey[i] * cy + t.ec[i] + sup[i] >= 0.0;
+                if (in) fn((size_t) y * W + x);
+            }
+        }
+    };
+    std::vector<uint32_t> start(npix + 1, 0);
+    for (uint32_t f = 0; f < nf; ++f) if (T[f].projected) for_pixels(f, [&](size_t p) { ++start[p + 1]; });
+    for (size_t p = 0; p < npix; ++p) start[p + 1] += start[p];
+    std::vector<uint16_t> cand(start[npix]); std::vector<uint32_t> fill(start.begin(), start.end() - 1);
+    for (uint32_t f = 0; f < nf; ++f) if (T[f].projected) for_pixels(f, [&](size_t p) { cand[fill[p]++] = (uint16_t) f; });
+    out.assign(npix, 0);
+    for (int y = 0; y < Hh; ++y) for (int x = 0; x < W; ++x) {
+        const size_t p = (size_t) y * W + x; const uint32_t b = start[p], e = start[p + 1];
+        int32_t id = everywhere;
+        if (e - b == 1) id = tree.lca(id, (int32_t) tree.face_leaf[cand[b]]);
+        else if (e > b) {
+            const double cx = (double) (x + cox) + 0.5, cy = (double) (y + coy) + 0.5;
+            double cover = INFINITY;
+            for (uint32_t k = b; k < e; ++k) {
+                const PeTri &A = T[cand[k]];
+                if (!A.occluder) continue;
+                bool in = true;
+                for (int i = 0; i < 3; ++i) in = in && A.ex[i] * cx + A.ey[i] * cy + A.ec[i] - half * (std::fabs(A.ex[i]) + std::fabs(A.ey[i])) >= delta * A.el[i];
+                if (!in) continue;
+                const double gmin = A.gx * cx + A.gy * cy + A.g0 - half * (std::fabs(A.gx) + std::fabs(A.gy));
+                if (gmin > 0.0) cover = std::min(cover, 1.0 / gmin);
+            }
+            for (uint32_t k = b; k < e; ++k) {
+                const PeTri &t = T[cand[k]];
+                if (cover < INFINITY && t.plane_ok) {
+                    const double gc = t.gx * cx + t.gy * cy + t.g0, gs = half * (std::fabs(t.gx) + std::fabs(t.gy));
+                    if (gc - gs > 0.0 && 1.0 / (gc + gs) > cover * (1.0 + tune.depth_margin)) continue;
+                }
+                id = tree.lca(id, (int32_t) tree.face_leaf[cand[k]]);
+            }
+        }
+        out[p] = tree.item(id);
+    }
+}
+
 static float fresnel_diffuse_reflectance(float eta) {
     const float inv_eta = 1.f / eta;
     const float approx_1 = fmaf(0.0636f, inv_eta, fmaf(eta, fmaf(eta, -1.4399f, 0.7099f), 0.6681f));
@@ -398,7 +572,15 @@
             g.enabled = 1; sc.grid = g;
         }
     }
-    if (P.use_lds && !P.ext && sc.grid.enabled && !opt.no_cone_proof && closed_records(d, d.sensor.medium)) { build_cone_table(d, P.cone_tab); sc.cone_enabled = 1; }
+    const bool closed_lds = P.use_lds && !P.ext && sc.grid.enabled && closed_records(d, d.sensor.medium);
+    if (closed_lds && !opt.no_cone_proof) { build_cone_table(d, P.cone_tab); sc.cone_enabled = 1; }
+    if (closed_lds && !bvh.root_is_leaf && !opt.no_primary_entry) {
+        build_primary_entry(d, bvh, P.primary_tab);
+        if (!P.primary_tab.empty()) {
+            if (!primary_entry_valid(bvh, P.primary_tab)) throw std::runtime_error("primary entry table: an item names no node or leaf of the BVH");
+            sc.primary_enabled = 1;
+        }
+    }
 }
 
 void prepare_shading(const lrt_scene_desc &d, const PrepOptions &opt, PreparedScene &P) {
diff --git a/liverrenderer_amd/csrc/scene_prep.h b/liverrenderer_amd/csrc/scene_prep.h
--- a/liverrenderer_amd/csrc/scene_prep.h
+++ b/liverrenderer_amd/csrc/scene_prep.h
@@ -13,6 +13,7 @@
     int dist_grid_res = 0;
     bool no_nee_reject = false;
     bool no_cone_proof = false;
+    bool no_primary_entry = false;
     size_t lds_limit = 0;
     int n_cus = 256;
     static PrepOptions from_env();
@@ -37,6 +38,7 @@
     float grid_abs_margin = 0.f;
     std::vector<DPhase> phases; std::vector<float> phase_pool;
     std::vector<uint16_t> cone_tab;
+    std::vector<uint16_t> primary_tab;
     bool env_interior_positive = false;
     bool ext = false, has_area_emitter = false, has_het = false, has_non_bio = false, prb_null = false, use_lds = false;
     bool smooth_bsdf = false;
@@ -46,8 +48,15 @@
 void prepare_shading(const lrt_scene_desc &d, const PrepOptions &opt, PreparedScene &P);
 PreparedScene prepare_scene(const lrt_scene_desc &d, const PrepOptions &opt);
 
+void build_camera(const lrt_scene_desc &d, DCamera &cam, DFilm &film);
+
 void build_cone_table(const lrt_scene_desc &d, std::vector<uint16_t> &out);
 float cone_table_value(uint16_t h);
+
+#define LRT_PRIMARY_NONE 0xffffu
+struct PrimaryEntryTune { double delta = 1.0 / 16.0, depth_margin = 1e-4; };
+void build_primary_entry(const lrt_scene_desc &d, const HostBVH &bvh, std::vector<uint16_t> &out, const PrimaryEntryTune &tune = PrimaryEntryTune());
+bool primary_entry_valid(const HostBVH &bvh, const std::vector<uint16_t> &tab);
 
 size_t lds_image_bytes(const HostBVH &b, uint32_t n_vertices);
 bool lds_image_fits(const lrt_scene_desc &d, const HostBVH &b, const PrepOptions &opt);
```

Measured after the change: 6960 Msamples/s, median of 6. 7.1% higher.
